# Eun0/XMC-GAN

Measured on AMD Instinct MI355X. Metric: images/sec per G+D step, higher is better.
Workload: dtype bf16; 1 GPU; 256x256 COCO-shaped synthetic batch, 256 images per GPU, one full G+D iteration (D step + G step + Adam x2), df_gan_damsm_nomagp.yml; per_gpu_batch=256, global_batch=256, image_size=256, cfg=df_gan_damsm_nomagp.yml, parallelism=dp1, hipgraph=True, losses_finite=True, workload_name=headline

## Files before the change

include/xmc_gan_hip.h:

```cpp
#ifndef XMC_GAN_HIP_H
#define XMC_GAN_HIP_H

#include <stdint.h>

#ifdef __cplusplus
extern "C" {
#endif

#define XMC_ABI_VERSION 12

enum { XMC_BF16 = 0, XMC_F32 = 1 };
enum { XMC_HALF_IS_BF16 = 0, XMC_HALF_IS_F16 = 1 };
enum { XMC_ACT_NONE = 0, XMC_ACT_LRELU = 1, XMC_ACT_TANH = 2, XMC_ACT_RELU = 3 };
enum { XMC_EINVAL = -1, XMC_EALIGN = -2, XMC_ESHAPE = -3 };

#define XMC_MAX_TAPS 16
#define XMC_MAX_CLASSES 4

typedef struct XmcConvDesc {
    const void* src;
    const void* wpk;
    void* dst;
    const float* bias;
    const void* res;
// ... 12 lines not shown
    int8_t dw[XMC_MAX_CLASSES][XMC_MAX_TAPS];
    int8_t wi[XMC_MAX_CLASSES][XMC_MAX_TAPS];
    int8_t dph[XMC_MAX_CLASSES];
    int8_t dpw[XMC_MAX_CLASSES];
    const void* mask;
    float res_scale;
    int32_t res_mode;
    void* dst2;
    void* dst_pool;
    int32_t round_act;
    int32_t groups;
    int32_t post_act;
    float pool_scale;
    void* sign_bits;
    float* dot;
    const void* mask_bits;
    const void* sc_img;
    const void* sc_frag;
    const float* sc_bias;
    void* splitk_ws;
    int64_t splitk_ws_bytes;
    const void* wpk_lo;
} XmcConvDesc;

int xmc_abi_version(void);
int xmc_half_format(void);
const char* xmc_last_kernel(void);
int xmc_set_fixed_order(int on);
int xmc_set_prezeroed(int on);

int64_t xmc_conv_splitk_ws_bytes(const XmcConvDesc* d);

int xmc_conv_igemm(const XmcConvDesc* d, void* stream);

int xmc_conv_wgrad(const XmcConvDesc* d , float* dwp, void* stream);
#define XMC_BIAS_REPLICAS 16
int xmc_conv_wgrad_bias(const XmcConvDesc* d, float* dwp, float* dbias, void* stream);

int xmc_pack_weight(const float* w, void* wpk, int Co, int Ci, int KH, int KW, int rows_pad, int cols_pad,
                    int transpose , int dtype, const int32_t* row_perm , void* stream);
int xmc_pack_weight_grouped(const float* w, void* wpk, int Co, int Ci, int KH, int KW, int rows_pad, int cols_pad, int transpose,
                            int dtype, const int32_t* row_perm, int groups, void* stream);
int xmc_unpack_wgrad_grouped(const float* dwp, float* gw, int Co, int Ci, int KH, int KW, int rows_pad, int cols_pad,
                             const float* scale_dev, const int32_t* row_perm, int accumulate, int groups, void* stream);
#define XMC_PACK_MULTI_MAX 48
typedef struct XmcPackJob {
    const float* w;
    void* wpk;
    const int32_t* row_perm;
    int32_t Co, Ci, KHW, rows_pad, cols_pad, transpose, dtype, groups, upconv;
    int32_t lo;
} XmcPackJob;
int xmc_pack_weight_multi(const XmcPackJob* jobs , int njobs, void* stream);
int xmc_pack_weight_upconv(const float* w, void* wpk, int Co, int Ci, int rows_pad, int cols_pad, int transpose, int dtype,
                           void* stream);
int xmc_unpack_wgrad(const float* dwp, float* gw, int Co, int Ci, int KH, int KW, int rows_pad, int cols_pad,
                     const float* scale_dev, const int32_t* row_perm, int accumulate, void* stream);
int xmc_unpack_wgrad_bias(const float* dwp, float* gw, int Co, int Ci, int KH, int KW, int rows_pad, int cols_pad,
                          const float* scale_dev, const int32_t* row_perm, int accumulate,
                          const float* gb_replicas, float* gb, int CD, void* stream);
int xmc_unpack_wgrad_bias_dot(const float* dwp, float* gw, int Co, int Ci, int KH, int KW, int rows_pad, int cols_pad,
                              const float* scale_dev, const int32_t* row_perm, int accumulate,
                              const float* gb_replicas, float* gb, int CD, const float* bias_dot, float* dot, void* stream);

int xmc_nchw_to_nhwc8(const float* src , void* dst , int N, int C, int H, int W,
                      int dtype, void* stream);
// ... 223 lines not shown
```

xmc-gan_amd/csrc/common.h:

```cpp
#pragma once
#include <hip/hip_runtime.h>
#include <stdint.h>

#include "xmc_gan_hip.h"

#ifdef XMC_H16_IS_F16
typedef _Float16 xmc_h16;
#define XMC_MFMA_16x16x32 __builtin_amdgcn_mfma_f32_16x16x32_f16
#define XMC_MFMA_32x32x16 __builtin_amdgcn_mfma_f32_32x32x16_f16
#define XMC_HALF_FORMAT 1
#else
typedef __bf16 xmc_h16;
#define XMC_MFMA_16x16x32 __builtin_amdgcn_mfma_f32_16x16x32_bf16
#define XMC_MFMA_32x32x16 __builtin_amdgcn_mfma_f32_32x32x16_bf16
#define XMC_HALF_FORMAT 0
#endif
typedef __attribute__((ext_vector_type(8))) xmc_h16 bf16x8;
typedef __attribute__((ext_vector_type(4))) xmc_h16 bf16x4;
typedef __attribute__((ext_vector_type(4))) float f32x4;
typedef __attribute__((__vector_size__(4 * sizeof(short)))) short xmc_s16x4;
typedef __attribute__((ext_vector_type(4))) uint32_t u32x4;
typedef __attribute__((ext_vector_type(2))) uint32_t u32x2;

#define XMC_LRELU 0.2f
// ... 78 lines not shown

struct XcdWalk { int first, step, end; };
__device__ __forceinline__ XcdWalk xmc_xcd_walk(int ntiles) {
    const int G = (int)gridDim.x, b = (int)blockIdx.x;
#ifdef XMC_XCD_HELPER_OFF
    return XcdWalk{b, G, ntiles};
#endif
    if ((G & 7) != 0 || G < 16) return XcdWalk{b, G, ntiles};
    const int T8 = (ntiles + 7) >> 3, base = (b & 7) * T8;
    return XcdWalk{base + (b >> 3), G >> 3, base + T8 < ntiles ? base + T8 : ntiles};
}
static inline int xmc_ab_grid(int g) {
    static const bool off = xmc_debug_off("no_xcd_map");
    return (off && g >= 16 && (g & 7) == 0) ? g - 1 : g;
}

__device__ __forceinline__ float xmc_xor1(float v) {
    return __builtin_bit_cast(float, __builtin_amdgcn_mov_dpp(__builtin_bit_cast(int, v), 0xB1, 0xF, 0xF, true));
}
__device__ __forceinline__ float xmc_xor2(float v) {
    return __builtin_bit_cast(float, __builtin_amdgcn_mov_dpp(__builtin_bit_cast(int, v), 0x4E, 0xF, 0xF, true));
}
__device__ __forceinline__ float wave_sum(float v) {
#pragma unroll
    for (int o = 32; o > 0; o >>= 1) v += __shfl_xor(v, o, 64);
    return v;
}
__device__ __forceinline__ float wave_max(float v) {
#pragma unroll
    for (int o = 32; o > 0; o >>= 1) v = fmaxf(v, __shfl_xor(v, o, 64));
    return v;
}

template <int ODT>
__device__ __forceinline__ void epilogue_tail(const XmcConvDesc& d, size_t idx8, size_t ridx8, float (&v)[8], float alpha, float* dacc = nullptr) {
    if (d.sign_bits) {
        unsigned b = 0;
#pragma unroll
        for (int k = 0; k < 8; ++k) b |= (v[k] > 0.f ? 1u : 0u) << k;
        reinterpret_cast<unsigned char*>(d.sign_bits)[idx8] = (unsigned char)b;
    }
    if (d.dst2) Vec8<ODT>::store(d.dst2, idx8, v);
    if (ODT == XMC_BF16 && (d.dst2 || d.round_act)) {
#pragma unroll
        for (int k = 0; k < 8; ++k) v[k] = (float)(xmc_h16)v[k];
    }
    float mk[8];
    if (d.mask) {
        Vec8<ODT>::load(d.mask, idx8, mk);
        if (d.dot && dacc) {
#pragma unroll
            for (int k = 0; k < 8; ++k) *dacc += v[k] * mk[k];
        }
    }
    if (d.alpha_dev) {
#pragma unroll
        for (int k = 0; k < 8; ++k) v[k] *= alpha;
    }
    if (d.mask) {
#pragma unroll
        for (int k = 0; k < 8; ++k) v[k] *= lrelu_slope(mk[k]);
    }
    if (d.res) {
        const float rs = d.res_scale == 0.f ? 1.f : d.res_scale;
        float rr[8];
        Vec8<ODT>::load(d.res, ridx8, rr);
#pragma unroll
        for (int k = 0; k < 8; ++k) v[k] += rs * rr[k];
    }
    if (d.post_act == XMC_ACT_LRELU) {
#pragma unroll
        for (int k = 0; k < 8; ++k) v[k] = lrelu_f(v[k]);
    }
    Vec8<ODT>::store(d.dst, idx8, v);
}

constexpr int kEpiBias = 1, kEpiLrelu = 2, kEpiRound = 4, kEpiDst2 = 8, kEpiAlpha = 16, kEpiMask = 32, kEpiRes = 64, kEpiPost = 128, kEpiPool = 256,
              kEpiSign = 512, kEpiDot = 1024, kEpiScImg = 2048;
constexpr int kEpiGSum = kEpiBias | kEpiRound | kEpiAlpha | kEpiRes;
constexpr int kEpiDKeep = kEpiLrelu | kEpiDst2 | kEpiAlpha | kEpiRes | kEpiPool;
constexpr int kEpiDFwd = kEpiLrelu | kEpiRound | kEpiAlpha | kEpiRes | kEpiPool;
constexpr int kEpiDLast = kEpiLrelu | kEpiDst2 | kEpiAlpha | kEpiRes;
constexpr int kEpiDLin = kEpiDst2 | kEpiAlpha | kEpiMask | kEpiRes;
constexpr int kEpiDKeepS = kEpiLrelu | kEpiRound | kEpiSign | kEpiAlpha | kEpiRes | kEpiPool;
constexpr int kEpiDLastS = kEpiLrelu | kEpiRound | kEpiSign | kEpiAlpha | kEpiRes;
constexpr int kEpiDgDot = kEpiMask | kEpiAlpha | kEpiDot;
static inline int xmc_epi_mask(const XmcConvDesc& d) {
    if ((d.act != XMC_ACT_NONE && d.act != XMC_ACT_LRELU) || d.out_dtype != XMC_BF16) return -1;
    return (d.bias ? kEpiBias : 0) | (d.act == XMC_ACT_LRELU ? kEpiLrelu : 0) | ((d.round_act && !d.dst2) ? kEpiRound : 0) | (d.dst2 ? kEpiDst2 : 0) |
           (d.alpha_dev ? kEpiAlpha : 0) | (d.mask ? kEpiMask : 0) | (d.res ? kEpiRes : 0) | (d.post_act == XMC_ACT_LRELU ? kEpiPost : 0) |
           (d.dst_pool ? kEpiPool : 0) | (d.sign_bits ? kEpiSign : 0) | (d.dot ? kEpiDot : 0) | (d.sc_img ? kEpiScImg : 0);
}

__device__ __forceinline__ size_t res_index8(const XmcConvDesc& d, size_t idx8, int n, int y, int x, int a, int b, int ch8) {
    if (d.res_mode == 0) return idx8;
    if (d.res_mode == 1) return ((size_t)(n * d.MH + a) * d.MW + b) * (d.CD >> 3) + ch8;
    return ((size_t)(n * (d.DH >> 1) + (y >> 1)) * (d.DW >> 1) + (x >> 1)) * (d.CD >> 3) + ch8;
}
```

xmc-gan_amd/csrc/conv_igemm.hip:

```cpp
#include "common.h"
#include <stdlib.h>

#ifndef XMC_IGEMM_PIN
#define XMC_IGEMM_PIN 1
#endif

namespace {

template <int DT> struct Mma;
template <> struct Mma<XMC_BF16> {
    __device__ static __forceinline__ f32x4 run(u32x4 a, u32x4 b, f32x4 c) {
        return XMC_MFMA_16x16x32(__builtin_bit_cast(bf16x8, a), __builtin_bit_cast(bf16x8, b), c, 0, 0, 0);
    }
};
template <> struct Mma<XMC_F32> {
    __device__ static __forceinline__ f32x4 run(u32x4 a, u32x4 b, f32x4 c) {
        f32x4 af = __builtin_bit_cast(f32x4, a), bf = __builtin_bit_cast(f32x4, b);
#pragma unroll
        for (int j = 0; j < 4; ++j) c = __builtin_amdgcn_mfma_f32_16x16x4f32(af[j], bf[j], c, 0, 0, 0);
        return c;
    }
};

__device__ __forceinline__ int swz(int row) {
    int q = (row >> 2) & 3;
    return (((q ^ (q >> 1)) & 1) << 1) | (q >> 1);
}

template <int BM, int BN, int KSUB>
struct IgemmLds {
    static constexpr int STAGE_U = 2 * KSUB * (BM + BN) * 4;
    static constexpr int EP_LD = BN + 4;
    static constexpr int EP_ROWS = BN > 128 ? 64 : (BM > 128 ? 128 : BM);
    static constexpr int EP_U = (EP_ROWS * EP_LD * 4 + 15) / 16;
    static constexpr int SMEM_U = STAGE_U > EP_U ? STAGE_U : EP_U;
    static constexpr bool DYNAMIC = SMEM_U * 16 + 4 * XMC_MAX_TAPS > 64 * 1024;
};

template <int ODT>
__device__ __forceinline__ void igemm_epi_item(const XmcConvDesc& d, int cls, int m, int ch, float (&v)[8], float alpha, float* dacc) {
    const int MHW = d.MH * d.MW;
    const int n = m / MHW, rem = m - n * MHW;
    const int a = rem / d.MW, b = rem - a * d.MW;
    const int dph = d.dph[cls], dpw = d.dpw[cls];
    const size_t pix = ((size_t)n * d.DH + a * d.DA + dph) * d.DW + b * d.DA + dpw;
    const size_t idx8 = (pix * d.CD + ch) >> 3;
    if (d.bias) {
#pragma unroll
        for (int k = 0; k < 8; ++k) v[k] += d.bias[ch + k];
    }
    if (d.act == XMC_ACT_LRELU) {
#pragma unroll
        for (int k = 0; k < 8; ++k) v[k] = lrelu_f(v[k]);
    } else if (d.act == XMC_ACT_RELU) {
#pragma unroll
        for (int k = 0; k < 8; ++k) v[k] = fmaxf(v[k], 0.f);
    } else if (d.act == XMC_ACT_TANH) {
#pragma unroll
        for (int k = 0; k < 8; ++k) v[k] = tanhf(v[k]);
    }
    const size_t ridx8 = res_index8(d, idx8, n, a * d.DA + dph, b * d.DA + dpw, a, b, ch >> 3);
    epilogue_tail<ODT>(d, idx8, ridx8, v, alpha, dacc);
}

template <int DT, int BM, int BN, int WM, int WN, int KSUB, bool SK = false>
__global__ __launch_bounds__(64 * WM * WN) void igemm_kernel(const XmcConvDesc d) {
    constexpr int NT = 64 * WM * WN;
    static_assert(WM * WN == 4 || WM * WN == 8, "4 or 8 waves");
    constexpr int RP = NT / 4;
    constexpr int WTM = BM / WM, WTN = BN / WN;
    constexpr int TM = WTM / 16, TN = WTN / 16;
    constexpr int AL = BM * 4 / NT;
    constexpr int BL = (BN * 4 + NT - 1) / NT;
    using Lds = IgemmLds<BM, BN, KSUB>;
    constexpr int EP_LD = Lds::EP_LD, EP_ROWS = Lds::EP_ROWS;
    extern __shared__ u32x4 smem_dyn[];
    __shared__ u32x4 smem_static[Lds::DYNAMIC ? 1 : Lds::SMEM_U];
    u32x4* const smem = Lds::DYNAMIC ? smem_dyn : smem_static;
    __shared__ int s_tap[XMC_MAX_TAPS];

    const int tid = threadIdx.x, lane = tid & 63, wave = tid >> 6;
    const int wm = wave / WN, wn = wave % WN;
    const int cls = blockIdx.z;
    const int MHW = d.MH * d.MW;
    const int M = d.N * MHW;
    int mt, nt;
    {
        const int MT = (M + BM - 1) / BM, NTn = d.CDw / BN;
        const int bid = blockIdx.x, nwg = MT * NTn;
        const int xcd = bid & 7, j = bid >> 3;
        const int q = nwg >> 3, r = nwg & 7;
        const int lin = (xcd < r ? xcd * (q + 1) : r * (q + 1) + (xcd - r) * q) + j;
        mt = lin / NTn; nt = lin - mt * NTn;
    }
    const int m0 = mt * BM, n0 = nt * BN;
    constexpr int ESZ = DT == XMC_BF16 ? 2 : 4;
    const int upt = d.CS * ESZ / 16;
    const int ktot = d.ntaps * upt;
    const int nsub = (ktot + 3) / 4;
// ... 117 lines not shown
    const float alpha = d.alpha_dev ? *d.alpha_dev : 1.f;
    float dacc = 0.f;
    constexpr int CPR = BN / 8;
    for (int half = 0; half < BM / EP_ROWS; ++half) {
        if (half) __syncthreads();
#pragma unroll
        for (int i = 0; i < TM; ++i) {
            const int rbase = wm * WTM + i * 16;
            if (rbase / EP_ROWS == half) {
#pragma unroll
                for (int j = 0; j < TN; ++j)
#pragma unroll
                    for (int r = 0; r < 4; ++r)
                        ep[(rbase - half * EP_ROWS + fc * 4 + r) * EP_LD + wn * WTN + j * 16 + fr] = acc[i][j][r];
            }
        }
        __syncthreads();
        for (int id = tid; id < EP_ROWS * CPR; id += NT) {
            int row = id / CPR, cc = id - row * CPR;
            int m = m0 + half * EP_ROWS + row, ch = n0 + cc * 8;
            if (m >= M) continue;
            const f32x4 e0 = *reinterpret_cast<const f32x4*>(&ep[row * EP_LD + cc * 8]);
            const f32x4 e1 = *reinterpret_cast<const f32x4*>(&ep[row * EP_LD + cc * 8 + 4]);
            if (SK) {
                f32x4* w = reinterpret_cast<f32x4*>(reinterpret_cast<float*>(d.splitk_ws) +
                                                    (((size_t)blockIdx.y * gridDim.z + cls) * M + m) * d.CDw + ch);
                w[0] = e0; w[1] = e1;
                continue;
            }
            if (ch >= d.CD) continue;
            float v[8];
#pragma unroll
            for (int k = 0; k < 4; ++k) { v[k] = e0[k]; v[4 + k] = e1[k]; }
            if (d.out_dtype == XMC_BF16) igemm_epi_item<XMC_BF16>(d, cls, m, ch, v, alpha, &dacc);
            else igemm_epi_item<XMC_F32>(d, cls, m, ch, v, alpha, &dacc);
        }
    }
    if (SK) return;
    if (d.dot) {
        dacc = wave_sum(dacc);
        if (lane == 0) atomicAdd(d.dot, dacc);
    }
}

constexpr int SK_FIN_ITEMS = 4;
__global__ __launch_bounds__(256) void igemm_splitk_finish_kernel(const XmcConvDesc d, int S) {
    const int cls = blockIdx.z;
    const int M = d.N * d.MH * d.MW, C8 = d.CD / 8;
    const float alpha = d.alpha_dev ? *d.alpha_dev : 1.f;
    float dacc = 0.f;
    for (int it = 0; it < SK_FIN_ITEMS; ++it) {
        const int64_t id = ((int64_t)blockIdx.x * SK_FIN_ITEMS + it) * 256 + threadIdx.x;
        if (id >= (int64_t)M * C8) break;
        const int m = (int)(id / C8), ch = (int)(id - (int64_t)m * C8) * 8;
        const float* w = reinterpret_cast<const float*>(d.splitk_ws) + ((size_t)cls * M + m) * d.CDw + ch;
        const size_t stride = (size_t)gridDim.z * M * d.CDw;
        float v[8] = {0, 0, 0, 0, 0, 0, 0, 0};
        for (int s = 0; s < S; ++s) {
            const f32x4 e0 = *reinterpret_cast<const f32x4*>(w + s * stride), e1 = *reinterpret_cast<const f32x4*>(w + s * stride + 4);
#pragma unroll
            for (int k = 0; k < 4; ++k) { v[k] += e0[k]; v[4 + k] += e1[k]; }
        }
        if (d.out_dtype == XMC_BF16) igemm_epi_item<XMC_BF16>(d, cls, m, ch, v, alpha, &dacc);
        else igemm_epi_item<XMC_F32>(d, cls, m, ch, v, alpha, &dacc);
    }
    if (d.dot) {
        __shared__ float sdot[4];
        dacc = wave_sum(dacc);
        if ((threadIdx.x & 63) == 0) sdot[threadIdx.x >> 6] = dacc;
        __syncthreads();
        if (threadIdx.x == 0) atomicAdd(d.dot, sdot[0] + sdot[1] + sdot[2] + sdot[3]);
    }
}

struct SkPlan { int S, big; };
static SkPlan splitk_plan(const XmcConvDesc& d) {
    static const bool off = xmc_debug_off("no_igemm_splitk"), no_big = xmc_debug_off("no_igemm_splitk256");
    SkPlan p = {0, 0};
    if (off || d.dtype != XMC_BF16 || d.CDw % 64 != 0) return p;
    const int64_t M = (int64_t)d.N * d.MH * d.MW, K = (int64_t)d.ntaps * d.CS;
    if (M > 16384 || K < 4096 || d.nclass != 1) return p;
    const int nstep = (int)((K * 2 / 16 + 3) / 4 + 1) / 2;
    p.big = (d.CDw % 256 == 0 && !no_big) ? 1 : (d.CDw % 128 == 0 ? 0 : 2);
    if (p.big == 1) {
        const int64_t t256 = (M + 255) / 256 * (d.CDw / 256);
        if (t256 * (nstep / 4 < 8 ? nstep / 4 : 8) < 192) p.big = 0;
    }
    const int BMp = p.big == 1 ? 256 : 128, BNp = p.big == 1 ? 256 : (p.big == 0 ? 128 : 64);
    const int64_t tiles = (M + BMp - 1) / BMp * (d.CDw / BNp) * d.nclass;
    int S = (int)((p.big == 1 ? 256 : 1024) / tiles);
    if (S > (p.big == 2 ? 16 : 8)) S = p.big == 2 ? 16 : 8;
    if (S > nstep / 4) S = nstep / 4;
    p.S = S >= 2 ? S : 0;
    return p;
}
static int64_t splitk_bytes(const XmcConvDesc& d, int S) { return (int64_t)S * d.nclass * d.N * d.MH * d.MW * d.CDw * 4; }

template <int BM, int BN, int WM, int WN>
int launch_splitk(const XmcConvDesc& d, int S, hipStream_t st) {
    const int64_t M = (int64_t)d.N * d.MH * d.MW;
    dim3 grid((unsigned)(((M + BM - 1) / BM) * (d.CDw / BN)), (unsigned)S, (unsigned)d.nclass);
    using Lds = IgemmLds<BM, BN, 2>;
    size_t dyn = 0;
    if (Lds::DYNAMIC) {
        dyn = (size_t)Lds::SMEM_U * 16;
        XMC_ALLOW_BIG_LDS((igemm_kernel<XMC_BF16, BM, BN, WM, WN, 2, true>));
    }
    hipLaunchKernelGGL((igemm_kernel<XMC_BF16, BM, BN, WM, WN, 2, true>), grid, dim3(64 * WM * WN), dyn, st, d);
    xmc_note_kernel("igemm_kernel<%d, %d, %d, %d, %d, %d, true>", XMC_BF16, BM, BN, WM, WN, 2);
    XMC_LAUNCH_CHECK();
    const int64_t items = M * (d.CD / 8);
    hipLaunchKernelGGL(igemm_splitk_finish_kernel, dim3((unsigned)((items + 256 * SK_FIN_ITEMS - 1) / (256 * SK_FIN_ITEMS)), 1, (unsigned)d.nclass), dim3(256), 0, st, d, S);
    XMC_LAUNCH_CHECK();
    return 0;
}

template <int DT, int BM, int BN, int WM, int WN, int KSUB>
int launch(const XmcConvDesc& d, hipStream_t st) {
    const int64_t M = (int64_t)d.N * d.MH * d.MW;
    dim3 grid((unsigned)(((M + BM - 1) / BM) * (d.CDw / BN)), 1, (unsigned)d.nclass);
    using Lds = IgemmLds<BM, BN, KSUB>;
    size_t dyn = 0;
    if (Lds::DYNAMIC) {
        dyn = (size_t)Lds::SMEM_U * 16;
        XMC_ALLOW_BIG_LDS((igemm_kernel<DT, BM, BN, WM, WN, KSUB>));
    }
    hipLaunchKernelGGL((igemm_kernel<DT, BM, BN, WM, WN, KSUB>), grid, dim3(64 * WM * WN), dyn, st, d);
    xmc_note_kernel("igemm_kernel<%d, %d, %d, %d, %d, %d>", DT, BM, BN, WM, WN, KSUB);
    XMC_LAUNCH_CHECK();
    return 0;
}

template <int DT>
int dispatch(const XmcConvDesc& d, hipStream_t st) {
    static const int variant = xmc_debug_off("igemm128") ? 1 : 0;
    static const bool no_small = xmc_debug_off("no_small_m");
    if (DT == XMC_BF16 && d.splitk_ws) {
        const SkPlan sp = splitk_plan(d);
        if (sp.S && d.splitk_ws_bytes >= splitk_bytes(d, sp.S))
            return sp.big == 1 ? launch_splitk<256, 256, 2, 4>(d, sp.S, st) : sp.big == 0 ? launch_splitk<128, 128, 2, 2>(d, sp.S, st)
                                                                                             : launch_splitk<128, 64, 4, 1>(d, sp.S, st);
    }
    if (!no_small && (int64_t)d.N * d.MH * d.MW <= 1024) return launch<DT, 128, 32, 4, 1, 2>(d, st);
    if (d.CDw % 128 == 0) {
        const int64_t M = (int64_t)d.N * d.MH * d.MW;
        if (variant == 1) return launch<DT, 128, 128, 2, 2, 2>(d, st);
        static const bool no_big = xmc_debug_off("no_igemm256");
        const int64_t tiles256 = (M + 255) / 256 * (d.CDw / 256) * d.nclass;
        if (DT == XMC_BF16 && (M >= 256 * 256 || tiles256 >= 256) && d.CDw % 256 == 0 && !no_big) return launch<DT, 256, 256, 2, 4, 2>(d, st);
        if (DT == XMC_BF16 && M >= 256 * 256) return launch<DT, 256, 128, 2, 2, 1>(d, st);
        static const bool no_m64 = xmc_debug_off("no_igemm_m64");
        static const bool no_k4 = xmc_debug_off("no_igemm_ksub4");
        const bool deepk = DT == XMC_BF16 && !no_k4 && (int64_t)d.ntaps * d.CS >= 2048;
        const int64_t t128 = (M + 127) / 128 * (d.CDw / 128) * d.nclass;
        if (DT == XMC_BF16 && !no_m64 && t128 < 256) {
            if (deepk && (M + 63) / 64 * (d.CDw / 128) * d.nclass <= 256) return launch<DT, 64, 128, 2, 2, 4>(d, st);
            return launch<DT, 64, 128, 2, 2, 2>(d, st);
        }
        if (deepk && t128 <= 256) return launch<DT, 128, 128, 2, 2, 4>(d, st);
        return launch<DT, 128, 128, 2, 2, 2>(d, st);
    }
    if (d.CDw % 64 == 0) {
        static const bool no_k4b = xmc_debug_off("no_igemm_ksub4");
        const int64_t Mb = (int64_t)d.N * d.MH * d.MW;
        if (DT == XMC_BF16 && !no_k4b && (int64_t)d.ntaps * d.CS >= 2048 && (Mb + 127) / 128 * (d.CDw / 64) * d.nclass <= 256)
            return launch<DT, 128, 64, 4, 1, 4>(d, st);
        return launch<DT, 128, 64, 4, 1, 2>(d, st);
    }
    return launch<DT, 128, 32, 4, 1, 2>(d, st);
}

}

int xmc_conv_tile_try(const XmcConvDesc* d, void* stream);
int xmc_conv_thin_try(const XmcConvDesc* d, void* stream);
int xmc_conv_pw1x1_try(const XmcConvDesc* d, void* stream);
int xmc_conv_wtile_try(const XmcConvDesc* d, void* stream);
int xmc_conv_wtile3_try(const XmcConvDesc* d, void* stream);
int xmc_conv_ptile_pool_try(const XmcConvDesc* d, void* stream);
int xmc_conv_ptile_slab128_try(const XmcConvDesc* d, void* stream);
int xmc_conv_group_try(const XmcConvDesc* d, void* stream);
int xmc_conv_thin_out_try(const XmcConvDesc* d, void* stream);

extern "C" int64_t xmc_conv_splitk_ws_bytes(const XmcConvDesc* d) {
    if (!d) return 0;
    const SkPlan sp = splitk_plan(*d);
    return sp.S ? splitk_bytes(*d, sp.S) : 0;
}

extern "C" int xmc_conv_igemm(const XmcConvDesc* d, void* stream) {
    if (!d || !d->src || !d->wpk || !d->dst) return XMC_EINVAL;
    if (d->dtype != XMC_BF16 && d->dtype != XMC_F32) return XMC_EINVAL;
    if (d->out_dtype != XMC_BF16 && d->out_dtype != XMC_F32) return XMC_EINVAL;
    const int esz = xmc_esz(d->dtype);
    if (d->ntaps < 1 || d->ntaps > XMC_MAX_TAPS || d->nclass < 1 || d->nclass > XMC_MAX_CLASSES) return XMC_ESHAPE;
    if ((d->CS * esz) % 16 != 0 || d->CD % 8 != 0 || d->CDw % 32 != 0 || d->CDw < d->CD) return XMC_EALIGN;
    if (d->N < 1 || d->MH < 1 || d->MW < 1 || d->SH < 1 || d->SW < 1 || d->DH < 1 || d->DW < 1) return XMC_ESHAPE;
    if (d->src_shift < 0 || d->src_shift > 1 || d->SA < 1 || d->DA < 1) return XMC_ESHAPE;
    for (int z = 0; z < d->nclass; ++z)
        if ((d->MH - 1) * d->DA + d->dph[z] >= d->DH || (d->MW - 1) * d->DA + d->dpw[z] >= d->DW || d->dph[z] < 0 || d->dpw[z] < 0)
            return XMC_ESHAPE;
    if ((int64_t)d->N * d->MH * d->MW >= (1ll << 31)) return XMC_ESHAPE;
    if (d->dst_pool && (d->DA != 1 || d->nclass != 1 || (d->DH & 1) || (d->DW & 1) || d->out_dtype != d->dtype)) return XMC_ESHAPE;
    if (d->post_act != XMC_ACT_NONE && d->post_act != XMC_ACT_LRELU) return XMC_EINVAL;
    if (d->dot && !d->mask) return XMC_EINVAL;
    if (d->mask_bits) return XMC_EINVAL;
    if (d->sc_img) return XMC_EINVAL;
    if (d->wpk_lo) return XMC_EINVAL;
    if (d->res_mode < 0 || d->res_mode > 2 || (d->res_mode == 2 && (d->DA != 1 || (d->DH & 1) || (d->DW & 1)))) return XMC_ESHAPE;
    static const bool no_tile = xmc_debug_off("no_tile");
    static const bool no_wt2 = xmc_debug_off("no_wtile_v2");
    static const bool no_wt3 = xmc_debug_off("no_wtile3");
    int rc = 1;
    if (!no_tile && d->dst_pool) {
        rc = xmc_conv_thin_try(d, stream);
        if (rc > 0 && !no_wt3) rc = xmc_conv_wtile3_try(d, stream);
        if (rc > 0 && !no_wt2) rc = xmc_conv_wtile_try(d, stream);
        if (rc > 0) rc = xmc_conv_ptile_pool_try(d, stream);
        if (rc <= 0) return rc;
    }
    XmcConvDesc dd = *d;
    dd.dst_pool = nullptr;
    if (!no_tile) {
        rc = xmc_conv_group_try(&dd, stream);
        if (rc > 0) rc = xmc_conv_thin_try(&dd, stream);
        if (rc > 0) rc = xmc_conv_thin_out_try(&dd, stream);
        if (rc > 0) rc = xmc_conv_pw1x1_try(&dd, stream);
        if (rc > 0) rc = xmc_conv_ptile_slab128_try(&dd, stream);
        if (rc > 0 && !no_wt3) rc = xmc_conv_wtile3_try(&dd, stream);
        if (rc > 0 && !no_wt2) rc = xmc_conv_wtile_try(&dd, stream);
        if (rc > 0) rc = xmc_conv_tile_try(&dd, stream);
        if (rc < 0) return rc;
    }
    if (rc > 0) {
        hipStream_t st = reinterpret_cast<hipStream_t>(stream);
        rc = dd.dtype == XMC_BF16 ? dispatch<XMC_BF16>(dd, st) : dispatch<XMC_F32>(dd, st);
        if (rc != 0) return rc;
    }
    if (d->dst_pool) return xmc_sumpool2(d->dst, d->dst_pool, d->N, d->DH, d->DW, d->CD, d->pool_scale == 0.f ? 0.25f : d->pool_scale, d->out_dtype, stream);
    return 0;
}
```

xmc-gan_amd/csrc/conv_tile.hip:

```cpp
#include "common.h"
#include <stdlib.h>
#include <type_traits>

namespace {

struct TileCfg {
    int TH, TW, log2TW;
    int tiles_y, tiles_x;
    int PH[XMC_MAX_CLASSES], PW[XMC_MAX_CLASSES];
    int dh0[XMC_MAX_CLASSES], dw0[XMC_MAX_CLASSES];
    int PHu, PWu, dh0u, dw0u;
    int slab;
    int no_xcd;
};

template <int BN, int WM, int WN>
__global__ __launch_bounds__(256) void tile_kernel(const XmcConvDesc d, const TileCfg t) {
    constexpr int NT = 256, BM = 256;
    static_assert(WM * WN == 4, "4 waves");
    constexpr int WTM = BM / WM, WTN = BN / WN;
    constexpr int TM = WTM / 16, TN = WTN / 16;
    constexpr int EP_ROWS = 128, EP_LD = BN + 4;
    extern __shared__ __attribute__((aligned(16))) unsigned char smem[];

// ... 139 lines not shown
            size_t pix = ((size_t)img * d.DH + (a0 + ty) * d.DA + dph) * d.DW + (b0 + tx) * d.DA + dpw;
            size_t idx8 = (pix * d.CD + ch) >> 3;
            float v[8];
            const f32x4 e0 = *reinterpret_cast<const f32x4*>(&ep[row * EP_LD + cc * 8]);
            const f32x4 e1 = *reinterpret_cast<const f32x4*>(&ep[row * EP_LD + cc * 8 + 4]);
#pragma unroll
            for (int k = 0; k < 4; ++k) { v[k] = e0[k]; v[4 + k] = e1[k]; }
            if (d.bias) {
#pragma unroll
                for (int k = 0; k < 8; ++k) v[k] += d.bias[ch + k];
            }
            if (d.act == XMC_ACT_LRELU) {
#pragma unroll
                for (int k = 0; k < 8; ++k) v[k] = lrelu_f(v[k]);
            } else if (d.act == XMC_ACT_RELU) {
#pragma unroll
                for (int k = 0; k < 8; ++k) v[k] = fmaxf(v[k], 0.f);
            } else if (d.act == XMC_ACT_TANH) {
#pragma unroll
                for (int k = 0; k < 8; ++k) v[k] = tanhf(v[k]);
            }
            const size_t ridx8 = res_index8(d, idx8, img, (a0 + ty) * d.DA + dph, (b0 + tx) * d.DA + dpw, a0 + ty, b0 + tx, (n0 >> 3) + cc);
            if (d.out_dtype == XMC_BF16) epilogue_tail<XMC_BF16>(d, idx8, ridx8, v, alpha, &dacc);
            else epilogue_tail<XMC_F32>(d, idx8, ridx8, v, alpha, &dacc);
        }
    }
    if (d.dot) {
        dacc = wave_sum(dacc);
        if (lane == 0) atomicAdd(d.dot, dacc);
    }
}


template <int BN, int SLAB, int NTAPS, int MC, int SA = 1, bool M32 = false, int EPI = -1>
__global__ __launch_bounds__(512) void ptile3_kernel(const XmcConvDesc d, const TileCfg t, int ntiles) {
    static_assert(!M32 || (SA == 1 && NTAPS > 0), "32x32x16 form: unit stride, unrolled taps");
    constexpr int NS = 256;
    constexpr int TM = SA == 1 ? 4 : 2, TN = BN / 16;
    constexpr int cps = SLAB / 8;
    constexpr int pstride = SLAB * 2 + (M32 ? 16 : 32);
    constexpr int PIT = ((SA == 1 ? 384 : 18 * 34) * cps + NS - 1) / NS;
    constexpr int UPL = BN / 32;
    constexpr int S = SLAB / 32;
    extern __shared__ __attribute__((aligned(16))) unsigned char smem[];

    const int tid = threadIdx.x, lane = tid & 63, wave = tid >> 6;
    const bool stager = wave >= 4;
    const int rt = tid & (NS - 1);
    const int wm = wave & 3;
    const int cls = MC > 1 ? 0 : blockIdx.z;
    const int n0 = blockIdx.y * BN;
    const int tpi = t.tiles_y * t.tiles_x;
    const int PH = MC > 1 ? t.PHu : t.PH[cls], PW = MC > 1 ? t.PWu : t.PW[cls];
    const int dh0 = MC > 1 ? t.dh0u : t.dh0[cls], dw0 = MC > 1 ? t.dw0u : t.dw0[cls];
    __shared__ int s_toff[XMC_MAX_TAPS];
    __shared__ __attribute__((aligned(16))) float s_bias[M32 ? 2 * BN : 4];
    if (M32 && tid >= 64 && tid < 64 + BN) {
        const int ch = n0 + tid - 64;
        s_bias[tid - 64] = (d.bias && ch < d.CD) ? d.bias[ch] : 0.f;
        s_bias[BN + tid - 64] = (d.sc_bias && ch < d.CD) ? d.sc_bias[ch] : 0.f;
    }
    if (tid < XMC_MAX_TAPS) {
        const int sl = tid < MC * d.ntaps ? tid : 0;
        const int c = MC > 1 ? sl / d.ntaps : cls, tt = MC > 1 ? sl % d.ntaps : sl;
        const int th = d.dh[c][tt] - dh0, tw = d.dw[c][tt] - dw0;
        s_toff[tid] = (SA == 1 ? th * PW + tw : (th * 2 + (tw & 1)) * (PW >> 1) + (tw >> 1)) * pstride;
    }
    const int cs_units = d.CS / 8;
    unsigned char* patch = smem;
// ... 317 lines not shown
                            dst8[idx8] = o;
                        }
                    if (MC == 1 && e_pool) {
                        bf16x8* __restrict__ pool8 = reinterpret_cast<bf16x8*>(d.dst_pool);
#pragma unroll
                        for (int v2 = 0; v2 < 2; ++v2) {
                            if (t.log2TW == 5) {
                                bf16x8 o;
#pragma unroll
                                for (int r = 0; r < 8; ++r) {
                                    float sm = fin[0][v2][r] + fin[1][v2][r];
                                    sm += xmc_xor1(sm);
                                    o[r] = (xmc_h16)(pscale * sm);
                                }
                                if ((l32 & 1) == 0)
                                    pool8[((img * (d.DH >> 1) + ((a0 + pty[0]) >> 1)) * (d.DW >> 1) + ((b0 + ptx[0]) >> 1)) * cd8 + (n0 >> 3) + ub + v2] = o;
                            } else {
#pragma unroll
                                for (int pb = 0; pb < 2; ++pb) {
                                    bf16x8 o;
#pragma unroll
                                    for (int r = 0; r < 8; ++r) {
                                        float sm = fin[pb][v2][r];
                                        sm += __shfl_xor(sm, 16, 64);
                                        sm += xmc_xor1(sm);
                                        o[r] = (xmc_h16)(pscale * sm);
                                    }
                                    if ((l32 & 17) == 0)
                                        pool8[((img * (d.DH >> 1) + ((a0 + pty[pb]) >> 1)) * (d.DW >> 1) + ((b0 + ptx[pb]) >> 1)) * cd8 + (n0 >> 3) + ub + v2] = o;
                                }
                            }
                        }
                    }
                }
                if (e_sign && pack_sign) {
#pragma unroll
                    for (int pb = 0; pb < 2; ++pb) {
                        const unsigned keep = hh == 0 ? (sgn[pb] & 0xFFFFu) : (sgn[pb] >> 16);
                        const unsigned send = hh == 0 ? (sgn[pb] >> 16) : (sgn[pb] & 0xFFFFu);
                        const unsigned recv = (unsigned)__shfl_xor((int)send, 32, 64);
                        const unsigned word = hh == 0 ? (keep | (recv << 16)) : (recv | (keep << 16));
                        reinterpret_cast<unsigned*>(d.sign_bits)[(size_t)(eo[pb] >> 2) + hh] = word;
                    }
                }
            }
        }
        if (e_dot) {
            dacc = wave_sum(dacc);
            if (lane == 0) atomicAdd(d.dot, dacc);
        }
    } else {
        const int fr = lane & 15, fc = lane >> 4;
        const int cd8 = d.CD / 8;
        int abyte[TM], eoff[TM], roff[TM];
#pragma unroll
        for (int i = 0; i < TM; ++i) {
            const int ml = wm * (16 * TM) + i * 16 + fr;
            const int ty = ml >> t.log2TW, tx = ml & (t.TW - 1);
            abyte[i] = ((SA == 1 ? ty * PW : 2 * ty * PW) + tx) * pstride + fc * 16;
            eoff[i] = ((ty * d.DA) * d.DW + tx * d.DA) * cd8 + fc;
            roff[i] = (ty * d.MW + tx) * cd8 + fc;
        }
        const int bbyte = fr * pstride + fc * 16;
        const int ch0 = n0 + fc * 8;
        const float alpha = d.alpha_dev ? *d.alpha_dev : 1.f;
        const float pscale = d.pool_scale == 0.f ? 0.25f : d.pool_scale;
        float bias8[UPL][8];
#pragma unroll
        for (int u = 0; u < UPL; ++u)
#pragma unroll
            for (int c = 0; c < 8; ++c) bias8[u][c] = (d.bias && ch0 + u * 32 < d.CD) ? d.bias[ch0 + u * 32 + c] : 0.f;
        constexpr bool RT = EPI < 0;
        constexpr int EB = RT ? 0 : (EPI & ~kEpiBias);
        const bool fast = RT ? (d.out_dtype == XMC_BF16 && d.res == nullptr && d.mask == nullptr && d.alpha_dev == nullptr && d.dst2 == nullptr &&
                                d.dst_pool == nullptr && d.post_act == XMC_ACT_NONE && d.sign_bits == nullptr && d.dot == nullptr &&
                                (d.act == XMC_ACT_NONE || d.act == XMC_ACT_LRELU || d.act == XMC_ACT_TANH))
                             : (EB == 0 || EB == kEpiLrelu);
        const bool do_tanh = RT ? d.act == XMC_ACT_TANH : false;
        const float slope = RT ? (d.act == XMC_ACT_LRELU ? XMC_LRELU : 1.f) : ((EPI & kEpiLrelu) ? XMC_LRELU : 1.f);
        const bool e_lrelu = RT ? d.act == XMC_ACT_LRELU : (EPI & kEpiLrelu) != 0;
        const bool e_relu = RT ? d.act == XMC_ACT_RELU : false;
        const bool e_round = RT ? (d.dst2 != nullptr || d.round_act != 0) : (EPI & (kEpiRound | kEpiDst2)) != 0;
        const bool e_dst2 = RT ? d.dst2 != nullptr : (EPI & kEpiDst2) != 0;
        const bool e_alpha = RT ? d.alpha_dev != nullptr : (EPI & kEpiAlpha) != 0;
        const bool e_mask = RT ? d.mask != nullptr : (EPI & kEpiMask) != 0;
        const bool e_res = RT ? d.res != nullptr : (EPI & kEpiRes) != 0;
        const bool e_post = RT ? d.post_act == XMC_ACT_LRELU : (EPI & kEpiPost) != 0;
        const bool e_pool = RT ? d.dst_pool != nullptr : (EPI & kEpiPool) != 0;
        constexpr bool e_sign = !RT && (EPI & kEpiSign) != 0;
        constexpr bool e_dot = !RT && (EPI & kEpiDot) != 0;
        float dacc = 0.f;
        __syncthreads();
        int toffr[NTAPS > 0 ? MC * NTAPS : 1];
        if constexpr (NTAPS > 0) {
#pragma unroll
            for (int k = 0; k < MC * NTAPS; ++k) toffr[k] = __builtin_amdgcn_readfirstlane(s_toff[k]);
        }
        for (int tile = tile0; tile < xlim; tile += tstep) {
            const int img = tile / tpi, trem = tile - img * tpi;
            const int a0 = (trem / t.tiles_x) * t.TH, b0 = (trem % t.tiles_x) * t.TW;
            __syncthreads();
            constexpr bool HOIST = UPL == 1;
            bf16x8 mkv[HOIST ? TM : 1], rrv[HOIST ? TM : 1];
#pragma unroll
          for (int mc = 0; mc < MC; ++mc) {
            const int ccls = MC > 1 ? mc : cls;
// ... 54 lines not shown
                for (int g = 0; g < G; ++g) fr_[0][gslot(g)] = rd(0, gslot(g));
#pragma unroll
                for (int st = 0; st < NST; ++st) {
                    const int cur = st & 1, nxt = cur ^ 1;
#pragma unroll
                    for (int g = 0; g < G; ++g) {
                        if (st + 1 < NST) fr_[nxt][gslot(g)] = rd(st + 1, gslot(g));
#pragma unroll
                        for (int m = g * M / G; m < (g + 1) * M / G; ++m) {
                            const int mi = m % TM, mj = m / TM;
                            acc[mi][mj] = XMC_MFMA_16x16x32(__builtin_bit_cast(bf16x8, fr_[cur][TM + mj]),
                                                                                   __builtin_bit_cast(bf16x8, fr_[cur][mi]), acc[mi][mj], 0, 0, 0);
                        }
                        __builtin_amdgcn_sched_barrier(0);
                    }
                }
            } else {
                u32x4 pf[2][TM], wf[2][TN];
                const int nsteps = d.ntaps * S;
                ldfrag(s_toff[0], 0, 0, pf[0], wf[0]);
                for (int step = 0; step < nsteps; step += 2) {
                    if (step + 1 < nsteps) ldfrag(s_toff[(step + 1) / S], (step + 1) / S, (step + 1) % S, pf[1], wf[1]);
                    mma(pf[0], wf[0]);
                    if (step + 2 < nsteps) ldfrag(s_toff[(step + 2) / S], (step + 2) / S, (step + 2) % S, pf[0], wf[0]);
                    if (step + 1 < nsteps) mma(pf[1], wf[1]);
                }
            }
            if (mc == MC - 1) __syncthreads();
            if (fast) {
                bf16x8* __restrict__ dst8 = reinterpret_cast<bf16x8*>(d.dst) + dbase;
#pragma unroll
                for (int u = 0; u < UPL; ++u) {
                    if (ch0 + u * 32 >= d.CD) continue;
#pragma unroll
                    for (int i = 0; i < TM; ++i) {
                        bf16x8 o;
                        if (slope != 1.f) {
#pragma unroll
                            for (int q = 0; q < 4; ++q) {
                                const float x0 = acc[i][2 * u][q] + bias8[u][q], x1 = acc[i][2 * u + 1][q] + bias8[u][4 + q];
                                o[q] = (xmc_h16)fmaxf(x0, x0 * slope);
                                o[4 + q] = (xmc_h16)fmaxf(x1, x1 * slope);
                            }
                        } else if (do_tanh) {
#pragma unroll
                            for (int q = 0; q < 4; ++q) {
                                o[q] = (xmc_h16)tanh_fast(acc[i][2 * u][q] + bias8[u][q]);
                                o[4 + q] = (xmc_h16)tanh_fast(acc[i][2 * u + 1][q] + bias8[u][4 + q]);
                            }
                        } else {
#pragma unroll
                            for (int q = 0; q < 4; ++q) {
                                o[q] = (xmc_h16)(acc[i][2 * u][q] + bias8[u][q]);
                                o[4 + q] = (xmc_h16)(acc[i][2 * u + 1][q] + bias8[u][4 + q]);
                            }
                        }
                        dst8[eoff[i] + u * 4] = o;
                    }
                }
            } else {
#pragma unroll
                for (int u = 0; u < UPL; ++u) {
                    if (ch0 + u * 32 >= d.CD) continue;
                    float fin[TM][8];
                    size_t rix[TM];
                    bf16x8 mkl[HOIST ? 1 : TM], rrl[HOIST ? 1 : TM];
                    if (!pre || !HOIST) {
#pragma unroll
                        for (int i = 0; i < TM; ++i) {
                            const size_t idx8 = (size_t)(dbase + eoff[i] + u * 4);
                            rix[i] = d.res_mode == 1 ? (size_t)(rbase + roff[i] + u * 4) : idx8;
                            if (d.res_mode == 2) {
                                const int ml_ = wm * (16 * TM) + i * 16 + fr;
                                const int y_ = (a0 + (ml_ >> t.log2TW)) * d.DA + dph, x_ = (b0 + (ml_ & (t.TW - 1))) * d.DA + dpw;
                                rix[i] = res_index8(d, idx8, img, y_, x_, 0, 0, (n0 >> 3) + fc + u * 4);
                            }
                            if (pre && e_mask) mkl[HOIST ? 0 : i] = reinterpret_cast<const bf16x8*>(d.mask)[idx8];
                            if (pre && e_res) rrl[HOIST ? 0 : i] = reinterpret_cast<const bf16x8*>(d.res)[rix[i]];
                        }
                    }
#pragma unroll
                    for (int i = 0; i < TM; ++i) {
                        const size_t idx8 = (size_t)(dbase + eoff[i] + u * 4);
                        float v[8];
#pragma unroll
                        for (int q = 0; q < 4; ++q) { v[q] = acc[i][2 * u][q] + bias8[u][q]; v[4 + q] = acc[i][2 * u + 1][q] + bias8[u][4 + q]; }
                        if (e_lrelu) {
#pragma unroll
                            for (int q = 0; q < 8; ++q) v[q] = lrelu_f(v[q]);
                        } else if (e_relu) {
// ... 48 lines not shown
                            for (int q = 0; q < 8; ++q) fin[i][q] = v[q];
                        }
                    }
                    if (SA == 1 && MC == 1 && TM == 4 && e_pool) {
                        bf16x8* __restrict__ pool8 = reinterpret_cast<bf16x8*>(d.dst_pool);
#pragma unroll
                        for (int pr = 0; pr < 2; ++pr) {
                            const int i0 = t.log2TW == 5 ? pr : 2 * pr;
                            const int ml_ = wm * 64 + i0 * 16 + fr;
                            const int ty_ = ml_ >> t.log2TW, tx_ = ml_ & (t.TW - 1);
                            bf16x8 o;
#pragma unroll
                            for (int q = 0; q < 8; ++q) {
                                float sm = t.log2TW == 5 ? fin[pr][q] + fin[(pr + 2) % TM][q] : fin[(2 * pr) % TM][q] + fin[(2 * pr + 1) % TM][q];
                                sm += xmc_xor1(sm);
                                o[q] = (xmc_h16)(pscale * sm);
                            }
                            if ((fr & 1) == 0)
                                pool8[((img * (d.DH >> 1) + ((a0 + ty_) >> 1)) * (d.DW >> 1) + ((b0 + tx_) >> 1)) * cd8 + (n0 >> 3) + fc + u * 4] = o;
                        }
                    }
                }
            }
          }
        }
        if (e_dot) {
            dacc = wave_sum(dacc);
            if (lane == 0) atomicAdd(d.dot, dacc);
        }
    }
}

template <int BN>
int launch_ptile(const XmcConvDesc& d, const TileCfg& t, hipStream_t st) {
    if (d.sc_img && !(d.SA == 1 && d.ntaps == 9 && d.nclass == 1 && t.slab == 64 && d.out_dtype == XMC_BF16 && (d.dst_pool || d.sign_bits))) return XMC_ESHAPE;
    int maxpatch = 0;
    for (int z = 0; z < d.nclass; ++z) maxpatch = t.PH[z] * t.PW[z] > maxpatch ? t.PH[z] * t.PW[z] : maxpatch;
    if (d.SA == 2) {
        const size_t lds2 = (size_t)((maxpatch * 96 + 15) & ~15) + (size_t)16 * BN * 96;
        if (lds2 > XMC_MAX_DYN_LDS || t.slab != 32) return XMC_ESHAPE;
        const int nt2 = d.N * t.tiles_y * t.tiles_x;
        int g2 = 256 / (int)(d.CDw / BN);
        if (g2 > nt2) g2 = nt2;
        static const bool no_epi2 = xmc_debug_off("no_ptile_epi");
        const int epi2 = no_epi2 ? -1 : (xmc_epi_mask(d) & ~kEpiBias);
#define XMC_PT3S2(E)                                                                                                        \
        if (epi2 == (E)) {                                                                                                  \
            XMC_ALLOW_BIG_LDS((ptile3_kernel<BN, 32, 16, 1, 2, false, (E)>));                                               \
            hipLaunchKernelGGL((ptile3_kernel<BN, 32, 16, 1, 2, false, (E)>), dim3(g2, d.CDw / BN, 1), dim3(512), lds2, st, d, t, nt2); \
            xmc_note_kernel("ptile3_kernel<%d, 32, 16, 1, 2>", BN);                                                         \
            XMC_LAUNCH_CHECK();                                                                                             \
            return 0;                                                                                                       \
        }
        XMC_PT3S2(kEpiLrelu) XMC_PT3S2(0) XMC_PT3S2(kEpiMask)
#undef XMC_PT3S2
        if (d.sign_bits || d.dot) return XMC_ESHAPE;
        xmc_note_generic_epi("ptile3<s2>", epi2);
        XMC_ALLOW_BIG_LDS((ptile3_kernel<BN, 32, 16, 1, 2>));
        hipLaunchKernelGGL((ptile3_kernel<BN, 32, 16, 1, 2>), dim3(g2, d.CDw / BN, 1), dim3(512), lds2, st, d, t, nt2);
        xmc_note_kernel("ptile3_kernel<%d, 32, 16, 1, 2>", BN);
        XMC_LAUNCH_CHECK();
        return 0;
    }
    if (maxpatch > 384) return XMC_ESHAPE;
    const int pstride = t.slab * 2 + 32;
    const size_t pb = (size_t)((maxpatch * pstride + 15) & ~15);
    const size_t lds = pb + (size_t)d.ntaps * BN * pstride;
    if (lds > XMC_MAX_DYN_LDS) return XMC_ESHAPE;
    const int ntiles = d.N * t.tiles_y * t.tiles_x;
    const int per_cu = (lds <= 80 * 1024 && BN == 32 && t.slab == 32) ? 2 : 1;
    int gx = 256 * per_cu / (int)((d.CDw / BN) * d.nclass);
    if (gx < 1) gx = 1;
    if (gx > ntiles) gx = ntiles;
    dim3 grid((unsigned)gx, (unsigned)(d.CDw / BN), (unsigned)d.nclass);
    if (t.slab == 128) {
        if (BN != 64 || d.ntaps != 4 || d.sign_bits || d.dot) return XMC_ESHAPE;
        const int epis = xmc_debug_off("no_ptile_epi") ? -1 : (xmc_epi_mask(d) & ~kEpiBias);
#define XMC_PT3W(E)                                                                                                         \
        if (epis == (E)) {                                                                                                  \
            XMC_ALLOW_BIG_LDS((ptile3_kernel<64, 128, 4, 1, 1, false, (E)>));                                               \
            hipLaunchKernelGGL((ptile3_kernel<64, 128, 4, 1, 1, false, (E)>), grid, dim3(512), lds, st, d, t, ntiles);      \
        } else
        XMC_PT3W(kEpiRes) XMC_PT3W(0)
#undef XMC_PT3W
        {
            xmc_note_generic_epi("ptile3<128>", epis);
            XMC_ALLOW_BIG_LDS((ptile3_kernel<64, 128, 4, 1>));
            hipLaunchKernelGGL((ptile3_kernel<64, 128, 4, 1>), grid, dim3(512), lds, st, d, t, ntiles);
        }
        xmc_note_kernel("ptile3_kernel<64, 128, 4, 1>");
        XMC_LAUNCH_CHECK();
        return 0;
    }
    if (d.nclass == 4 && d.ntaps == 4 && t.PHu * t.PWu <= 384) {
        const size_t ldsm = (size_t)((t.PHu * t.PWu * pstride + 15) & ~15) + (size_t)16 * BN * pstride;
        static const bool no_merge = xmc_debug_off("no_class_merge");
        if (ldsm <= XMC_MAX_DYN_LDS && !no_merge) {
            int gm = 256 / (int)(d.CDw / BN);
            if (gm > ntiles) gm = ntiles;
            dim3 gridm((unsigned)gm, (unsigned)(d.CDw / BN), 1);
            if (d.sign_bits || d.dot) return XMC_ESHAPE;
            static const bool no_epim = xmc_debug_off("no_ptile_epi");
            const int epim = no_epim ? -1 : (xmc_epi_mask(d) & ~kEpiBias);
#define XMC_PT3M(SL, E)                                                                                                     \
            if (t.slab == (SL) && epim == (E)) {                                                                            \
                XMC_ALLOW_BIG_LDS((ptile3_kernel<BN, SL, 4, 4, 1, false, (E)>));                                            \
                hipLaunchKernelGGL((ptile3_kernel<BN, SL, 4, 4, 1, false, (E)>), gridm, dim3(512), ldsm, st, d, t, ntiles); \
            } else
            XMC_PT3M(64, kEpiRes) XMC_PT3M(64, 0) XMC_PT3M(32, kEpiRes) XMC_PT3M(32, 0)
#undef XMC_PT3M
            if (t.slab == 64) {
                xmc_note_generic_epi("ptile3<4,4>", epim);
                XMC_ALLOW_BIG_LDS((ptile3_kernel<BN, 64, 4, 4>));
                hipLaunchKernelGGL((ptile3_kernel<BN, 64, 4, 4>), gridm, dim3(512), ldsm, st, d, t, ntiles);
            } else {
                XMC_ALLOW_BIG_LDS((ptile3_kernel<BN, 32, 4, 4>));
                hipLaunchKernelGGL((ptile3_kernel<BN, 32, 4, 4>), gridm, dim3(512), ldsm, st, d, t, ntiles);
            }
            xmc_note_kernel("ptile3_kernel<%d, %d, 4, 4>", BN, t.slab);
            XMC_LAUNCH_CHECK();
            return 0;
        }
    }
    static const bool no_m32 = xmc_debug_off("no_ptile_m32");
    static const bool m32_all = xmc_debug_off("ptile_m32_all");
    if (!no_m32 && d.ntaps == 9 && d.out_dtype == XMC_BF16 && t.slab == 64 &&
        (m32_all || d.res || d.dst2 || d.dst_pool || d.mask || d.sign_bits)) {
        int epi = xmc_epi_mask(d);
        static const bool no_epi = xmc_debug_off("no_ptile_epi");
        if (no_epi) epi = -1;
        if (d.sc_img) {
            if (BN != 64 || d.res || t.TW != 32 || d.CD != 64 || lds + 18 * 66 * 8 > XMC_MAX_DYN_LDS) return XMC_ESHAPE;
#define XMC_PT3_SCI(E)                                                                                                   \
            if (epi == (E)) {                                                                                            \
                XMC_ALLOW_BIG_LDS((ptile3_kernel<64, 64, 9, 1, 1, true, (E)>));                                          \
                hipLaunchKernelGGL((ptile3_kernel<64, 64, 9, 1, 1, true, (E)>), grid, dim3(512), lds + 18 * 66 * 8, st, d, t, ntiles); \
                xmc_note_kernel("ptile3_kernel<64, 64, 9, 1, 1, true, sc>");                                             \
                XMC_LAUNCH_CHECK();                                                                                      \
                return 0;                                                                                                \
            }
            XMC_PT3_SCI((kEpiDKeepS & ~kEpiRes) | kEpiScImg) XMC_PT3_SCI((kEpiDFwd & ~kEpiRes) | kEpiScImg)
#undef XMC_PT3_SCI
            return XMC_ESHAPE;
        }
#define XMC_PT3_EPI(E)                                                                                                   \
        if (epi == (E)) {                                                                                                \
            XMC_ALLOW_BIG_LDS((ptile3_kernel<BN, 64, 9, 1, 1, true, (E)>));                                              \
            hipLaunchKernelGGL((ptile3_kernel<BN, 64, 9, 1, 1, true, (E)>), grid, dim3(512), lds, st, d, t, ntiles);     \
            xmc_note_kernel("ptile3_kernel<%d, 64, 9, 1, 1, true>", BN);                                                 \
            XMC_LAUNCH_CHECK();                                                                                          \
            return 0;                                                                                                    \
        }
        XMC_PT3_EPI(kEpiGSum) XMC_PT3_EPI(kEpiDKeep) XMC_PT3_EPI(kEpiDFwd) XMC_PT3_EPI(kEpiDLast) XMC_PT3_EPI(kEpiDLin)
        XMC_PT3_EPI(kEpiDKeepS) XMC_PT3_EPI(kEpiDLastS) XMC_PT3_EPI(kEpiDgDot)
        XMC_PT3_EPI(kEpiMask)
#undef XMC_PT3_EPI
        if (d.sign_bits || d.dot) return XMC_ESHAPE;
        xmc_note_generic_epi("ptile3<M32>", epi);
// ... 100 lines not shown
    if (!(d->CS <= 64 && t.slab == d->CS && d->CDw <= 64) || xmc_debug_off("no_ptile")) return 1;
    const int rc = d->CDw == 64 ? launch_ptile<64>(*d, t, reinterpret_cast<hipStream_t>(stream))
                                : launch_ptile<32>(*d, t, reinterpret_cast<hipStream_t>(stream));
    return rc == XMC_ESHAPE ? 1 : rc;
}

extern "C" int xmc_conv_ptile_scimg(const XmcConvDesc* d, void* stream) {
    if (!d || !d->src || !d->wpk || !d->dst || !d->sc_img || !d->sc_frag || !d->sc_bias) return XMC_EINVAL;
    static const bool off = xmc_debug_off("no_scimg");
    if (off || d->res || d->dtype != XMC_BF16 || d->out_dtype != XMC_BF16 || d->SA != 1 || d->DA != 1 || d->nclass != 1 || d->ntaps != 9 ||
        d->src_shift != 0 || d->CS != 64 || d->CDw != 64 || d->CD != 64 || d->MW % 32 != 0 || d->MH % 8 != 0 || d->SH != d->MH || d->SW != d->MW ||
        d->DH != d->MH || d->DW != d->MW || xmc_debug_off("no_ptile") || xmc_debug_off("no_ptile_m32") || xmc_debug_off("no_ptile_epi"))
        return 1;
    for (int k = 0; k < 9; ++k)
        if (d->dh[0][k] < -1 || d->dh[0][k] > 1 || d->dw[0][k] < -1 || d->dw[0][k] > 1) return 1;
    TileCfg t;
    if (!tile_plan(d, &t) || t.slab != 64) return 1;
    const int rc = launch_ptile<64>(*d, t, reinterpret_cast<hipStream_t>(stream));
    return rc == XMC_ESHAPE ? 1 : rc;
}

extern "C" int xmc_conv_ptile_bits(const XmcConvDesc* d, void* stream) {
    if (!d || !d->src || !d->wpk || !d->dst || !d->mask_bits) return XMC_EINVAL;
    static const bool off = xmc_debug_off("no_stage_bits");
    if (off || d->dtype != XMC_BF16 || d->SA != 1 || d->DA != 1 || d->nclass != 1 || d->src_shift != 0 || d->dst_pool) return 1;
    TileCfg t;
    if (!tile_plan(d, &t)) return 1;
    if (!(d->CS <= 64 && t.slab == d->CS && d->CDw <= 64) || xmc_debug_off("no_ptile")) return 1;
    const int rc = d->CDw == 64 ? launch_ptile<64>(*d, t, reinterpret_cast<hipStream_t>(stream))
                                : launch_ptile<32>(*d, t, reinterpret_cast<hipStream_t>(stream));
    return rc == XMC_ESHAPE ? 1 : rc;
}

int xmc_conv_ptile_slab128_try(const XmcConvDesc* d, void* stream) {
    if (d->CS != 128 || d->CDw != 64 || d->ntaps != 4 || d->nclass != 4 || d->dst_pool || xmc_debug_off("no_ptile")) return 1;
    TileCfg t;
    if (!tile_plan(d, &t) || t.slab != 128) return 1;
    const int rc = launch_ptile<64>(*d, t, reinterpret_cast<hipStream_t>(stream));
    return rc == XMC_ESHAPE ? 1 : rc;
}

int xmc_conv_tile_try(const XmcConvDesc* d, void* stream) {
    TileCfg t;
    if (!tile_plan(d, &t)) return 1;
    if (t.slab == 128) return 1;
    hipStream_t st = reinterpret_cast<hipStream_t>(stream);
    int rc;
    static const bool no_pt = xmc_debug_off("no_ptile");
    if (!no_pt && d->CS <= 64 && t.slab == d->CS && d->CDw <= 64) {
        rc = d->CDw == 64 ? launch_ptile<64>(*d, t, st) : launch_ptile<32>(*d, t, st);
        if (rc != XMC_ESHAPE) return rc;
    }
    static const bool no_pt128 = xmc_debug_off("no_ptile_cd128");
    if (!no_pt && !no_pt128 && d->CS == 32 && t.slab == 32 && d->CDw == 128 && d->SA == 1 && d->nclass == 1 && d->ntaps == 9) {
        rc = launch_ptile<64>(*d, t, st);
        if (rc != XMC_ESHAPE) return rc;
    }
    if (d->SA != 1) return 1;
    if (d->CDw % 128 == 0) rc = launch_tile<128, 2, 2>(*d, t, st);
    else if (d->CDw % 64 == 0) rc = launch_tile<64, 4, 1>(*d, t, st);
    else rc = launch_tile<32, 4, 1>(*d, t, st);
    return rc == XMC_ESHAPE ? 1 : rc;
}
```

xmc-gan_amd/csrc/conv_wtile.hip:

```cpp
#include "common.h"
#include <stdlib.h>
#include <type_traits>

#ifndef WT_ABL
#define WT_ABL 0
#endif

namespace {

struct WtCfg {
    int TH, TW, log2TW;
    int tiles_y, tiles_x;
    int PH[XMC_MAX_CLASSES], PW[XMC_MAX_CLASSES];
    int dh0[XMC_MAX_CLASSES], dw0[XMC_MAX_CLASSES];
    int nslab;
    int patch_bytes;
    int8_t tsel[4][4];
};

constexpr int kPStride = 160;
constexpr int kPIT = 12;

template <int NTAPS, int MODE, int TN, int CW, int EPI = -1>
__global__ __launch_bounds__(64 * CW + 256) void wtile2_kernel(const XmcConvDesc d, const WtCfg t, int ntiles) {
    constexpr int BN = 16 * TN, TM = 4, NS = 64 * CW;
    constexpr int TNW = TN * 4 / CW;
    static_assert(CW == 4 || CW == 8, "4 or 8 compute waves");
    static_assert(TNW % 2 == 0, "a lane's 8-channel unit needs a pair of blocks");
    constexpr int WL = BN / 32;
    constexpr int WSTG = BN * 128;
    extern __shared__ __attribute__((aligned(16))) unsigned char smem[];
    __shared__ int s_toff[XMC_MAX_TAPS];
    __shared__ int s_wbase[XMC_MAX_TAPS];
    __shared__ int s_slab[64];

    const int tid = threadIdx.x, lane = tid & 63, wave = tid >> 6;
    const int n0 = blockIdx.y * BN;
    const int cls = blockIdx.z;
    const int tpi = t.tiles_y * t.tiles_x;
    const int PW = t.PW[cls];
    const int dh0 = MODE == 0 ? t.dh0[cls] : 0, dw0 = MODE == 0 ? t.dw0[cls] : 0;
    const int cs_units = d.CS / 8;
    const int nslab = t.nslab;
    const int cb = d.CS / 64;
    if (tid < XMC_MAX_TAPS) {
        if (MODE == 0) {
            const int tt = tid < NTAPS ? tid : 0;
            s_toff[tid] = ((d.dh[cls][tt] - dh0) * PW + (d.dw[cls][tt] - dw0)) * kPStride;
            s_wbase[tid] = d.wi[cls][tt] * d.CDw * cs_units;
        } else {
            const int g4 = tid >> 2, tp = tid & 3;
            s_toff[tid] = ((tp >> 1) * PW + (tp & 1)) * kPStride;
            s_wbase[tid] = d.wi[0][t.tsel[g4][tp]] * d.CDw * cs_units;
        }
    }
    if (tid >= 64 && tid < 128) {
        const int sl = tid - 64;
// ... 167 lines not shown
        auto rdw = [&](const unsigned char* wb, int sub, int mj) -> u32x4 {
            return *reinterpret_cast<const u32x4*>(wb + (sub ? bb1 : bb0) + mj * 2048);
        };
        const int ch0 = n0 + wn * (BN / 2) * (CW / 4 - 1) + fc * 8;
        const int nw8 = (n0 + wn * (BN / 2) * (CW / 4 - 1)) >> 3;
        auto epilogue = [&](int tile) {
            int lane_op = fr;
            asm volatile("" : "+v"(lane_op) :: "memory");
            const int img = tile / tpi, trem = tile - img * tpi;
            const int a0 = (trem / t.tiles_x) * t.TH, b0 = (trem % t.tiles_x) * t.TW;
            const int dbase = (((img * d.DH + a0 * d.DA + d.dph[cls]) * d.DW) + b0 * d.DA + d.dpw[cls]) * cd8 + nw8;
            const int rbase = d.res_mode ? ((img * d.MH + a0) * d.MW + b0) * cd8 + nw8 : dbase;
            const int rsy = d.res_mode ? d.MW : d.DA * d.DW, rsx = d.res_mode ? 1 : d.DA;
            constexpr bool RT = EPI < 0;
            const bool e_bias = RT ? d.bias != nullptr : (EPI & kEpiBias) != 0;
            const bool e_tanh = RT ? d.act == XMC_ACT_TANH : false;
            const bool e_round = RT ? (d.dst2 != nullptr || d.round_act != 0) : (EPI & (kEpiRound | kEpiDst2)) != 0;
            const bool e_dst2 = RT ? d.dst2 != nullptr : (EPI & kEpiDst2) != 0;
            const bool e_alpha = RT ? d.alpha_dev != nullptr : (EPI & kEpiAlpha) != 0;
            const bool e_mask = RT ? d.mask != nullptr : (EPI & kEpiMask) != 0;
            const bool e_res = RT ? d.res != nullptr : (EPI & kEpiRes) != 0;
            const bool e_post = RT ? d.post_act == XMC_ACT_LRELU : (EPI & kEpiPost) != 0;
            const bool e_pool = RT ? d.dst_pool != nullptr : (EPI & kEpiPool) != 0;
            constexpr bool e_sign = !RT && (EPI & kEpiSign) != 0;
            constexpr bool e_dot = !RT && (EPI & kEpiDot) != 0;
            const float slope = RT ? (d.act == XMC_ACT_LRELU ? XMC_LRELU : (d.act == XMC_ACT_RELU ? 0.f : 1.f)) : ((EPI & kEpiLrelu) ? XMC_LRELU : 1.f);
            const float alpha = d.alpha_dev ? *d.alpha_dev : 1.f;
            const float rs = d.res_scale == 0.f ? 1.f : d.res_scale;
            bf16x8* __restrict__ dst8 = reinterpret_cast<bf16x8*>(d.dst);
            const bf16x8* __restrict__ mask8 = reinterpret_cast<const bf16x8*>(d.mask);
            const bf16x8* __restrict__ res8 = reinterpret_cast<const bf16x8*>(d.res);
            bf16x8* __restrict__ dst2_8 = reinterpret_cast<bf16x8*>(d.dst2);
            bf16x8* __restrict__ pool8 = reinterpret_cast<bf16x8*>(d.dst_pool);
            int eo[TM], ro[TM];
#pragma unroll
            for (int i = 0; i < TM; ++i) {
                const int ml = wm * 64 + i * 16 + lane_op;
                const int ty = ml >> t.log2TW, tx = ml & (t.TW - 1);
                eo[i] = dbase + ((ty * d.DA) * d.DW + tx * d.DA) * cd8 + fc;
                if (d.res_mode == 2)
                    ro[i] = ((img * (d.DH >> 1) + ((a0 + ty) >> 1)) * (d.DW >> 1) + ((b0 + tx) >> 1)) * cd8 + nw8 + fc;
                else
                    ro[i] = rbase + (ty * rsy + tx * rsx) * cd8 + fc;
            }
#pragma unroll
            for (int u = 0; u < TNW / 2; ++u) {
                if (ch0 + u * 32 >= d.CD) continue;
                float fin[TM][8];
                bf16x8 mkv[TM], rrv[TM];
                if (e_mask) {
#pragma unroll
                    for (int i = 0; i < TM; ++i) mkv[i] = mask8[eo[i] + u * 4];
                }
                if (e_res) {
#pragma unroll
                    for (int i = 0; i < TM; ++i) rrv[i] = res8[ro[i] + u * 4];
                }
#pragma unroll
                for (int i = 0; i < TM; ++i) {
                    float v[8];
#pragma unroll
                    for (int r = 0; r < 4; ++r) { v[r] = acc[i][2 * u][r]; v[4 + r] = acc[i][2 * u + 1][r]; }
                    if (e_bias && !(WT_ABL & 32)) {
                        const f32x4 b0v = *reinterpret_cast<const f32x4*>(d.bias + ch0 + u * 32), b1v = *reinterpret_cast<const f32x4*>(d.bias + ch0 + u * 32 + 4);
#pragma unroll
                        for (int r = 0; r < 4; ++r) { v[r] += b0v[r]; v[4 + r] += b1v[r]; }
                    }
                    if (e_tanh) {
#pragma unroll
                        for (int r = 0; r < 8; ++r) v[r] = tanhf(v[r]);
                    } else if (slope != 1.f) {
#pragma unroll
                        for (int r = 0; r < 8; ++r) v[r] = fmaxf(v[r], v[r] * slope);
                    }
                    if (e_sign) {
                        unsigned sb = 0;
#pragma unroll
                        for (int r = 0; r < 8; ++r) sb |= (v[r] > 0.f ? 1u : 0u) << r;
                        reinterpret_cast<unsigned char*>(d.sign_bits)[eo[i] + u * 4] = (unsigned char)sb;
                    }
                    if (e_round) {
                        bf16x8 o2;
#pragma unroll
                        for (int r = 0; r < 8; ++r) { o2[r] = (xmc_h16)v[r]; v[r] = (float)o2[r]; }
                        if (e_dst2) dst2_8[eo[i] + u * 4] = o2;
                    }
                    if (e_dot && e_mask) {
#pragma unroll
                        for (int r = 0; r < 8; ++r) dacc += v[r] * (float)mkv[i][r];
                    }
                    if (e_alpha) {
#pragma unroll
                        for (int r = 0; r < 8; ++r) v[r] *= alpha;
                    }
                    if (e_mask) {
#pragma unroll
                        for (int r = 0; r < 8; ++r) v[r] *= lrelu_slope((float)mkv[i][r]);
                    }
                    if (e_res) {
#pragma unroll
                        for (int r = 0; r < 8; ++r) v[r] += rs * (float)rrv[i][r];
                    }
                    if (e_post) {
#pragma unroll
                        for (int r = 0; r < 8; ++r) v[r] = fmaxf(v[r], v[r] * XMC_LRELU);
                    }
                    bf16x8 o;
#pragma unroll
                    for (int r = 0; r < 8; ++r) { o[r] = (xmc_h16)v[r]; fin[i][r] = (float)o[r]; }
                    if (!(WT_ABL & 16)) dst8[eo[i] + u * 4] = o;
                    else asm volatile("" :: "v"(o));
                }
                if (e_pool) {
#pragma unroll
                    for (int pr = 0; pr < 2; ++pr) {
                        const int i0 = t.log2TW == 5 ? pr : 2 * pr, i1 = t.log2TW == 5 ? pr + 2 : 2 * pr + 1;
                        const int ml = wm * 64 + i0 * 16 + lane_op;
                        const int ty = ml >> t.log2TW, tx = ml & (t.TW - 1);
                        bf16x8 o;
#pragma unroll
                        for (int r = 0; r < 8; ++r) {
                            float sm = (t.log2TW == 5 ? fin[pr][r] + fin[pr + 2][r] : fin[2 * pr][r] + fin[2 * pr + 1][r]);
                            sm += xmc_xor1(sm);
                            o[r] = (xmc_h16)((d.pool_scale == 0.f ? 0.25f : d.pool_scale) * sm);
                        }
                        (void)i1;
                        if ((lane_op & 1) == 0)
                            pool8[((img * (d.DH >> 1) + ((a0 + ty) >> 1)) * (d.DW >> 1) + ((b0 + tx) >> 1)) * cd8 + nw8 + fc + u * 4] = o;
                    }
                }
            }
#pragma unroll
            for (int i = 0; i < TM; ++i)
#pragma unroll
                for (int j = 0; j < TNW; ++j) acc[i][j] = f32x4{0.f, 0.f, 0.f, 0.f};
        };
        int toffr[NTAPS];
#pragma unroll
        for (int k = 0; k < NTAPS; ++k) toffr[k] = __builtin_amdgcn_readfirstlane(s_toff[k]);
        __syncthreads();
        {
            const unsigned char* pa = patch0 + toffr[0];
#pragma unroll
            for (int k = 0; k < TM; ++k) P[0][k] = rdp(pa, 0, k);
// ... 72 lines not shown
            t->PH[z] = TH + (hmax - hmin); t->PW[z] = TW + (wmax - wmin);
            if (t->PH[z] * t->PW[z] > 32 * kPIT) return 0;
            if (d->SH != d->MH || d->SW != d->MW) return 0;
            maxpix = t->PH[z] * t->PW[z] > maxpix ? t->PH[z] * t->PW[z] : maxpix;
        }
    } else if (d->SA == 2) {
        if (d->ntaps != 16 || d->nclass != 1 || d->DA != 1 || d->SH != 2 * d->MH || d->SW != 2 * d->MW) return 0;
        *mode = 1;
        t->nslab = 4 * (d->CS / 64);
        if (t->nslab > 64) return 0;
        for (int g = 0; g < 4; ++g)
            for (int tp = 0; tp < 4; ++tp) {
                const int wh = 2 * (tp >> 1) + (g >> 1) - 1, ww = 2 * (tp & 1) + (g & 1) - 1;
                int found = -1;
                for (int k = 0; k < 16; ++k)
                    if (d->dh[0][k] == wh && d->dw[0][k] == ww) found = found < 0 ? k : 99;
                if (found < 0 || found > 15) return 0;
                t->tsel[g][tp] = (int8_t)found;
            }
        t->PH[0] = TH + 1; t->PW[0] = TW + 1; t->dh0[0] = t->dw0[0] = 0;
        maxpix = t->PH[0] * t->PW[0];
        if (maxpix > 32 * kPIT) return 0;
    } else {
        return 0;
    }
    if (d->dst_pool && (d->DA != 1 || d->nclass != 1 || (d->DH & 1) || (d->DW & 1))) return 0;
    if (d->res_mode == 2 && d->DA != 1) return 0;
    t->patch_bytes = (maxpix * kPStride + 15) & ~15;
    if ((int64_t)d->N * d->SH * d->SW * (d->CS / 8) >= (1ll << 31) || (int64_t)d->N * d->DH * d->DW * (d->CD / 8) >= (1ll << 31)) return 0;
    return 1;
}

template <int NTAPS, int MODE, int TN, int CW>
int launch(const XmcConvDesc& d, const WtCfg& t, hipStream_t st) {
    constexpr int BN = 16 * TN;
    const size_t lds = (size_t)3 * BN * 128 + 2 * (size_t)t.patch_bytes;
    if (lds > XMC_MAX_DYN_LDS) return XMC_ESHAPE;
    const int ntiles = d.N * t.tiles_y * t.tiles_x, ny = d.CDw / BN;
    int gx = 256 / (ny * d.nclass);
    if (gx < 1) gx = 1;
    if (gx > ntiles) gx = ntiles;
    gx = xmc_ab_grid(gx);
    static const bool no_epi = xmc_debug_off("no_wtile_epi");
    const int epi = (no_epi || CW != 8) ? -1 : xmc_epi_mask(d);
#define XMC_W2_EPI(E)                                                                                                                          \
    if (epi == (E)) {                                                                                                                          \
        XMC_ALLOW_BIG_LDS((wtile2_kernel<NTAPS, MODE, TN, CW, (E)>));                                                                          \
        hipLaunchKernelGGL((wtile2_kernel<NTAPS, MODE, TN, CW, (E)>), dim3((unsigned)gx, (unsigned)ny, (unsigned)d.nclass), dim3(64 * CW + 256), lds, st, \
                           d, t, ntiles);                                                                                                      \
        xmc_note_kernel("wtile2_kernel<%d, %d, %d, %d>", NTAPS, MODE, TN, CW);                                                                 \
        XMC_LAUNCH_CHECK();                                                                                                                    \
        return 0;                                                                                                                              \
    }
    if constexpr (CW == 8 && NTAPS == 9 && TN == 8) {
        XMC_W2_EPI(kEpiGSum) XMC_W2_EPI(kEpiDKeep) XMC_W2_EPI(kEpiDFwd) XMC_W2_EPI(kEpiDLast) XMC_W2_EPI(kEpiMask) XMC_W2_EPI(0) XMC_W2_EPI(kEpiDLin)
        XMC_W2_EPI(kEpiDKeepS) XMC_W2_EPI(kEpiDLastS) XMC_W2_EPI(kEpiDgDot)
        XMC_W2_EPI(kEpiBias) XMC_W2_EPI(kEpiBias | kEpiLrelu)
    } else if constexpr (CW == 8 && NTAPS == 9) {
        XMC_W2_EPI(kEpiBias) XMC_W2_EPI(kEpiBias | kEpiLrelu) XMC_W2_EPI(0)
    } else if constexpr (CW == 8 && MODE == 1 && TN == 8) {
        XMC_W2_EPI(kEpiLrelu) XMC_W2_EPI(0) XMC_W2_EPI(kEpiMask)
    } else if constexpr (CW == 8 && NTAPS == 4 && MODE == 0) {
        XMC_W2_EPI(kEpiRes) XMC_W2_EPI(kEpiBias) XMC_W2_EPI(0)
    }
#undef XMC_W2_EPI
    if (d.sign_bits || d.dot) return 1;
    xmc_note_generic_epi(NTAPS == 9 ? (TN == 8 ? "wtile2<9,0,8>" : "wtile2<9,0,4>") : MODE == 1 ? (TN == 8 ? "wtile2<4,1,8>" : "wtile2<4,1,4>") : "wtile2<4,0>", CW == 8 ? xmc_epi_mask(d) : -1);
    XMC_ALLOW_BIG_LDS((wtile2_kernel<NTAPS, MODE, TN, CW>));
    hipLaunchKernelGGL((wtile2_kernel<NTAPS, MODE, TN, CW>), dim3((unsigned)gx, (unsigned)ny, (unsigned)d.nclass), dim3(64 * CW + 256), lds, st, d, t,
                       ntiles);
    xmc_note_kernel("wtile2_kernel<%d, %d, %d, %d>", NTAPS, MODE, TN, CW);
    XMC_LAUNCH_CHECK();
    return 0;
}

}

int xmc_conv_wtile_try(const XmcConvDesc* d, void* stream) {
    WtCfg t;
    int mode = 0, tn = 8;
    if (!plan(d, &t, &mode, &tn)) return 1;
    hipStream_t st = reinterpret_cast<hipStream_t>(stream);
    int rc;
    static const bool cw4 = xmc_debug_off("wtile_cw4");
#define WT_GO(NT_, MD_, TN_) (cw4 ? launch<NT_, MD_, TN_, 4>(*d, t, st) : launch<NT_, MD_, TN_, 8>(*d, t, st))
    if (mode == 1) rc = tn == 8 ? WT_GO(4, 1, 8) : WT_GO(4, 1, 4);
    else if (d->ntaps == 9) rc = tn == 8 ? WT_GO(9, 0, 8) : WT_GO(9, 0, 4);
    else rc = tn == 8 ? WT_GO(4, 0, 8) : WT_GO(4, 0, 4);
#undef WT_GO
    return rc == XMC_ESHAPE ? 1 : rc;
}
```

xmc-gan_amd/csrc/conv_wtile3.hip:

```cpp
#include "common.h"
#include <stdlib.h>
#include <type_traits>

namespace {

struct W3Cfg {
    int TH, TW, log2TW;
    int tiles_y, tiles_x;
    int PH[XMC_MAX_CLASSES], PW[XMC_MAX_CLASSES];
    int dh0[XMC_MAX_CLASSES], dw0[XMC_MAX_CLASSES];
    int nslab;
    int patch_bytes;
    int8_t tsel[4][4];
    int ipt;
};

constexpr int kPI = 6;
constexpr int kPieces = 47;
constexpr int kPatchSlots = kPieces * 8;

__device__ __attribute__((aligned(16))) unsigned char g_zero16[16];

typedef __attribute__((address_space(3))) unsigned char lds_u8;
typedef const __attribute__((address_space(1))) void* gptr_t;

__device__ __forceinline__ void glds16(const void* src, lds_u8* dst) {
    __builtin_amdgcn_global_load_lds((gptr_t)src, (__attribute__((address_space(3))) void*)dst, 16, 0, 0);
}

template <int NTAPS, int MODE, int WM, int EPI = -1>
__global__ __launch_bounds__(512) void wtile3_kernel(const XmcConvDesc d, const W3Cfg t, int ntiles) {
    constexpr int WN = 8 / WM, BN = 64 * WN;
    constexpr int TMW = 16 / WM;
    constexpr int TNW = 4;
    constexpr int NPH = TMW / 2;
    constexpr int RING = WM == 2 ? 2 : 4;
    constexpr int WSTG = BN * 128;
    constexpr int NI = BN / 64;
    constexpr int PPS = (kPI + NTAPS - 1) / NTAPS;
    extern __shared__ __attribute__((aligned(16))) unsigned char smem[];
    unsigned char* const wring = smem;
    unsigned char* const patch0 = smem + RING * WSTG;
    const int pbytes = t.patch_bytes;
    int* const s_toff = reinterpret_cast<int*>(smem + RING * WSTG + 2 * pbytes);
    int* const s_wbase = s_toff + XMC_MAX_TAPS;
    int* const s_slab = s_wbase + XMC_MAX_TAPS;

    const int tid = threadIdx.x, lane = tid & 63;
    const int wave = __builtin_amdgcn_readfirstlane(tid >> 6);
    const int half = wave >> 2;
    const int wr = WM == 2 ? (wave >> 2) : (wave & 3);
    const int wc = WM == 2 ? (wave & 3) : (wave >> 2);
    const int n0 = blockIdx.y * BN;
    const int cls = blockIdx.z;
    const int tpi = t.tiles_y * t.tiles_x;
    const int PW = t.PW[cls], PH = t.PH[cls];
    const int dh0 = MODE == 0 ? t.dh0[cls] : 0, dw0 = MODE == 0 ? t.dw0[cls] : 0;
    const int cs_units = d.CS / 8;
    const int nslab = t.nslab;
    const int cb = d.CS / 64;
    const bool mi = t.ipt > 1;
    if (tid < XMC_MAX_TAPS) {
        if (MODE == 0) {
            const int tt = tid < NTAPS ? tid : 0;
// ... 118 lines not shown

    const int cd8 = d.CD / 8;
    const int ch0 = n0 + wc * 64 + fc * 8;
    const int nw8 = (n0 + wc * 64) >> 3;
    auto epilogue = [&](int tile) {
        int lane_op = fr;
        asm volatile("" : "+v"(lane_op) :: "memory");
        const int timg = tile / tpi, trem = tile - timg * tpi, img = timg * t.ipt;
        const int a0 = (trem / t.tiles_x) * t.TH, b0 = (trem % t.tiles_x) * t.TW;
        const int dbase = (((img * d.DH + a0 * d.DA + d.dph[cls]) * d.DW) + b0 * d.DA + d.dpw[cls]) * cd8 + nw8;
        const int dimg = d.DH * d.DW * cd8, rimg = d.res_mode ? d.MH * d.MW * cd8 : dimg;
        const int rbase = d.res_mode ? ((img * d.MH + a0) * d.MW + b0) * cd8 + nw8 : dbase;
        const int rsy = d.res_mode ? d.MW : d.DA * d.DW, rsx = d.res_mode ? 1 : d.DA;
        constexpr bool RT = EPI < 0;
        const bool e_bias = RT ? d.bias != nullptr : (EPI & kEpiBias) != 0;
        const bool e_tanh = RT ? d.act == XMC_ACT_TANH : false;
        const bool e_round = RT ? (d.dst2 != nullptr || d.round_act != 0) : (EPI & (kEpiRound | kEpiDst2)) != 0;
        const bool e_dst2 = RT ? d.dst2 != nullptr : (EPI & kEpiDst2) != 0;
        const bool e_alpha = RT ? d.alpha_dev != nullptr : (EPI & kEpiAlpha) != 0;
        const bool e_mask = RT ? d.mask != nullptr : (EPI & kEpiMask) != 0;
        const bool e_res = RT ? d.res != nullptr : (EPI & kEpiRes) != 0;
        const bool e_post = RT ? d.post_act == XMC_ACT_LRELU : (EPI & kEpiPost) != 0;
        const bool e_pool = RT ? d.dst_pool != nullptr : (EPI & kEpiPool) != 0;
        constexpr bool e_sign = !RT && (EPI & kEpiSign) != 0;
        constexpr bool e_dot = !RT && (EPI & kEpiDot) != 0;
        const float slope = RT ? (d.act == XMC_ACT_LRELU ? XMC_LRELU : (d.act == XMC_ACT_RELU ? 0.f : 1.f)) : ((EPI & kEpiLrelu) ? XMC_LRELU : 1.f);
        const float alpha = d.alpha_dev ? *d.alpha_dev : 1.f;
        const float rs = d.res_scale == 0.f ? 1.f : d.res_scale;
        bf16x8* __restrict__ dst8 = reinterpret_cast<bf16x8*>(d.dst);
        const bf16x8* __restrict__ mask8 = reinterpret_cast<const bf16x8*>(d.mask);
        const bf16x8* __restrict__ res8 = reinterpret_cast<const bf16x8*>(d.res);
        bf16x8* __restrict__ dst2_8 = reinterpret_cast<bf16x8*>(d.dst2);
        bf16x8* __restrict__ pool8 = reinterpret_cast<bf16x8*>(d.dst_pool);
#pragma unroll
        for (int g = 0; g < TMW / 4; ++g) {
            int eo[4], ro[4];
#pragma unroll
            for (int i = 0; i < 4; ++i) {
                const int ml = wr * (256 / WM) + (g * 4 + i) * 16 + lane_op;
                const int ty = ml >> t.log2TW, txt = ml & (t.TW - 1);
                const int tx = mi ? (txt & 7) : txt, ki = mi ? (txt >> 3) : 0;
                eo[i] = dbase + ((ty * d.DA) * d.DW + tx * d.DA) * cd8 + ki * dimg + fc;
                if (d.res_mode == 2)
                    ro[i] = (((img + ki) * (d.DH >> 1) + ((a0 + ty) >> 1)) * (d.DW >> 1) + ((b0 + tx) >> 1)) * cd8 + nw8 + fc;
                else
                    ro[i] = rbase + (ty * rsy + tx * rsx) * cd8 + ki * rimg + fc;
            }
#pragma unroll
            for (int u = 0; u < TNW / 2; ++u) {
                if (ch0 + u * 32 >= d.CD) continue;
                float fin[4][8];
                bf16x8 mkv[4], rrv[4];
                if (e_mask) {
#pragma unroll
                    for (int i = 0; i < 4; ++i) mkv[i] = mask8[eo[i] + u * 4];
                }
                if (e_res) {
#pragma unroll
                    for (int i = 0; i < 4; ++i) rrv[i] = res8[ro[i] + u * 4];
                }
#pragma unroll
                for (int i = 0; i < 4; ++i) {
                    float v[8];
#pragma unroll
                    for (int r = 0; r < 4; ++r) { v[r] = acc[g * 4 + i][2 * u][r]; v[4 + r] = acc[g * 4 + i][2 * u + 1][r]; }
                    if (e_bias) {
                        const f32x4 b0v = *reinterpret_cast<const f32x4*>(d.bias + ch0 + u * 32), b1v = *reinterpret_cast<const f32x4*>(d.bias + ch0 + u * 32 + 4);
#pragma unroll
                        for (int r = 0; r < 4; ++r) { v[r] += b0v[r]; v[4 + r] += b1v[r]; }
                    }
                    if (e_tanh) {
#pragma unroll
                        for (int r = 0; r < 8; ++r) v[r] = tanhf(v[r]);
                    } else if (slope != 1.f) {
#pragma unroll
                        for (int r = 0; r < 8; ++r) v[r] = fmaxf(v[r], v[r] * slope);
                    }
                    if (e_sign) {
                        unsigned sb = 0;
#pragma unroll
                        for (int r = 0; r < 8; ++r) sb |= (v[r] > 0.f ? 1u : 0u) << r;
                        reinterpret_cast<unsigned char*>(d.sign_bits)[eo[i] + u * 4] = (unsigned char)sb;
                    }
                    if (e_round) {
                        bf16x8 o2;
#pragma unroll
                        for (int r = 0; r < 8; ++r) { o2[r] = (xmc_h16)v[r]; v[r] = (float)o2[r]; }
                        if (e_dst2) dst2_8[eo[i] + u * 4] = o2;
                    }
                    if (e_dot && e_mask) {
#pragma unroll
                        for (int r = 0; r < 8; ++r) dacc += v[r] * (float)mkv[i][r];
                    }
                    if (e_alpha) {
#pragma unroll
                        for (int r = 0; r < 8; ++r) v[r] *= alpha;
                    }
                    if (e_mask) {
#pragma unroll
                        for (int r = 0; r < 8; ++r) v[r] *= lrelu_slope((float)mkv[i][r]);
                    }
                    if (e_res) {
#pragma unroll
                        for (int r = 0; r < 8; ++r) v[r] += rs * (float)rrv[i][r];
                    }
                    if (e_post) {
#pragma unroll
                        for (int r = 0; r < 8; ++r) v[r] = fmaxf(v[r], v[r] * XMC_LRELU);
                    }
                    bf16x8 o;
#pragma unroll
                    for (int r = 0; r < 8; ++r) { o[r] = (xmc_h16)v[r]; fin[i][r] = (float)o[r]; }
                    dst8[eo[i] + u * 4] = o;
                }
                if (e_pool) {
#pragma unroll
                    for (int pr = 0; pr < 2; ++pr) {
                        const int i0 = t.log2TW == 5 ? pr : 2 * pr;
                        const int ml = wr * (256 / WM) + (g * 4 + i0) * 16 + lane_op;
                        const int ty = ml >> t.log2TW, txt = ml & (t.TW - 1);
                        const int tx = mi ? (txt & 7) : txt, ki = mi ? (txt >> 3) : 0;
                        bf16x8 o;
#pragma unroll
                        for (int r = 0; r < 8; ++r) {
                            float sm = (t.log2TW == 5 ? fin[pr][r] + fin[pr + 2][r] : fin[2 * pr][r] + fin[2 * pr + 1][r]);
                            sm += xmc_xor1(sm);
                            o[r] = (xmc_h16)((d.pool_scale == 0.f ? 0.25f : d.pool_scale) * sm);
                        }
                        if ((lane_op & 1) == 0)
                            pool8[(((img + ki) * (d.DH >> 1) + ((a0 + ty) >> 1)) * (d.DW >> 1) + ((b0 + tx) >> 1)) * cd8 + nw8 + fc + u * 4] = o;
                    }
                }
            }
        }
#pragma unroll
        for (int i = 0; i < TMW; ++i)
#pragma unroll
            for (int j = 0; j < TNW; ++j) acc[i][j] = f32x4{0.f, 0.f, 0.f, 0.f};
    };

    int toffr[NTAPS];
#pragma unroll
    for (int k = 0; k < NTAPS; ++k) toffr[k] = __builtin_amdgcn_readfirstlane(s_toff[k]);

    patch_setup(0);
    if (MODE == 1) wbm_setup(0, 0);
// ... 138 lines not shown
                if (t->PH[z] * t->PW[z] > kPieces * 8 || (hmax > 0 ? (t->PH[z] - 1) * t->PW[z] : t->PH[z] * t->PW[z]) > (kPieces - 1) * 8) return 0;
            }
            if (d->SH != d->MH || d->SW != d->MW) return 0;
            if (!mi) maxpix = t->PH[z] * t->PW[z] > maxpix ? t->PH[z] * t->PW[z] : maxpix;
        }
    } else if (d->SA == 2) {
        if (d->ntaps != 16 || d->nclass != 1 || d->DA != 1 || d->SH != 2 * d->MH || d->SW != 2 * d->MW) return 0;
        *mode = 1;
        t->nslab = 4 * (d->CS / 64);
        if (t->nslab > 64) return 0;
        for (int g = 0; g < 4; ++g)
            for (int tp = 0; tp < 4; ++tp) {
                const int wh = 2 * (tp >> 1) + (g >> 1) - 1, ww = 2 * (tp & 1) + (g & 1) - 1;
                int found = -1;
                for (int k = 0; k < 16; ++k)
                    if (d->dh[0][k] == wh && d->dw[0][k] == ww) found = found < 0 ? k : 99;
                if (found < 0 || found > 15) return 0;
                t->tsel[g][tp] = (int8_t)found;
            }
        t->PH[0] = TH + 1; t->PW[0] = mi ? 36 : TW + 1; t->dh0[0] = t->dw0[0] = 0;
        maxpix = t->PH[0] * t->PW[0];
    } else {
        return 0;
    }
    if (maxpix > (kPieces - 1) * 8) return 0;
    if (d->dst_pool && (d->DA != 1 || d->nclass != 1 || (d->DH & 1) || (d->DW & 1))) return 0;
    if (d->res_mode == 2 && d->DA != 1) return 0;
    t->patch_bytes = kPatchSlots * 128;
    if ((int64_t)d->N * d->SH * d->SW * (d->CS / 8) >= (1ll << 31) || (int64_t)d->N * d->DH * d->DW * (d->CD / 8) >= (1ll << 31)) return 0;
    return 1;
}

template <int NTAPS, int MODE, int WM>
int launch3(const XmcConvDesc& d, const W3Cfg& t, hipStream_t st) {
    constexpr int BN = 64 * (8 / WM), RING = WM == 2 ? 2 : 4;
    const size_t lds = (size_t)RING * BN * 128 + 2 * (size_t)t.patch_bytes + (size_t)(2 * XMC_MAX_TAPS + 64) * sizeof(int);
    if (lds > XMC_MAX_DYN_LDS) return XMC_ESHAPE;
    const int ntiles = d.N / t.ipt * t.tiles_y * t.tiles_x, ny = d.CDw / BN;
    int gx = 256 / (ny * d.nclass);
    if (gx < 1) gx = 1;
    if (gx > ntiles) gx = ntiles;
    gx = xmc_ab_grid(gx);
    static const bool no_epi = xmc_debug_off("no_wtile_epi");
    const int epi = no_epi ? -1 : xmc_epi_mask(d);
#define XMC_W3_EPI(E)                                                                                                                        \
    if (epi == (E)) {                                                                                                                        \
        XMC_ALLOW_BIG_LDS((wtile3_kernel<NTAPS, MODE, WM, (E)>));                                                                            \
        hipLaunchKernelGGL((wtile3_kernel<NTAPS, MODE, WM, (E)>), dim3((unsigned)gx, (unsigned)ny, (unsigned)d.nclass), dim3(512), lds, st, d, t, ntiles); \
        xmc_note_kernel("wtile3_kernel<%d, %d, %d>", NTAPS, MODE, WM);                                                                       \
        XMC_LAUNCH_CHECK();                                                                                                                  \
        return 0;                                                                                                                            \
    }
    if constexpr (NTAPS == 9) {
        XMC_W3_EPI(kEpiGSum) XMC_W3_EPI(kEpiDKeep) XMC_W3_EPI(kEpiDFwd) XMC_W3_EPI(kEpiDLast) XMC_W3_EPI(kEpiMask) XMC_W3_EPI(0) XMC_W3_EPI(kEpiDLin)
        XMC_W3_EPI(kEpiDKeepS) XMC_W3_EPI(kEpiDLastS) XMC_W3_EPI(kEpiDgDot)
    } else if constexpr (MODE == 1) {
        XMC_W3_EPI(kEpiLrelu) XMC_W3_EPI(0) XMC_W3_EPI(kEpiMask)
    } else {
        XMC_W3_EPI(kEpiRes) XMC_W3_EPI(kEpiBias) XMC_W3_EPI(0)
    }
#undef XMC_W3_EPI
    if (d.sign_bits || d.dot) return 1;
    xmc_note_generic_epi(NTAPS == 9 ? "wtile3<9,0>" : MODE == 1 ? "wtile3<4,1>" : "wtile3<4,0>", epi);
    XMC_ALLOW_BIG_LDS((wtile3_kernel<NTAPS, MODE, WM>));
    hipLaunchKernelGGL((wtile3_kernel<NTAPS, MODE, WM>), dim3((unsigned)gx, (unsigned)ny, (unsigned)d.nclass), dim3(512), lds, st, d, t, ntiles);
    xmc_note_kernel("wtile3_kernel<%d, %d, %d>", NTAPS, MODE, WM);
    XMC_LAUNCH_CHECK();
    return 0;
}

}

int xmc_conv_wtile3_try(const XmcConvDesc* d, void* stream) {
    W3Cfg t;
    int mode = 0, wm = 2;
    if (!plan3(d, &t, &mode, &wm)) return 1;
    static const bool bn128 = xmc_debug_off("wtile3_bn128"), bn128_epi = xmc_debug_off("wtile3_bn128_epi"), bn128_plain = xmc_debug_off("wtile3_bn128_plain");
    const bool heavy = d->res || d->dst2 || d->dst_pool || d->mask || d->sign_bits;
    static const bool any_count = xmc_debug_off("wtile3_any_tile_count");
    const long long tiles = (long long)d->N / t.ipt * t.tiles_y * t.tiles_x * d->nclass;
    if (t.ipt > 1) {
        if (wm == 2 && tiles * (d->CDw / 256) < 256 && !any_count) wm = 4;
        if (wm == 4 && tiles * (d->CDw / 128) < 256 && !any_count) return 1;
    } else {
        if (wm == 4 && !(bn128 || (bn128_epi && heavy) || (bn128_plain && !heavy))) return 1;
        if (wm == 2 && tiles * (d->CDw / 256) < 256 && !any_count) return 1;
    }
    hipStream_t st = reinterpret_cast<hipStream_t>(stream);
    int rc;
#define W3_GO(NT_, MD_) (wm == 2 ? launch3<NT_, MD_, 2>(*d, t, st) : launch3<NT_, MD_, 4>(*d, t, st))
    if (mode == 1) rc = W3_GO(4, 1);
    else if (d->ntaps == 9) rc = W3_GO(9, 0);
    else rc = W3_GO(4, 0);
#undef W3_GO
    return rc == XMC_ESHAPE ? 1 : rc;
}
```

xmc-gan_amd/csrc/pointwise.hip:

```cpp
#include "common.h"
#include <stdlib.h>
#include <string.h>
#include <cstdarg>
#include <cstdio>

namespace {

constexpr int NT = 256;
inline int nblocks(int64_t items, int per_block = NT, int cap = 256 * 16) {
    int64_t b = (items + per_block - 1) / per_block;
    if (b < 1) b = 1;
    return (int)(b > cap ? cap : b);
}

constexpr int UN = 4;
constexpr int STREAM_BLOCKS = 1024;
inline int sblocks(int64_t n8) { return nblocks((n8 + UN - 1) / UN, NT, STREAM_BLOCKS); }

template <int DT, class F>
__global__ void map1_kernel(const void* x, void* y, int64_t n8, F f) {
    for (int64_t base = (int64_t)blockIdx.x * (NT * UN); base < n8; base += (int64_t)gridDim.x * (NT * UN)) {
        float v[UN][8];
#pragma unroll
        for (int j = 0; j < UN; ++j) {
// ... 296 lines not shown
        for (int c = 0; c < C; ++c) v[c] = src[(n * C + c) * HW + p];
        Vec8<DT>::store(dst, i, v);
    }
}
template <int DT>
__global__ void nhwc8_to_nchw_kernel(const void* src, float* dst, int N, int C, int HW) {
    const int64_t total = (int64_t)N * HW;
    for (int64_t i = blockIdx.x * (int64_t)blockDim.x + threadIdx.x; i < total; i += (int64_t)gridDim.x * blockDim.x) {
        int64_t n = i / HW, p = i - n * HW;
        float v[8];
        Vec8<DT>::load(src, i, v);
        for (int c = 0; c < C; ++c) dst[(n * C + c) * HW + p] = v[c];
    }
}

template <int DT>
__global__ void affine2_fwd_kernel(const void* x, const float* g0, const float* b0, const float* g1, const float* b1,
                                   void* y, int HW, int C8, int pix_per_block, float slope) {
    const int n = blockIdx.y, groups = NT / C8;
    const int cc = threadIdx.x % C8, g = threadIdx.x / C8;
    if (g >= groups) return;
    float G0[8], B0[8], G1[8], B1[8];
    const size_t pb = ((size_t)n * C8 + cc) * 8;
    const bool two = g1 != nullptr;
#pragma unroll
    for (int k = 0; k < 8; ++k) { G0[k] = g0[pb + k]; B0[k] = b0[pb + k]; G1[k] = two ? g1[pb + k] : 1.f; B1[k] = two ? b1[pb + k] : 0.f; }
    const int p_end = min(HW, (int)(blockIdx.x + 1) * pix_per_block);
    for (int p = blockIdx.x * pix_per_block + g; p < p_end; p += groups) {
        float v[8];
        const size_t idx = ((size_t)n * HW + p) * C8 + cc;
        Vec8<DT>::load(x, idx, v);
#pragma unroll
        for (int k = 0; k < 8; ++k) {
            float u = v[k] * G0[k] + B0[k];
            u = u > 0.f ? u : slope * u;
            const float t = u * G1[k] + B1[k];
            v[k] = two ? (t > 0.f ? t : slope * t) : u;
        }
        Vec8<DT>::store(y, idx, v);
    }
}
template <int DT, bool POOL>
__global__ __launch_bounds__(NT, 2) void affine2_bwd_kernel(
                                   const void* x, const void* dy, const float* g0, const float* b0, const float* g1,
                                   const float* b1, void* dx, float* dg0, float* db0, float* dg1, float* db1,
                                   int HW, int C8, int pix_per_block, float slope, const void* dx_in,
                                   const float* alpha_dev, float* dot, void* dx_pool, int Wq) {
    const float al = alpha_dev ? *alpha_dev : 1.f;
    float dacc = 0.f;
    const int n = blockIdx.y, groups = NT / C8;
    const int cc = threadIdx.x % C8, g = threadIdx.x / C8;
    float G0[8], B0[8], G1[8], B1[8];
    float sg0[8], sb0[8], sg1[8], sb1[8];
    const size_t pb = ((size_t)n * C8 + cc) * 8;
    const bool two = g1 != nullptr;
#pragma unroll
    for (int k = 0; k < 8; ++k) {
        G0[k] = g0[pb + k]; B0[k] = b0[pb + k]; G1[k] = two ? g1[pb + k] : 1.f; B1[k] = two ? b1[pb + k] : 0.f;
        sg0[k] = sb0[k] = sg1[k] = sb1[k] = 0.f;
    }
    auto pixel = [&](size_t idx, float (&xv)[8], const float (&dv)[8], const float (&o)[8], float* acc8) {
#pragma unroll
        for (int k = 0; k < 8; ++k) {
            float u = xv[k] * G0[k] + B0[k];
            float a1 = u > 0.f ? u : slope * u;
            float v = a1 * G1[k] + B1[k];
            if (dot) {
                const float y2 = two ? (v > 0.f ? v : slope * v) : a1;
                dacc += dv[k] * (DT == XMC_BF16 ? (float)(xmc_h16)y2 : y2);
            }
// ... 786 lines not shown
```

xmc-gan_amd/lib.py:

```python
import ctypes as C
import os

HERE = os.path.dirname(os.path.abspath(__file__))
LIB_PATH = os.environ.get("XMC_LIB_PATH", os.path.join(HERE, "libxmc_gan_hip.so"))
LIB_PATH_F16 = os.environ.get("XMC_LIB_PATH_F16", os.path.join(HERE, "libxmc_gan_hip_f16.so"))
ABI_VERSION = 12

BF16, F32 = 0, 1
H16 = BF16
ACT_NONE, ACT_LRELU, ACT_TANH, ACT_RELU = 0, 1, 2, 3
MAX_TAPS, MAX_CLASSES = 16, 4
POOL_MAX, POOL_AVG_VALID = 0, 1
DIFFAUG_PARTS = 64

vp, i32, i64, f32 = C.c_void_p, C.c_int32, C.c_int64, C.c_float


class ConvDesc(C.Structure):
    _fields_ = [("src", vp), ("wpk", vp), ("dst", vp), ("bias", vp), ("res", vp), ("alpha_dev", vp),
                ("N", i32), ("SH", i32), ("SW", i32), ("CS", i32),
                ("DH", i32), ("DW", i32), ("CD", i32),
                ("MH", i32), ("MW", i32), ("SA", i32), ("DA", i32), ("src_shift", i32),
                ("ntaps", i32), ("nclass", i32), ("CDw", i32), ("act", i32), ("dtype", i32), ("out_dtype", i32),
                ("dh", (C.c_int8 * MAX_TAPS) * MAX_CLASSES), ("dw", (C.c_int8 * MAX_TAPS) * MAX_CLASSES),
                ("wi", (C.c_int8 * MAX_TAPS) * MAX_CLASSES),
                ("dph", C.c_int8 * MAX_CLASSES), ("dpw", C.c_int8 * MAX_CLASSES),
                ("mask", vp), ("res_scale", f32), ("res_mode", i32), ("dst2", vp), ("dst_pool", vp), ("round_act", i32), ("groups", i32),
                ("post_act", i32), ("pool_scale", f32), ("sign_bits", vp), ("dot", vp), ("mask_bits", vp), ("sc_img", vp), ("sc_frag", vp), ("sc_bias", vp),
                ("splitk_ws", vp), ("splitk_ws_bytes", C.c_int64), ("wpk_lo", vp)]


GEMM_PROBLEM = [("A", "u8"), ("B", "u8"), ("bias", "u8"), ("mask", "u8"), ("C", "u8"), ("rowsum", "u8"),
                ("M", "i4"), ("N", "i4"), ("K", "i4"), ("sa_i", "i4"), ("sa_r", "i4"), ("sb_j", "i4"), ("sb_r", "i4"),
                ("flags", "i4"), ("tile0", "i4"), ("reserved", "i4")]
GP_BIAS, GP_RELU, GP_MASK, GP_ATOMIC = 1, 2, 4, 8


class PackJob(C.Structure):
    _fields_ = [("w", vp), ("wpk", vp), ("row_perm", vp), ("Co", i32), ("Ci", i32), ("KHW", i32), ("rows_pad", i32),
                ("cols_pad", i32), ("transpose", i32), ("dtype", i32), ("groups", i32), ("upconv", i32), ("lo", i32)]


class AdamEntry(C.Structure):
    _fields_ = [("param", vp), ("grad", vp), ("m", vp), ("v", vp), ("step", vp), ("n", i64)]


class EmaEntry(C.Structure):
    _fields_ = [("shadow", vp), ("param", vp), ("n", i64)]


_SIGS = {
    "xmc_abi_version": [],
    "xmc_half_format": [],
    "xmc_last_kernel": [],
    "xmc_set_fixed_order": [i32],
    "xmc_set_prezeroed": [i32],
    "xmc_conv_splitk_ws_bytes": [vp],
    "xmc_conv_igemm": [C.POINTER(ConvDesc), vp],
    "xmc_conv_wgrad": [C.POINTER(ConvDesc), vp, vp],
    "xmc_conv_wgrad_bias": [C.POINTER(ConvDesc), vp, vp, vp],
    "xmc_pack_weight": [vp, vp, i32, i32, i32, i32, i32, i32, i32, i32, vp, vp],
    "xmc_pack_weight_grouped": [vp, vp, i32, i32, i32, i32, i32, i32, i32, i32, vp, i32, vp],
    "xmc_pack_weight_upconv": [vp, vp, i32, i32, i32, i32, i32, i32, vp],
    "xmc_pack_weight_multi": [C.POINTER(PackJob), i32, vp],
    "xmc_axpby_up": [vp, vp, vp, vp, i32, i32, i32, i32, i32, vp],
    "xmc_unpack_wgrad": [vp, vp, i32, i32, i32, i32, i32, i32, vp, vp, i32, vp],
    "xmc_unpack_wgrad_grouped": [vp, vp, i32, i32, i32, i32, i32, i32, vp, vp, i32, i32, vp],
    "xmc_unpack_wgrad_bias": [vp, vp, i32, i32, i32, i32, i32, i32, vp, vp, i32, vp, vp, i32, vp],
    "xmc_unpack_wgrad_bias_dot": [vp, vp, i32, i32, i32, i32, i32, i32, vp, vp, i32, vp, vp, i32, vp, vp, vp],
    "xmc_nchw_to_nhwc8": [vp, vp, i32, i32, i32, i32, i32, vp],
    "xmc_nhwc8_to_nchw": [vp, vp, i32, i32, i32, i32, i32, vp],
    "xmc_lrelu": [vp, vp, i64, f32, i32, vp],
    "xmc_lrelu_mask": [vp, vp, vp, i64, f32, i32, vp],
    "xmc_tanh": [vp, vp, i64, i32, vp],
    "xmc_signmask_apply": [vp, vp, vp, i64, f32, i32, vp],
    "xmc_conv_pw1x1_masked_src": [C.POINTER(ConvDesc), vp, vp, f32, vp],
    "xmc_conv_pw1x1_split": [C.POINTER(ConvDesc), vp],
    "xmc_conv_ptile_bits": [C.POINTER(ConvDesc), vp],
    "xmc_conv_ptile_scimg": [C.POINTER(ConvDesc), vp],
    "xmc_conv_wgrad_bits": [C.POINTER(ConvDesc), vp, vp],
    "xmc_tanh_bwd": [vp, vp, vp, i64, i32, vp],
    "xmc_axpby": [vp, vp, vp, vp, i64, i32, vp],
    "xmc_scale_mask_dot": [vp, vp, vp, vp, vp, i64, i32, vp],
    "xmc_axpby_bwd": [vp, vp, vp, vp, vp, vp, i32, i32, i32, i32, i32, vp, i32, vp],
    "xmc_axpby_up_lrelu": [vp, vp, vp, vp, i32, i32, i32, i32, i32, vp],
    "xmc_scale": [vp, vp, vp, i64, i32, vp],
    "xmc_dot": [vp, vp, vp, i64, i32, vp],
    "xmc_gemm_group": [vp, i32, vp],
    "xmc_embedding_gather": [vp, vp, vp, i64, i32, i64, vp],
    "xmc_lstm_bidir": [vp, vp, vp, vp, vp, i32, i32, i32, vp],
    "xmc_gru_bidir": [vp, vp, vp, vp, vp, vp, i32, i32, i32, vp],
# ... 139 lines not shown
```

xmc-gan_amd/ops/_engine.py:

```python
import ctypes as C
import weakref
import torch
from .. import lib as L
from .. import prof
from ._config import (
    _DEBUG_DISPATCH, _code, _nbytes, _need_cuda, _p, _st, _weights_epoch, bump_weights_epoch, chan_pad, pad_to)


class ConvGeom:

    __slots__ = ("cin", "cout", "k", "s", "p", "row_perm", "_perm_dev", "groups", "kh", "kw", "ph", "pw")

    def __init__(self, cin, cout, k=1, s=1, p=0, row_perm=None, groups=1):
        self.kh, self.kw = k if isinstance(k, (tuple, list)) else (k, k)
        self.ph, self.pw = p if isinstance(p, (tuple, list)) else (p, p)
        assert self.kh >= 1 and self.kw >= 1 and self.kh * self.kw <= 127 and s >= 1
        assert cin % groups == 0 and cout % groups == 0
        self.cin, self.cout, self.s = cin, cout, s
        self.k = self.kh if self.kh == self.kw else None
        self.p = self.ph if self.ph == self.pw else None
        self.groups = groups
        self.row_perm = row_perm
        self._perm_dev = None

    @property
    def ntaps(self):
        return self.kh * self.kw

    def out_hw(self, h, w):
        return (h + 2 * self.ph - self.kh) // self.s + 1, (w + 2 * self.pw - self.kw) // self.s + 1

    def taps(self):
        return [(i - self.ph, j - self.pw, i * self.kw + j) for i in range(self.kh) for j in range(self.kw)]

    def perm_dev(self, device):
        if self.row_perm is None:
            return None
        if self._perm_dev is None or self._perm_dev.device != device:
            self._perm_dev = torch.as_tensor(self.row_perm, dtype=torch.int32, device=device).contiguous()
        return self._perm_dev


def _igemm(d, what):
    lib = L.load()
    nb = lib.xmc_conv_splitk_ws_bytes(C.byref(d))
    if nb > 0:
        ws = torch.empty(nb, dtype=torch.uint8, device=torch.cuda.current_device())
        d.splitk_ws, d.splitk_ws_bytes = ws.data_ptr(), nb
    L.check(lib.xmc_conv_igemm(C.byref(d), _st()), what)


def _fill_taps(d, cls, taps):
    for t, (dh, dw, wi) in enumerate(taps):
        d.dh[cls][t] = dh
        d.dw[cls][t] = dw
        d.wi[cls][t] = wi


_pack_cache = {}


class _PackEntry:
    __slots__ = ("ref", "version", "pepoch", "gepoch", "geom", "out", "up", "transpose", "wf", "private", "born", "lo")

    def valid(self, w, geom):
        return (self.ref() is w and self.version == w._version and self.pepoch == getattr(w, "_xmc_epoch", 0) and
                self.gepoch == _weights_epoch[0] and self.geom is geom)


def _pack_shape(geom, transpose, dtype, up):
    cs_p = chan_pad(geom.cin, dtype)
    cd_p = pad_to(geom.cout, 8)
    rows, cols = (pad_to(cs_p, 32), cd_p) if transpose else (pad_to(cd_p, 32), cs_p)
    return (16 if up else geom.ntaps), rows, cols


def _pack_job(wf, out, geom, transpose, up, lo=False):
    j = L.PackJob()
    j.lo = int(bool(lo))
    j.w, j.wpk = wf.data_ptr(), out.data_ptr()
    perm = None if up else geom.perm_dev(wf.device)
    j.row_perm = perm.data_ptr() if perm is not None else None
# ... 77 lines not shown
def repack_params(params):
    ids = {id(p): p for p in params}
    jobs, ents = [], []
    for k in [k for k, e in _pack_cache.items() if e.ref() is None]:
        if _graphs_alive[0]:
            _retired_packs.append(_pack_cache[k].out)
        del _pack_cache[k]
    for (pid, _up, _tr, _dt), e in _pack_cache.items():
        w = ids.get(pid)
        if w is None or e.ref() is not w or e.wf is None or e.gepoch != _weights_epoch[0] or e.version != w._version:
            continue
        if e.wf.data_ptr() != w.data_ptr():
            continue
        jobs.append(_pack_job(e.wf, e.out, e.geom, e.transpose, e.up, e.lo))
        ents.append((e, w))
    if not jobs:
        return 0
    arr = (L.PackJob * len(jobs))(*jobs)
    L.check(L.load().xmc_pack_weight_multi(arr, len(jobs), _st()), "xmc_pack_weight_multi")
    for e, w in ents:
        e.pepoch = getattr(w, "_xmc_epoch", 0)
    return len(jobs)


def _cast_raw(x, dtype):
    if x.dtype == dtype:
        return x
    x = x.contiguous()
    y = torch.empty_like(x, dtype=dtype)
    L.call("xmc_cast", _p(x), _p(y), x.numel(), _code(x.dtype), _code(dtype), _st())
    return y


def _upconv_fwd_raw(x, w, bias, geom, act, out_dtype):
    _need_cuda(x, w)
    assert geom.k == 3 and geom.s == 1 and geom.p == 1
    N, H, W, CS = x.shape
    cd_p = pad_to(geom.cout, 8)
    wpk = _packed_upconv_cached(w, geom, 0, x.dtype)
    y = torch.empty((N, 2 * H, 2 * W, cd_p), dtype=out_dtype, device=x.device)
    d = L.ConvDesc()
    d.src, d.wpk, d.dst = x.data_ptr(), wpk.data_ptr(), y.data_ptr()
    d.bias = bias.data_ptr() if bias is not None else None
    d.N, d.SH, d.SW, d.CS = N, H, W, CS
    d.DH, d.DW, d.CD = 2 * H, 2 * W, cd_p
    d.MH, d.MW, d.SA, d.DA, d.src_shift = H, W, 1, 2, 0
    d.ntaps, d.nclass, d.CDw = 4, 4, wpk.shape[1]
    d.act, d.dtype, d.out_dtype = act, _code(x.dtype), _code(out_dtype)
    for i in range(2):
        for j in range(2):
            cls = i * 2 + j
            _fill_taps(d, cls, [(i - 1 + th, j - 1 + tw, cls * 4 + th * 2 + tw) for th in range(2) for tw in range(2)])
            d.dph[cls], d.dpw[cls] = i, j
    with prof.launch("igemm_kernel (conv fwd+dgrad, MFMA implicit GEMM)", 2.0 * N * 4 * H * W * geom.cout * geom.cin * 9,
                     f"upconv-fwd {x.dtype} N{N} {2 * H}x{2 * W} {geom.cin}->{geom.cout} k3s1", _nbytes(x, wpk, y)):
        _igemm(d, "xmc_conv_igemm(upconv fwd)")
    return y


def _upconv_dgrad_raw(dy, w, geom, in_dtype):
    _need_cuda(dy, w)
    N, OH, OW, CDy = dy.shape
    H, W = OH // 2, OW // 2
    cs_p = chan_pad(geom.cin, in_dtype)
    wpk = _packed_upconv_cached(w, geom, 1, dy.dtype)
    dx = torch.empty((N, H, W, cs_p), dtype=in_dtype, device=dy.device)
    d = L.ConvDesc()
    d.src, d.wpk, d.dst = dy.data_ptr(), wpk.data_ptr(), dx.data_ptr()
    d.N, d.SH, d.SW, d.CS = N, OH, OW, CDy
    d.DH, d.DW, d.CD = H, W, cs_p
    d.MH, d.MW, d.SA, d.DA, d.src_shift = H, W, 2, 1, 0
    d.ntaps, d.nclass, d.CDw = 16, 1, wpk.shape[1]
    d.act, d.dtype, d.out_dtype = L.ACT_NONE, _code(dy.dtype), _code(in_dtype)
    taps = []
    for i in range(2):
        for th in range(2):
            ro = i - 2 * (i - 1 + th)
            for j in range(2):
                for tw in range(2):
                    co = j - 2 * (j - 1 + tw)
                    taps.append((ro, co, (i * 2 + j) * 4 + th * 2 + tw))
    _fill_taps(d, 0, taps)
    with prof.launch("igemm_kernel (conv fwd+dgrad, MFMA implicit GEMM)", 2.0 * N * OH * OW * geom.cout * geom.cin * 9,
                     f"upconv-dgrad {dy.dtype} N{N} {OH}x{OW} {geom.cin}->{geom.cout} k3s1", _nbytes(dy, wpk, dx)):
        _igemm(d, "xmc_conv_igemm(upconv dgrad)")
    return dx


def _conv_fwd_raw(x, w, bias, geom, act, out_dtype, res=None, alpha=None, up=False, res_mode=0, want2=False, want_pool=False,
                  round_act=False, mask=None, out=None, post_act=L.ACT_NONE, want_sign=False, sc_img=None, w_lo=False, taps=None):
    _need_cuda(x, w)
    table = geom.taps() if taps is None else geom.taps()[taps[0]:taps[1]]
    assert 1 <= len(table) <= L.MAX_TAPS, (geom.kh, geom.kw, taps)
    N, H, W, CS = x.shape
    sh = 1 if up else 0
    Hv, Wv = H << sh, W << sh
    OH, OW = geom.out_hw(Hv, Wv)
    cd_p = pad_to(geom.cout, 8)
    assert CS == chan_pad(geom.cin, x.dtype), (CS, geom.cin)
    wpk = _packed_cached(w, geom, 0, x.dtype, lo=w_lo)
    if out is None:
        y = torch.empty((N, OH, OW, cd_p), dtype=out_dtype, device=x.device)
    else:
        assert tuple(out.shape) == (N, OH, OW, cd_p) and out.dtype == out_dtype and out.is_contiguous() and out.device == x.device
        y = out
    d = L.ConvDesc()
    d.src, d.wpk, d.dst = x.data_ptr(), wpk.data_ptr(), y.data_ptr()
    d.bias = bias.data_ptr() if bias is not None else None
    d.res = res.data_ptr() if res is not None else None
    d.alpha_dev = alpha.data_ptr() if alpha is not None else None
    d.N, d.SH, d.SW, d.CS = N, H, W, CS
    d.DH, d.DW, d.CD = OH, OW, cd_p
    d.MH, d.MW, d.SA, d.DA, d.src_shift = OH, OW, geom.s, 1, sh
    d.ntaps, d.nclass, d.CDw = len(table), 1, wpk.shape[1]
    d.act, d.dtype, d.out_dtype = act, _code(x.dtype), _code(out_dtype)
    d.res_mode, d.round_act = res_mode, int(bool(round_act))
    d.groups = geom.groups
    d.post_act = post_act
    _fill_taps(d, 0, table)
    if bias is not None:
        assert bias.dtype == torch.float32 and bias.numel() >= cd_p, "bias must be f32 and padded to the stored channels"
    if res is not None:
        want = (N, OH // 2, OW // 2, cd_p) if res_mode == 2 else tuple(y.shape)
        assert tuple(res.shape) == want and res.dtype == out_dtype and res.is_contiguous(), (res.shape, want)
    if mask is not None:
        assert mask.shape == y.shape and mask.dtype == out_dtype and mask.is_contiguous()
        d.mask = mask.data_ptr()
    outs = [y]
    if want2:
        y2 = torch.empty_like(y)
        d.dst2 = y2.data_ptr()
        outs.append(y2)
    if want_sign:
        assert not want2
        bits = torch.empty((N, OH, OW, cd_p // 8), dtype=torch.uint8, device=x.device)
        d.sign_bits = bits.data_ptr()
        outs.append(bits)
    if want_pool:
        assert OH % 2 == 0 and OW % 2 == 0 and out_dtype == x.dtype
        yp = torch.empty((N, OH // 2, OW // 2, cd_p), dtype=out_dtype, device=x.device)
        d.dst_pool = yp.data_ptr()
        outs.append(yp)
    if sc_img is not None:
        img, frag, sbias = sc_img
        assert res is None and tuple(img.shape) == (N, 2 * OH, 2 * OW, 8) and img.dtype == x.dtype and img.is_contiguous()
        d.sc_img, d.sc_frag, d.sc_bias = img.data_ptr(), frag.data_ptr(), sbias.data_ptr()
        with prof.launch("igemm_kernel (conv fwd+dgrad, MFMA implicit GEMM)", 2.0 * N * OH * OW * geom.cout * (geom.cin * geom.k * geom.k + 48),
                         f"fwd+sc {x.dtype} N{N} {H}x{W} {geom.cin}->{geom.cout} k{geom.k}s{geom.s}", _nbytes(x, wpk, img, *outs)):
            rc = L.load().xmc_conv_ptile_scimg(C.byref(d), _st())
        if rc == 1:
            return None
        L.check(rc, "xmc_conv_ptile_scimg")
        return y if len(outs) == 1 else tuple(outs)
    with prof.launch("igemm_kernel (conv fwd+dgrad, MFMA implicit GEMM)", 2.0 * N * OH * OW * geom.cout * geom.cin * len(table),
                     f"fwd {x.dtype} N{N} {H}x{W} {geom.cin}->{geom.cout} k{geom.k or f'{geom.kh}x{geom.kw}'}s{geom.s}", _nbytes(x, wpk, res, mask, *outs)):
        _igemm(d, "xmc_conv_igemm(fwd)")
    return y if len(outs) == 1 else tuple(outs)


def _conv1x1_pair_raw(x, w, bias, geom, out_dtype):
    _need_cuda(x, w)
    assert geom.k == 1 and geom.s == 1 and geom.p == 0 and geom.groups == 1
    N, H, W, CS = x.shape
    cd_p = pad_to(geom.cout, 8)
    if "no_pw1x1_split" not in _DEBUG_DISPATCH:
        wpk, wlo = _packed_cached(w, geom, 0, x.dtype), _packed_cached(w, geom, 0, x.dtype, lo=True)
        y = torch.empty((N, H, W, cd_p), dtype=out_dtype, device=x.device)
        d = L.ConvDesc()
        d.src, d.wpk, d.wpk_lo, d.dst = x.data_ptr(), wpk.data_ptr(), wlo.data_ptr(), y.data_ptr()
        d.bias = bias.data_ptr() if bias is not None else None
        d.N, d.SH, d.SW, d.CS = N, H, W, CS
        d.DH, d.DW, d.CD = H, W, cd_p
        d.MH, d.MW, d.SA, d.DA, d.src_shift = H, W, 1, 1, 0
        d.ntaps, d.nclass, d.CDw = 1, 1, wpk.shape[1]
        d.act, d.dtype, d.out_dtype = L.ACT_NONE, _code(x.dtype), _code(out_dtype)
        _fill_taps(d, 0, [(0, 0, 0)])
        with prof.launch("igemm_kernel (conv fwd+dgrad, MFMA implicit GEMM)", 2.0 * N * H * W * geom.cout * geom.cin,
                         f"fwd-pair {x.dtype} N{N} {H}x{W} {geom.cin}->{geom.cout} k1s1", _nbytes(x, wpk, wlo, y)):
            rc = L.load().xmc_conv_pw1x1_split(C.byref(d), _st())
        if rc == 0:
            return y
        if rc != 1:
            L.check(rc, "xmc_conv_pw1x1_split")
    y32 = _conv_fwd_raw(_cast_raw(x, torch.float32), w, bias, geom, L.ACT_NONE, torch.float32)
    return _cast_raw(y32, out_dtype)


class _StagedMask:

# ... 399 lines not shown
```

xmc-gan_amd/ops/_functional.py:

```python
import torch
from ._config import act_dtype
from ._nodes_leaf import AxpbyFn, AxpbyUpFn, CastFn, DiffAugFn, GapFn, LreluFn, NchwToNhwc8Fn, Nhwc8ToNchwFn, SumPool2Fn, Up2Fn
from ._nodes_conv import UpConvFn
from ._nodes_block import Affine2LreluFn, AttnPoolFn, GroupNormFn
from ._nodes_loss import ContrastiveFn, HingeFn


def lrelu(x, slope=0.2):
    return LreluFn.apply(x, slope)


def avgpool2(x):
    return SumPool2Fn.apply(x, 0.25)


def upsample2(x):
    return Up2Fn.apply(x, 1.0)


def axpby(a, b, alpha):
    return AxpbyFn.apply(a, b, alpha)


def global_avgpool(x, out_dtype=torch.float32):
    return GapFn.apply(x, out_dtype)


def to_nhwc8(x_nchw, out=None):
    return NchwToNhwc8Fn.apply(x_nchw, act_dtype(), out)


def to_nchw(x_nhwc8, c):
    return Nhwc8ToNchwFn.apply(x_nhwc8, c)


def affine2_lrelu(x, g0, b0, g1, b1):
    return Affine2LreluFn.apply(x, g0, b0, g1, b1)


def upconv3x3(x_lo, w, b, geom):
    return UpConvFn.apply(x_lo, w, b, geom)


def axpby_up(a_lo, b_hi, alpha, lrelu=False):
    return AxpbyUpFn.apply(a_lo, b_hi, alpha, lrelu)


def affine_lrelu(x, g, b):
    return Affine2LreluFn.apply(x, g, b, None, None)


def affine_act(x, g, b, slope):
    return Affine2LreluFn.apply(x, g, b, None, None, slope)


def groupnorm(x, w, b, groups, slope=-1.0, eps=1e-5):
    return GroupNormFn.apply(x, w, b, groups, slope, eps)


def attn_pool(key, q, x, ncon, scale=1.0):
    return AttnPoolFn.apply(key, q, x, ncon, scale)


def hinge(logits_padded, sign):
    return HingeFn.apply(logits_padded, sign)


def contrastive(a, b, labels=None, inv_num_pos=None):
    return ContrastiveFn.apply(a, b, labels, inv_num_pos)


def cast(x, dtype):
    return CastFn.apply(x, dtype)

# ... 4 lines not shown
```

xmc-gan_amd/ops/_nodes_block.py:

```python
import torch
from .. import lib as L
from ._config import _DEBUG_DISPATCH, _code, _need_cuda, _p, _second_order, _skip_wgrad, _st, precise_trunk
from ._engine import (
    _StagedMask, _affine_bwd_raw, _affine_fwd_raw, _conv1x1_pair_raw, _conv_dgrad_raw, _conv_fwd_raw, _conv_wgrad_raw,
    _dstem_border_fwd_raw, _dstem_compose_bwd_raw, _dstem_compose_raw, _dstem_dgrad_raw, _dstem_fwd_raw, _dstem_sc_operands,
    _dstem_wgrad_raw, _pooled_put, _zeros_f32, _zeros_f32_out)
from ._nodes_leaf import CastFn
from ._nodes_conv import _bias_padded


class ResDFn(torch.autograd.Function):

    @staticmethod
    def forward(ctx, x, w0, w2, ws, bs, gamma, g0, g2, gs, xp_hint=None, want_pool=False):
        x = x.contiguous()
        dt = x.dtype
        N, H, W, _ = x.shape
        xp32 = None
        if xp_hint is not None and xp_hint.dtype == torch.float32 and dt != torch.float32:
            xp32 = xp_hint
            xp = None
        elif xp_hint is not None:
            xp = xp_hint
        else:
# ... 354 lines not shown
    @staticmethod
    @torch.autograd.function.once_differentiable
    def backward(ctx, dy):
        x, *ps = ctx.saved_tensors
        dx, red = _affine_bwd_raw(x, dy.contiguous(), ps, ctx.slope)
        if ctx.two:
            return dx, red[0], red[1], red[2], red[3], None
        return dx, red[0], red[1], None, None, None


def _gn_fwd_raw(x, wf, bf, groups, slope, eps):
    N, H, W, Cc = x.shape
    y = torch.empty_like(x)
    stats = torch.empty((N, groups, 2), dtype=torch.float32, device=x.device)
    ws = _zeros_f32((N, Cc, 2), x.device)
    L.call("xmc_groupnorm_fwd", _p(x), _p(wf), _p(bf), _p(y), _p(stats), _p(ws), N, H * W, Cc, groups, float(eps),
           float(slope), _code(x.dtype), _st())
    return y, stats


def _gn_bwd_raw(x, dy, wf, bf, stats, groups, slope):
    N, H, W, Cc = x.shape
    dx = torch.empty_like(x)
    dw, db = torch.empty_like(wf), torch.empty_like(bf)
    ws = _zeros_f32(N * Cc * 2 + N * groups * 2, x.device)
    L.call("xmc_groupnorm_bwd", _p(x), _p(dy), _p(wf), _p(bf), _p(stats), _p(dx), _p(dw), _p(db), _p(ws), N, H * W, Cc,
           groups, float(slope), _code(x.dtype), _st())
    return dx, dw, db


class Affine2LreluSkipFn(torch.autograd.Function):

    @staticmethod
    def forward(ctx, x, g0, b0, g1, b1, pool_grad=False):
        x = x.contiguous()
        ps = [t.contiguous().float() for t in (g0, b0, g1, b1)]
        y = _affine_fwd_raw(x, ps, 0.2)
        ctx.set_materialize_grads(False)
        ctx.pool = bool(pool_grad)
        ctx.save_for_backward(x, *ps)
        return y, x.view_as(x)

    @staticmethod
    @torch.autograd.function.once_differentiable
    def backward(ctx, dy, dskip):
        x, *ps = ctx.saved_tensors
        if dy is None:
            return dskip, None, None, None, None, None
        if ctx.pool and x.shape[1] % 2 == 0 and x.shape[2] % 2 == 0 and x.shape[3] // 8 in (1, 2, 4, 8, 16, 32):
            dx, red, dxp = _affine_bwd_raw(x, dy.contiguous(), ps, 0.2, dx_acc=dskip, want_sumpool=True)
            _pooled_put(dx, dxp)
        else:
            dx, red = _affine_bwd_raw(x, dy.contiguous(), ps, 0.2, dx_acc=dskip)
        return dx, red[0], red[1], red[2], red[3], None


def affine2_lrelu_skip(x, g0, b0, g1, b1, pool_grad=False):
    return Affine2LreluSkipFn.apply(x, g0, b0, g1, b1, pool_grad)


class GroupNormFn(torch.autograd.Function):

    @staticmethod
    def forward(ctx, x, w, b, groups, slope, eps):
        x = x.contiguous()
        wf, bf = w.detach().float().contiguous(), b.detach().float().contiguous()
        y, stats = _gn_fwd_raw(x, wf, bf, groups, slope, eps)
        ctx.groups, ctx.slope = groups, slope
        ctx.save_for_backward(x, wf, bf, stats)
        return y

    @staticmethod
    @torch.autograd.function.once_differentiable
    def backward(ctx, dy):
        x, wf, bf, stats = ctx.saved_tensors
        dx, dw, db = _gn_bwd_raw(x, dy.contiguous(), wf, bf, stats, ctx.groups, ctx.slope)
        return dx, dw, db, None, None, None


class BatchNormTrainFn(torch.autograd.Function):

    @staticmethod
    def forward(ctx, x, w, b, eps):
        x = x.contiguous()
        N, H, W, Cc = x.shape
        wf, bf = w.detach().float().contiguous(), b.detach().float().contiguous()
        y = torch.empty_like(x)
        stats = torch.empty((1, Cc, 2), dtype=torch.float32, device=x.device)
        ws = _zeros_f32((1, Cc, 2), x.device)
        L.call("xmc_groupnorm_fwd", _p(x), _p(wf), _p(bf), _p(y), _p(stats), _p(ws), 1, N * H * W, Cc, Cc, float(eps), -1.0,
               _code(x.dtype), _st())
# ... 96 lines not shown
```

xmc-gan_amd/ops/_nodes_conv.py:

```python
import ctypes as C
import numpy as np
import torch
from .. import lib as L
from ._config import _code, _p, _skip_wgrad, _st, act_dtype, pad_to
from ._engine import (
    _affine_bwd_raw, _affine_fwd_raw, _axpby_bwd_fused, _conv1x1_pair_raw, _conv_dgrad_raw, _conv_fwd_raw, _conv_wgrad_raw,
    _pooled_take, _upconv_dgrad_raw, _upconv_fwd_raw, _zeros_f32, _zeros_f32_out)
from ._nodes_leaf import CastFn, ColSumFn, MaskFn, TanhBwdFn


def _bias_padded(b, geom, permute=False):
    if b is None:
        return None
    bp = b.detach().float()
    if permute and geom.row_perm is not None:
        bp = bp.index_select(0, geom.perm_dev(b.device).long())
    cd_p = pad_to(geom.cout, 8)
    if bp.numel() < cd_p:
        bp = torch.nn.functional.pad(bp, (0, cd_p - bp.numel()))
    return bp.contiguous()


def _act_bwd(dy, y, act, dtype):
    dy = dy.contiguous()
# ... 123 lines not shown
        if ctx.needs_input_grad[1] and not _skip_wgrad():
            dw = ConvWgradFn.apply(g, dy, geom).view(w.shape)
        return ddy, dw, None, None, None


class ConvWgradFn(torch.autograd.Function):

    @staticmethod
    def forward(ctx, x, dy, geom, want_bias=False):
        x, dy = x.contiguous(), dy.contiguous()
        r = _conv_wgrad_raw(x, dy, geom, want_bias=want_bias)
        ctx.geom = geom
        ctx.save_for_backward(x, dy)
        if want_bias:
            ctx.mark_non_differentiable(r[1])
        return r

    @staticmethod
    def backward(ctx, ggw, _ggb=None):
        x, dy = ctx.saved_tensors
        geom = ctx.geom
        ggw = ggw.contiguous().view(geom.cout, geom.cin // geom.groups, geom.k, geom.k)
        dx = ddy = None
        if ctx.needs_input_grad[0]:
            dx = ConvDgradFn.apply(dy, ggw, geom, (x.shape[1], x.shape[2]), x.dtype)
        if ctx.needs_input_grad[1]:
            ddy = ConvFn.apply(x, ggw, None, geom, L.ACT_NONE, dy.dtype)
        return dx, ddy, None, None


class UpConvFn(torch.autograd.Function):

    @staticmethod
    def forward(ctx, x, w, b, geom):
        x = x.contiguous()
        y = _upconv_fwd_raw(x, w, _bias_padded(b, geom), geom, L.ACT_NONE, x.dtype)
        ctx.geom, ctx.has_b = geom, b is not None
        ctx.save_for_backward(x, w)
        return y

    @staticmethod
    @torch.autograd.function.once_differentiable
    def backward(ctx, dy):
        x, w = ctx.saved_tensors
        geom = ctx.geom
        dy = dy.contiguous()
        dx = _upconv_dgrad_raw(dy, w, geom, x.dtype) if ctx.needs_input_grad[0] else None
        dw, db = _wgrad_bias_raw(ctx, x, dy, w, geom, up=True)
        return dx, dw, db, None


class ConvAxpbyUpFn(torch.autograd.Function):

    @staticmethod
    def forward(ctx, h, w, b, geom, sc_lo, gamma):
        h, sc_lo = h.contiguous(), sc_lo.contiguous()
        bp = _bias_padded(b, geom)
        al = gamma.detach().reshape(-1).float()
        y, res = _conv_fwd_raw(h, w, bp, geom, L.ACT_NONE, h.dtype, res=sc_lo, alpha=al, res_mode=2, want2=True)
        ctx.geom, ctx.has_b = geom, b is not None
        ctx.save_for_backward(h, w, res, gamma)
        return y

    @staticmethod
    @torch.autograd.function.once_differentiable
    def backward(ctx, dy):
        h, w, res, gamma = ctx.saved_tensors
        geom = ctx.geom
        dy = dy.contiguous()
        al = gamma.detach().reshape(-1).float()
        dsc, _, dgamma = _axpby_bwd_fused(dy, res, gamma, up=True, want_db=False)
        dh = _conv_dgrad_raw(dy, w, geom, (h.shape[1], h.shape[2]), h.dtype, alpha=al) if ctx.needs_input_grad[0] else None
        dw, db = _wgrad_bias_raw(ctx, h, dy, w, geom, scale=al)
        return dh, dw, db, None, (dsc if ctx.needs_input_grad[4] else None), (dgamma if ctx.needs_input_grad[5] else None)


def conv_axpby_up(h, w, b, geom, sc_lo, gamma):
    return ConvAxpbyUpFn.apply(h, w, b, geom, sc_lo, gamma)


class GBlockEndFn(torch.autograd.Function):

    @staticmethod
    def forward(ctx, h1, g0, b0, g1, b1, w2, b2, geom2, sc_lo, gamma, w_out=None, b_out=None, geom_out=None, nhwc_dst=None):
        h1, sc_lo = h1.contiguous(), sc_lo.contiguous()
        ps = [t.contiguous().float() for t in (g0, b0, g1, b1)]
        h2 = _affine_fwd_raw(h1, ps, 0.2)
        al = gamma.detach().reshape(-1).float()
        tail = w_out is not None
        y = _conv_fwd_raw(h2, w2, _bias_padded(b2, geom2), geom2, L.ACT_NONE, h2.dtype, res=sc_lo, alpha=al, res_mode=2,
                          round_act=True, post_act=L.ACT_LRELU if tail else L.ACT_NONE)
        img = None
        if tail:
            assert nhwc_dst is None or nhwc_dst._version == 0, "GBlockEndFn(nhwc_dst=): the destination must be a fresh tensor"
            img = _conv_fwd_raw(y, w_out, _bias_padded(b_out, geom_out), geom_out, L.ACT_TANH, y.dtype, out=nhwc_dst)
        ctx.geom2, ctx.geom_out, ctx.tail = geom2, geom_out, tail
        ctx.has_b2, ctx.has_bo = b2 is not None, b_out is not None
        ctx.save_for_backward(h1, *ps, h2, w2, b2, gamma, y if tail else None, w_out, img)
        return img if tail else y

    @staticmethod
    @torch.autograd.function.once_differentiable
    def backward(ctx, dy):
        h1, g0, b0, g1, b1, h2, w2, b2, gamma, y, w_out, img = ctx.saved_tensors
        geom2, geom_out = ctx.geom2, ctx.geom_out
        dt = h1.dtype
        N, H, W, _ = h2.shape
        dy = dy.contiguous()
        if dy.dtype != dt:
            dy = dy.to(dt)
        skip_w = _skip_wgrad()
        dw_out = db_out = None
        if ctx.tail:
            dpre = torch.empty_like(dy)
            L.call("xmc_tanh_bwd", _p(dy), _p(img), _p(dpre), dy.numel(), _code(dt), _st())
            if not skip_w:
                r = _conv_wgrad_raw(y, dpre, geom_out, want_bias=ctx.has_bo)
                dw_out, db_out = r if ctx.has_bo else (r, None)
                dw_out = dw_out.view(w_out.shape)
                if db_out is not None:
                    db_out = db_out[: geom_out.cout]
            dz, dsc = _conv_dgrad_raw(dpre, w_out, geom_out, (H, W), dt, mask=y, want_sumpool=True)
        else:
            dz = dy
            dsc = _pooled_take(dz)
            if dsc is None:
                dsc = torch.empty((N, H // 2, W // 2, dz.shape[3]), dtype=dt, device=dz.device)
                L.call("xmc_sumpool2", _p(dz), _p(dsc), N, H, W, dz.shape[3], 1.0, _code(dt), _st())
        al = gamma.detach().reshape(-1).float()
        dot = _zeros_f32_out(1, dz.device)
        dw2 = db2 = None
        if ctx.has_b2:
            bdot = _bias_padded(b2, geom2)
            dw2, db2 = _conv_wgrad_raw(h2, dz, geom2, scale=al, want_bias=True, bias_dot=bdot, dot=dot)
            dw2, db2 = dw2.view(w2.shape), db2[: geom2.cout]
        elif not skip_w:
            dw2 = _conv_wgrad_raw(h2, dz, geom2, scale=al).view(w2.shape)
        dh2u = _conv_dgrad_raw(dz, w2, geom2, (H, W), dt)
        dh1, red = _affine_bwd_raw(h1, dh2u, (g0, b0, g1, b1), 0.2, alpha=al, dot=dot)
        dgamma = dot.reshape(gamma.shape).to(gamma.dtype)
        if skip_w:
            dw2 = db2 = None
        return (dh1, red[0], red[1], red[2], red[3], dw2, db2, None, dsc, dgamma, dw_out, db_out, None, None)


def g_block_end(h1, mod4, c2w, c2b, geom2, sc_lo, gamma, tail=None, nhwc_dst=None):
    if tail is None:
        return GBlockEndFn.apply(h1, *mod4, c2w, c2b, geom2, sc_lo, gamma)
    return GBlockEndFn.apply(h1, *mod4, c2w, c2b, geom2, sc_lo, gamma, tail[0], tail[1], tail[2], nhwc_dst)


def conv2d(x, w, b, geom, act=L.ACT_NONE, out_dtype=None, want_pool=False, out=None, pair=False):
    return ConvFn.apply(x, w, b, geom, act, out_dtype or x.dtype, want_pool, out, pair)


def linear(x, w, b, geom, act=L.ACT_NONE, out_dtype=None):
    y = ConvFn.apply(x.contiguous().view(x.shape[0], 1, 1, x.shape[1]), w, b, geom, act, out_dtype or x.dtype)
    return y.view(x.shape[0], -1)


def _gemm_group(tab):
    L.call("xmc_gemm_group", C.c_void_p(tab.ctypes.data), len(tab), _st())


def _offsets(sizes):
    off = np.zeros(len(sizes) + 1, dtype=np.int64)
    np.cumsum(sizes, out=off[1:])
    return off


class CondMLPBankFn(torch.autograd.Function):

    @staticmethod
    def forward(ctx, c, *params):
        assert len(params) % 4 == 0 and c.dtype == torch.float32 and c.is_cuda
        c = c.contiguous()
        G = len(params) // 4
        w1, b1, w2, b2 = params[0::4], params[1::4], params[2::4], params[3::4]
        B, K = c.shape
        Hd = w1[0].shape[0]
        for g in range(G):
            assert w1[g].shape == (Hd, K) and w2[g].shape[1] == Hd and w1[g].is_contiguous() and w2[g].is_contiguous()
# ... 239 lines not shown
```

xmc_gan/model/df_gan.py:

```python
from collections import OrderedDict

import torch
import torch.nn as nn

from xmc_gan_amd import ops
from xmc_gan_amd.lib import ACT_LRELU, ACT_NONE, ACT_RELU, ACT_TANH

from .modules import HipConv2d, HipLinear, as_nchw_view, as_nhwc, conv2d_nxn, linear


def gen_arch(img_size, nch):
    assert img_size in [64, 128, 256]
    depth = {64: 5, 128: 6, 256: 7}[img_size]
    mult = [8] * (depth - 2) + [4, 2, 1]
    return {
        'in_channels': [m * nch for m in mult[:-1]],
        'out_channels': [m * nch for m in mult[1:]],
        'upsample': [True] * (depth - 1) + [False],
        'resolution': [8 << i for i in range(depth - 1)] + [img_size],
        'depth': depth,
    }


def disc_arch(img_size, nch):
# ... 28 lines not shown
        self.proj_sent = HipLinear(cfg.TEXT.EMBEDDING_DIM, cfg.TRAIN.NEF) \
            if (cfg.TEXT.EMBEDDING_DIM != cfg.TRAIN.NEF) else nn.Identity()
        self.upblocks = nn.ModuleList(
            [G_Block(in_dim=arch['in_channels'][i], out_dim=arch['out_channels'][i],
                     cond_dim=cfg.TRAIN.NEF, upsample=arch['upsample'][i]) for i in range(arch['depth'])])
        self.conv_out = nn.Sequential(
            nn.LeakyReLU(0.2, inplace=True),
            HipConv2d(arch['out_channels'][-1], 3, 3, 1, 1),
            nn.Tanh(),
        )

    def stem(self, noise):
        out = self.proj_noise(noise.float(), out_dtype=ops.act_dtype())
        return out.view(noise.size(0), 4, 4, 8 * self.ngf)

    nhwc_dst_ok = True

    def tail(self, out, lrelu_done=False, return_nhwc=False, nhwc_dst=None):
        if not lrelu_done:
            out = ops.lrelu(out)
        out = self.conv_out[1](out, act=ACT_TANH, out=nhwc_dst)
        img = ops.to_nchw(out, 3)
        return (img, out) if return_nhwc else img

    def forward(self, noise, sent_embs, return_nhwc=False, nhwc_dst=None, **kwargs):
        out = self.stem(noise)
        sent_embs = self.proj_sent(sent_embs.float())
        nblk = len(self.upblocks)
        flat = ops.cond_mlp_bank(sent_embs, [m for g in self.upblocks for m in g.modulation_mlps()])
        mods = [flat[8 * i:8 * i + 8] for i in range(nblk)]
        pending_up = False
        lrelu_done = False
        from_end = False
        for bi, (gblock, m) in enumerate(zip(self.upblocks, mods)):
            last = bi == nblk - 1 and not gblock.upsample
            fuse = gblock.fuses_end(out, pending_up)
            if last and fuse:
                co = self.conv_out[1]
                out8 = gblock.forward_fused(out, m, pending_up, out_lrelu=True, tail=(co.weight, co.bias, co.geom), nhwc_dst=nhwc_dst,
                                            x_from_end=from_end)
                img = ops.to_nchw(out8, 3)
                return (img, out8) if return_nhwc else img
            out = gblock.forward_fused(out, m, pending_up, out_lrelu=last, x_from_end=from_end)
            from_end = fuse and not last
            lrelu_done = last
            pending_up = gblock.upsample
        if pending_up:
            out = ops.upsample2(out)
        return self.tail(out, lrelu_done, return_nhwc, nhwc_dst)


class NetD(nn.Module):
    def __init__(self, cfg, **kwargs):
        super(NetD, self).__init__()
        ndf = cfg.TRAIN.NCH
        spec_norm = cfg.DISC.SPEC_NORM
        arch = disc_arch(img_size=cfg.IMG.SIZE, nch=ndf)
        self.conv_img = conv2d_nxn(in_dim=arch['in_channels'][0], out_dim=arch['out_channels'][0], kernel_size=3,
                                   stride=1, padding=1, spec_norm=spec_norm)
        self.downblocks = nn.ModuleList(
            [resD(in_dim=arch['in_channels'][i], out_dim=arch['out_channels'][i],
                  downsample=arch['downsample'][i], spec_norm=spec_norm) for i in range(1, arch['depth'])])
        self.COND_DNET = D_GET_LOGITS(cfg, ndf=ndf, spec_norm=spec_norm)

    def forward(self, x, nhwc8=None, **kwargs):
        pooled = None
        xin = ops.to_nhwc8(x) if nhwc8 is None else nhwc8
        src = x if nhwc8 is None else nhwc8
        leaf_in = torch.is_tensor(src) and src.requires_grad and src.is_leaf
        with ops.second_order(leaf_in or ops.second_order_active()):
            nblk = len(self.downblocks)
            b0 = self.downblocks[0]
            first = 0
            sink, cut = self.cut_sink, self.cut_block()
            if (ops.fused_blocks() and not self.conv_img.spec_norm and b0.downsample
                    and not (ops.second_order_active() and ops.debug_switch("no_dstem2"))
# ... 87 lines not shown
        super(G_Block, self).__init__()
        self.learnable_sc = (in_dim != out_dim)
        self.upsample = upsample
        self.c1 = HipConv2d(in_dim, out_dim, 3, 1, 1)
        self.c2 = HipConv2d(out_dim, out_dim, 3, 1, 1)
        self.affine0 = affine(num_features=in_dim, cond_dim=cond_dim)
        self.affine1 = affine(num_features=in_dim, cond_dim=cond_dim)
        self.affine2 = affine(num_features=out_dim, cond_dim=cond_dim)
        self.affine3 = affine(num_features=out_dim, cond_dim=cond_dim)
        self.gamma = nn.Parameter(torch.zeros(1))
        if self.learnable_sc:
            self.c_sc = HipConv2d(in_dim, out_dim, 1, stride=1, padding=0)

    def modulation_mlps(self):
        out = []
        for a in (self.affine0, self.affine1, self.affine2, self.affine3):
            for m in (a.fc_gamma, a.fc_beta):
                out.append((m.linear1.weight, m.linear1.bias, m.linear2.weight, m.linear2.bias))
        return out

    def modulation(self, c):
        return (*self.affine0.scale_shift(c), *self.affine1.scale_shift(c),
                *self.affine2.scale_shift(c), *self.affine3.scale_shift(c))

    def forward(self, x, c, mod=None):
        out = ops.axpby(self.shortcut(x), self.residual(x, c, mod), self.gamma)
        if self.upsample:
            out = ops.upsample2(out)
        return out

    def fuses_end(self, x, x_pending_up):
        return bool(x_pending_up) and ops.fused_blocks() and x.is_cuda

    def forward_fused(self, x, mod, x_pending_up, out_lrelu=False, tail=None, nhwc_dst=None, x_from_end=False):
        if not x_pending_up:
            out = ops.axpby(self.shortcut(x), self.residual(x, None, mod), self.gamma)
            return ops.lrelu(out) if out_lrelu else out
        h, xs = ops.affine2_lrelu_skip(x, *mod[0:4], pool_grad=x_from_end) if x.is_cuda else (ops.affine2_lrelu(x, *mod[0:4]), x)
        h = ops.upconv3x3(h, self.c1.weight, self.c1.bias, self.c1.geom)
        if self.fuses_end(x, x_pending_up) and (tail is not None or not out_lrelu):
            return ops.g_block_end(h, mod[4:8], self.c2.weight, self.c2.bias, self.c2.geom, self.shortcut(xs), self.gamma,
                                   tail=tail, nhwc_dst=nhwc_dst)
        assert tail is None
        h = ops.affine2_lrelu(h, *mod[4:8])
        if not out_lrelu and ops.fused_blocks() and h.shape[1] % 2 == 0:
            return ops.conv_axpby_up(h, self.c2.weight, self.c2.bias, self.c2.geom, self.shortcut(xs), self.gamma)
        return ops.axpby_up(self.shortcut(xs), self.c2(h), self.gamma, lrelu=out_lrelu)

    def shortcut(self, x):
        return self.c_sc(x, pair=ops.precise_trunk()) if self.learnable_sc else x

    def residual(self, x, c, mod=None):
        m = self.modulation(c) if mod is None else mod
        h = ops.affine2_lrelu(x, *m[0:4])
        h = self.c1(h)
        h = ops.affine2_lrelu(h, *m[4:8])
        return self.c2(h)


class _CondMLP(nn.Module):

    def __init__(self, cond_dim, num_features):
        super().__init__()
        self.linear1 = HipLinear(cond_dim, 256)
        self.relu1 = nn.ReLU(inplace=True)
        self.linear2 = HipLinear(256, num_features)

    def forward(self, y):
        return self.linear2(self.linear1(y, act=ACT_RELU))


class affine(nn.Module):
    def __init__(self, num_features, cond_dim):
        super(affine, self).__init__()
        self.fc_gamma = _CondMLP(cond_dim, num_features)
        self.fc_beta = _CondMLP(cond_dim, num_features)
# ... 54 lines not shown
```

Measured before the change: 5949 images/s.

## Fuse affine2+LeakyReLU into conv epilogues for generator blocks

Adds a second output to the implicit-GEMM and tile conv kernels that applies the double affine modulation plus LeakyReLU in the epilogue and writes the activated tensor alongside the raw conv output. The generator uses it for the upconv's following affine and for the next block's first affine, which skips separate elementwise passes over large activations. The cost is an extra bf16 store and parameter loads per epilogue item, plus more register pressure in those kernels. Large non-resident sites fall back to the unfused path by heuristic.

```diff
diff --git a/include/xmc_gan_hip.h b/include/xmc_gan_hip.h
--- a/include/xmc_gan_hip.h
+++ b/include/xmc_gan_hip.h
@@ -68,6 +68,16 @@
 int64_t xmc_conv_splitk_ws_bytes(const XmcConvDesc* d);
 
 int xmc_conv_igemm(const XmcConvDesc* d, void* stream);
+
+typedef struct XmcAffOut {
+    void* dst;
+    const float* g0;
+    const float* b0;
+    const float* g1;
+    const float* b1;
+    float slope;
+} XmcAffOut;
+int xmc_conv_igemm_aff(const XmcConvDesc* d, const XmcAffOut* a, void* stream);
 
 int xmc_conv_wgrad(const XmcConvDesc* d , float* dwp, void* stream);
 #define XMC_BIAS_REPLICAS 16
diff --git a/xmc-gan_amd/csrc/common.h b/xmc-gan_amd/csrc/common.h
--- a/xmc-gan_amd/csrc/common.h
+++ b/xmc-gan_amd/csrc/common.h
@@ -134,8 +134,33 @@
     return v;
 }
 
+__device__ __forceinline__ float xmc_affine_act(float x, float g, float b, float slope) {
+    const float u = __builtin_fmaf(x, g, b);
+    return u > 0.f ? u : slope * u;
+}
+__device__ __forceinline__ float xmc_affine2_act(float x, float g0, float b0, float g1, float b1, float slope) {
+    return xmc_affine_act(xmc_affine_act(x, g0, b0, slope), g1, b1, slope);
+}
+struct XmcAffRegs { f32x4 g0[2], b0[2], g1[2], b1[2]; };
+__device__ __forceinline__ void xmc_aff_load(const XmcAffOut& a, int off, XmcAffRegs& p) {
+#pragma unroll
+    for (int h = 0; h < 2; ++h) {
+        p.g0[h] = *reinterpret_cast<const f32x4*>(a.g0 + off + 4 * h); p.b0[h] = *reinterpret_cast<const f32x4*>(a.b0 + off + 4 * h);
+        p.g1[h] = *reinterpret_cast<const f32x4*>(a.g1 + off + 4 * h); p.b1[h] = *reinterpret_cast<const f32x4*>(a.b1 + off + 4 * h);
+    }
+}
+__device__ __forceinline__ bf16x8 xmc_aff_unit(const bf16x8 r, const XmcAffRegs& p, float slope) {
+    bf16x8 o;
+#pragma unroll
+    for (int k = 0; k < 8; ++k) o[k] = (xmc_h16)xmc_affine2_act((float)r[k], p.g0[k >> 2][k & 3], p.b0[k >> 2][k & 3], p.g1[k >> 2][k & 3], p.b1[k >> 2][k & 3], slope);
+    return o;
+}
+__device__ __forceinline__ const XmcAffOut* xmc_aff_arg() { return nullptr; }
+__device__ __forceinline__ const XmcAffOut* xmc_aff_arg(const XmcAffOut& a) { return &a; }
+
 template <int ODT>
-__device__ __forceinline__ void epilogue_tail(const XmcConvDesc& d, size_t idx8, size_t ridx8, float (&v)[8], float alpha, float* dacc = nullptr) {
+__device__ __forceinline__ void epilogue_tail(const XmcConvDesc& d, size_t idx8, size_t ridx8, float (&v)[8], float alpha, float* dacc = nullptr,
+                                              const XmcAffOut* aff = nullptr, int aff_off = 0) {
     if (d.sign_bits) {
         unsigned b = 0;
 #pragma unroll
@@ -175,10 +200,19 @@
         for (int k = 0; k < 8; ++k) v[k] = lrelu_f(v[k]);
     }
     Vec8<ODT>::store(d.dst, idx8, v);
+    if (ODT == XMC_BF16 && aff) {
+        bf16x8 r;
+#pragma unroll
+        for (int k = 0; k < 8; ++k) r[k] = (xmc_h16)v[k];
+        XmcAffRegs p;
+        xmc_aff_load(*aff, aff_off, p);
+        reinterpret_cast<bf16x8*>(aff->dst)[idx8] = xmc_aff_unit(r, p, aff->slope);
+    }
 }
 
 constexpr int kEpiBias = 1, kEpiLrelu = 2, kEpiRound = 4, kEpiDst2 = 8, kEpiAlpha = 16, kEpiMask = 32, kEpiRes = 64, kEpiPost = 128, kEpiPool = 256,
-              kEpiSign = 512, kEpiDot = 1024, kEpiScImg = 2048;
+              kEpiSign = 512, kEpiDot = 1024, kEpiScImg = 2048,
+              kEpiAff = 4096;
 constexpr int kEpiGSum = kEpiBias | kEpiRound | kEpiAlpha | kEpiRes;
 constexpr int kEpiDKeep = kEpiLrelu | kEpiDst2 | kEpiAlpha | kEpiRes | kEpiPool;
 constexpr int kEpiDFwd = kEpiLrelu | kEpiRound | kEpiAlpha | kEpiRes | kEpiPool;
diff --git a/xmc-gan_amd/csrc/conv_igemm.hip b/xmc-gan_amd/csrc/conv_igemm.hip
--- a/xmc-gan_amd/csrc/conv_igemm.hip
+++ b/xmc-gan_amd/csrc/conv_igemm.hip
@@ -38,7 +38,8 @@
 };
 
 template <int ODT>
-__device__ __forceinline__ void igemm_epi_item(const XmcConvDesc& d, int cls, int m, int ch, float (&v)[8], float alpha, float* dacc) {
+__device__ __forceinline__ void igemm_epi_item(const XmcConvDesc& d, int cls, int m, int ch, float (&v)[8], float alpha, float* dacc,
+                                               const XmcAffOut* aff = nullptr) {
     const int MHW = d.MH * d.MW;
     const int n = m / MHW, rem = m - n * MHW;
     const int a = rem / d.MW, b = rem - a * d.MW;
@@ -60,11 +61,12 @@
         for (int k = 0; k < 8; ++k) v[k] = tanhf(v[k]);
     }
     const size_t ridx8 = res_index8(d, idx8, n, a * d.DA + dph, b * d.DA + dpw, a, b, ch >> 3);
-    epilogue_tail<ODT>(d, idx8, ridx8, v, alpha, dacc);
-}
-
-template <int DT, int BM, int BN, int WM, int WN, int KSUB, bool SK = false>
-__global__ __launch_bounds__(64 * WM * WN) void igemm_kernel(const XmcConvDesc d) {
+    epilogue_tail<ODT>(d, idx8, ridx8, v, alpha, dacc, aff, n * d.CD + ch);
+}
+
+template <int DT, int BM, int BN, int WM, int WN, int KSUB, bool SK = false, class... AFF>
+__global__ __launch_bounds__(64 * WM * WN) void igemm_kernel(const XmcConvDesc d, const AFF... aff) {
+    static_assert(sizeof...(AFF) == 0 || (DT == XMC_BF16 && !SK), "affine output: 16-bit launches, not the partial sums of a split one");
     constexpr int NT = 64 * WM * WN;
     static_assert(WM * WN == 4 || WM * WN == 8, "4 or 8 waves");
     constexpr int RP = NT / 4;
@@ -248,7 +250,7 @@
             float v[8];
 #pragma unroll
             for (int k = 0; k < 4; ++k) { v[k] = e0[k]; v[4 + k] = e1[k]; }
-            if (d.out_dtype == XMC_BF16) igemm_epi_item<XMC_BF16>(d, cls, m, ch, v, alpha, &dacc);
+            if (d.out_dtype == XMC_BF16) igemm_epi_item<XMC_BF16>(d, cls, m, ch, v, alpha, &dacc, xmc_aff_arg(aff...));
             else igemm_epi_item<XMC_F32>(d, cls, m, ch, v, alpha, &dacc);
         }
     }
@@ -260,7 +262,8 @@
 }
 
 constexpr int SK_FIN_ITEMS = 4;
-__global__ __launch_bounds__(256) void igemm_splitk_finish_kernel(const XmcConvDesc d, int S) {
+template <class... AFF>
+__global__ __launch_bounds__(256) void igemm_splitk_finish_kernel(const XmcConvDesc d, int S, const AFF... aff) {
     const int cls = blockIdx.z;
     const int M = d.N * d.MH * d.MW, C8 = d.CD / 8;
     const float alpha = d.alpha_dev ? *d.alpha_dev : 1.f;
@@ -277,7 +280,7 @@
 #pragma unroll
             for (int k = 0; k < 4; ++k) { v[k] += e0[k]; v[4 + k] += e1[k]; }
         }
-        if (d.out_dtype == XMC_BF16) igemm_epi_item<XMC_BF16>(d, cls, m, ch, v, alpha, &dacc);
+        if (d.out_dtype == XMC_BF16) igemm_epi_item<XMC_BF16>(d, cls, m, ch, v, alpha, &dacc, xmc_aff_arg(aff...));
         else igemm_epi_item<XMC_F32>(d, cls, m, ch, v, alpha, &dacc);
     }
     if (d.dot) {
@@ -313,7 +316,7 @@
 static int64_t splitk_bytes(const XmcConvDesc& d, int S) { return (int64_t)S * d.nclass * d.N * d.MH * d.MW * d.CDw * 4; }
 
 template <int BM, int BN, int WM, int WN>
-int launch_splitk(const XmcConvDesc& d, int S, hipStream_t st) {
+int launch_splitk(const XmcConvDesc& d, int S, hipStream_t st, const XmcAffOut* aff) {
     const int64_t M = (int64_t)d.N * d.MH * d.MW;
     dim3 grid((unsigned)(((M + BM - 1) / BM) * (d.CDw / BN)), (unsigned)S, (unsigned)d.nclass);
     using Lds = IgemmLds<BM, BN, 2>;
@@ -326,17 +329,32 @@
     xmc_note_kernel("igemm_kernel<%d, %d, %d, %d, %d, %d, true>", XMC_BF16, BM, BN, WM, WN, 2);
     XMC_LAUNCH_CHECK();
     const int64_t items = M * (d.CD / 8);
-    hipLaunchKernelGGL(igemm_splitk_finish_kernel, dim3((unsigned)((items + 256 * SK_FIN_ITEMS - 1) / (256 * SK_FIN_ITEMS)), 1, (unsigned)d.nclass), dim3(256), 0, st, d, S);
+    const dim3 fgrid((unsigned)((items + 256 * SK_FIN_ITEMS - 1) / (256 * SK_FIN_ITEMS)), 1, (unsigned)d.nclass);
+    if (aff) hipLaunchKernelGGL(igemm_splitk_finish_kernel<XmcAffOut>, fgrid, dim3(256), 0, st, d, S, *aff);
+    else hipLaunchKernelGGL(igemm_splitk_finish_kernel<>, fgrid, dim3(256), 0, st, d, S);
     XMC_LAUNCH_CHECK();
     return 0;
 }
 
 template <int DT, int BM, int BN, int WM, int WN, int KSUB>
-int launch(const XmcConvDesc& d, hipStream_t st) {
+int launch(const XmcConvDesc& d, hipStream_t st, const XmcAffOut* aff) {
     const int64_t M = (int64_t)d.N * d.MH * d.MW;
     dim3 grid((unsigned)(((M + BM - 1) / BM) * (d.CDw / BN)), 1, (unsigned)d.nclass);
     using Lds = IgemmLds<BM, BN, KSUB>;
     size_t dyn = 0;
+    if constexpr (DT == XMC_BF16) {
+        if (aff) {
+            if (Lds::DYNAMIC) {
+                dyn = (size_t)Lds::SMEM_U * 16;
+                XMC_ALLOW_BIG_LDS((igemm_kernel<DT, BM, BN, WM, WN, KSUB, false, XmcAffOut>));
+            }
+            hipLaunchKernelGGL((igemm_kernel<DT, BM, BN, WM, WN, KSUB, false, XmcAffOut>), grid, dim3(64 * WM * WN), dyn, st, d, *aff);
+            xmc_note_kernel("igemm_kernel<%d, %d, %d, %d, %d, %d, aff>", DT, BM, BN, WM, WN, KSUB);
+            XMC_LAUNCH_CHECK();
+            return 0;
+        }
+    }
+    if (aff) return XMC_EINVAL;
     if (Lds::DYNAMIC) {
         dyn = (size_t)Lds::SMEM_U * 16;
         XMC_ALLOW_BIG_LDS((igemm_kernel<DT, BM, BN, WM, WN, KSUB>));
@@ -348,53 +366,53 @@
 }
 
 template <int DT>
-int dispatch(const XmcConvDesc& d, hipStream_t st) {
+int dispatch(const XmcConvDesc& d, hipStream_t st, const XmcAffOut* aff = nullptr) {
     static const int variant = xmc_debug_off("igemm128") ? 1 : 0;
     static const bool no_small = xmc_debug_off("no_small_m");
     if (DT == XMC_BF16 && d.splitk_ws) {
         const SkPlan sp = splitk_plan(d);
         if (sp.S && d.splitk_ws_bytes >= splitk_bytes(d, sp.S))
-            return sp.big == 1 ? launch_splitk<256, 256, 2, 4>(d, sp.S, st) : sp.big == 0 ? launch_splitk<128, 128, 2, 2>(d, sp.S, st)
-                                                                                             : launch_splitk<128, 64, 4, 1>(d, sp.S, st);
-    }
-    if (!no_small && (int64_t)d.N * d.MH * d.MW <= 1024) return launch<DT, 128, 32, 4, 1, 2>(d, st);
+            return sp.big == 1 ? launch_splitk<256, 256, 2, 4>(d, sp.S, st, aff) : sp.big == 0 ? launch_splitk<128, 128, 2, 2>(d, sp.S, st, aff)
+                                                                                             : launch_splitk<128, 64, 4, 1>(d, sp.S, st, aff);
+    }
+    if (!no_small && (int64_t)d.N * d.MH * d.MW <= 1024) return launch<DT, 128, 32, 4, 1, 2>(d, st, aff);
     if (d.CDw % 128 == 0) {
         const int64_t M = (int64_t)d.N * d.MH * d.MW;
-        if (variant == 1) return launch<DT, 128, 128, 2, 2, 2>(d, st);
+        if (variant == 1) return launch<DT, 128, 128, 2, 2, 2>(d, st, aff);
         static const bool no_big = xmc_debug_off("no_igemm256");
         const int64_t tiles256 = (M + 255) / 256 * (d.CDw / 256) * d.nclass;
-        if (DT == XMC_BF16 && (M >= 256 * 256 || tiles256 >= 256) && d.CDw % 256 == 0 && !no_big) return launch<DT, 256, 256, 2, 4, 2>(d, st);
-        if (DT == XMC_BF16 && M >= 256 * 256) return launch<DT, 256, 128, 2, 2, 1>(d, st);
+        if (DT == XMC_BF16 && (M >= 256 * 256 || tiles256 >= 256) && d.CDw % 256 == 0 && !no_big) return launch<DT, 256, 256, 2, 4, 2>(d, st, aff);
+        if (DT == XMC_BF16 && M >= 256 * 256) return launch<DT, 256, 128, 2, 2, 1>(d, st, aff);
         static const bool no_m64 = xmc_debug_off("no_igemm_m64");
         static const bool no_k4 = xmc_debug_off("no_igemm_ksub4");
         const bool deepk = DT == XMC_BF16 && !no_k4 && (int64_t)d.ntaps * d.CS >= 2048;
         const int64_t t128 = (M + 127) / 128 * (d.CDw / 128) * d.nclass;
         if (DT == XMC_BF16 && !no_m64 && t128 < 256) {
-            if (deepk && (M + 63) / 64 * (d.CDw / 128) * d.nclass <= 256) return launch<DT, 64, 128, 2, 2, 4>(d, st);
-            return launch<DT, 64, 128, 2, 2, 2>(d, st);
-        }
-        if (deepk && t128 <= 256) return launch<DT, 128, 128, 2, 2, 4>(d, st);
-        return launch<DT, 128, 128, 2, 2, 2>(d, st);
+            if (deepk && (M + 63) / 64 * (d.CDw / 128) * d.nclass <= 256) return launch<DT, 64, 128, 2, 2, 4>(d, st, aff);
+            return launch<DT, 64, 128, 2, 2, 2>(d, st, aff);
+        }
+        if (deepk && t128 <= 256) return launch<DT, 128, 128, 2, 2, 4>(d, st, aff);
+        return launch<DT, 128, 128, 2, 2, 2>(d, st, aff);
     }
     if (d.CDw % 64 == 0) {
         static const bool no_k4b = xmc_debug_off("no_igemm_ksub4");
         const int64_t Mb = (int64_t)d.N * d.MH * d.MW;
         if (DT == XMC_BF16 && !no_k4b && (int64_t)d.ntaps * d.CS >= 2048 && (Mb + 127) / 128 * (d.CDw / 64) * d.nclass <= 256)
-            return launch<DT, 128, 64, 4, 1, 4>(d, st);
-        return launch<DT, 128, 64, 4, 1, 2>(d, st);
-    }
-    return launch<DT, 128, 32, 4, 1, 2>(d, st);
-}
-
-}
-
-int xmc_conv_tile_try(const XmcConvDesc* d, void* stream);
+            return launch<DT, 128, 64, 4, 1, 4>(d, st, aff);
+        return launch<DT, 128, 64, 4, 1, 2>(d, st, aff);
+    }
+    return launch<DT, 128, 32, 4, 1, 2>(d, st, aff);
+}
+
+}
+
+int xmc_conv_tile_try(const XmcConvDesc* d, void* stream, const XmcAffOut* aff = nullptr);
 int xmc_conv_thin_try(const XmcConvDesc* d, void* stream);
 int xmc_conv_pw1x1_try(const XmcConvDesc* d, void* stream);
-int xmc_conv_wtile_try(const XmcConvDesc* d, void* stream);
-int xmc_conv_wtile3_try(const XmcConvDesc* d, void* stream);
+int xmc_conv_wtile_try(const XmcConvDesc* d, void* stream, const XmcAffOut* aff = nullptr);
+int xmc_conv_wtile3_try(const XmcConvDesc* d, void* stream, const XmcAffOut* aff = nullptr);
 int xmc_conv_ptile_pool_try(const XmcConvDesc* d, void* stream);
-int xmc_conv_ptile_slab128_try(const XmcConvDesc* d, void* stream);
+int xmc_conv_ptile_slab128_try(const XmcConvDesc* d, void* stream, const XmcAffOut* aff = nullptr);
 int xmc_conv_group_try(const XmcConvDesc* d, void* stream);
 int xmc_conv_thin_out_try(const XmcConvDesc* d, void* stream);
 
@@ -404,7 +422,7 @@
     return sp.S ? splitk_bytes(*d, sp.S) : 0;
 }
 
-extern "C" int xmc_conv_igemm(const XmcConvDesc* d, void* stream) {
+static int igemm_validate(const XmcConvDesc* d) {
     if (!d || !d->src || !d->wpk || !d->dst) return XMC_EINVAL;
     if (d->dtype != XMC_BF16 && d->dtype != XMC_F32) return XMC_EINVAL;
     if (d->out_dtype != XMC_BF16 && d->out_dtype != XMC_F32) return XMC_EINVAL;
@@ -424,6 +442,11 @@
     if (d->sc_img) return XMC_EINVAL;
     if (d->wpk_lo) return XMC_EINVAL;
     if (d->res_mode < 0 || d->res_mode > 2 || (d->res_mode == 2 && (d->DA != 1 || (d->DH & 1) || (d->DW & 1)))) return XMC_ESHAPE;
+    return 0;
+}
+
+extern "C" int xmc_conv_igemm(const XmcConvDesc* d, void* stream) {
+    if (const int bad = igemm_validate(d)) return bad;
     static const bool no_tile = xmc_debug_off("no_tile");
     static const bool no_wt2 = xmc_debug_off("no_wtile_v2");
     static const bool no_wt3 = xmc_debug_off("no_wtile3");
@@ -456,3 +479,34 @@
     if (d->dst_pool) return xmc_sumpool2(d->dst, d->dst_pool, d->N, d->DH, d->DW, d->CD, d->pool_scale == 0.f ? 0.25f : d->pool_scale, d->out_dtype, stream);
     return 0;
 }
+
+extern "C" int xmc_affine2_act_fwd(const void* x, const float* g0, const float* b0, const float* g1, const float* b1,
+                                   void* y, int N, int HW, int C, float slope, int dtype, void* s);
+
+static bool aff_site_unfused(const XmcConvDesc& d) {
+    const bool up_resident = d.ntaps == 4 && d.nclass == 4 && d.DA == 2 && d.CDw <= 64 && d.CS <= 128;
+    return !up_resident && (int64_t)d.N * d.MH * d.MW > 8192;
+}
+
+extern "C" int xmc_conv_igemm_aff(const XmcConvDesc* d, const XmcAffOut* a, void* stream) {
+    if (!a || !a->dst || !a->g0 || !a->b0 || !a->g1 || !a->b1) return XMC_EINVAL;
+    if (const int bad = igemm_validate(d)) return bad;
+    if (d->out_dtype != XMC_BF16 || d->dtype != XMC_BF16) return XMC_EINVAL;
+    if (d->post_act != XMC_ACT_NONE || d->dst_pool || d->sign_bits || d->dot || d->mask_bits || d->sc_img || d->wpk_lo) return XMC_EINVAL;
+    static const bool off = xmc_debug_off("no_aff_epi"), all = xmc_debug_off("aff_epi_all");
+    static const bool no_tile = xmc_debug_off("no_tile"), no_wt2 = xmc_debug_off("no_wtile_v2"), no_wt3 = xmc_debug_off("no_wtile3");
+    int rc = (off || (!all && aff_site_unfused(*d))) ? 2 : 1;
+    if (rc == 1 && !no_tile) {
+        rc = xmc_conv_ptile_slab128_try(d, stream, a);
+        if (rc == 1 && !no_wt3) rc = xmc_conv_wtile3_try(d, stream, a);
+        if (rc == 1 && !no_wt2) rc = xmc_conv_wtile_try(d, stream, a);
+        if (rc == 1) rc = xmc_conv_tile_try(d, stream, a);
+        if (rc <= 0) return rc;
+    }
+    if (rc == 2) {
+        rc = xmc_conv_igemm(d, stream);
+        if (rc != 0) return rc;
+        return xmc_affine2_act_fwd(d->dst, a->g0, a->b0, a->g1, a->b1, a->dst, d->N, d->DH * d->DW, d->CD, a->slope, XMC_BF16, stream);
+    }
+    return dispatch<XMC_BF16>(*d, reinterpret_cast<hipStream_t>(stream), a);
+}
diff --git a/xmc-gan_amd/csrc/conv_tile.hip b/xmc-gan_amd/csrc/conv_tile.hip
--- a/xmc-gan_amd/csrc/conv_tile.hip
+++ b/xmc-gan_amd/csrc/conv_tile.hip
@@ -195,9 +195,13 @@
 }
 
 
-template <int BN, int SLAB, int NTAPS, int MC, int SA = 1, bool M32 = false, int EPI = -1>
-__global__ __launch_bounds__(512) void ptile3_kernel(const XmcConvDesc d, const TileCfg t, int ntiles) {
+template <int BN, int SLAB, int NTAPS, int MC, int SA = 1, bool M32 = false, int EPI = -1, class... AFF>
+__global__ __launch_bounds__(512) void ptile3_kernel(const XmcConvDesc d, const TileCfg t, int ntiles, const AFF... aff) {
     static_assert(!M32 || (SA == 1 && NTAPS > 0), "32x32x16 form: unit stride, unrolled taps");
+    constexpr bool e_aff = sizeof...(AFF) > 0;
+    static_assert(e_aff == (EPI >= 0 && (EPI & kEpiAff) != 0), "the affine output travels with kEpiAff, and only with it");
+    static_assert(!e_aff || M32 || (EPI & ~(kEpiBias | kEpiAff)) == 0, "16x16x32 role: the affine output is written by the bias-only epilogue");
+    const XmcAffOut* const ao = xmc_aff_arg(aff...);
     constexpr int NS = 256;
     constexpr int TM = SA == 1 ? 4 : 2, TN = BN / 16;
     constexpr int cps = SLAB / 8;
@@ -581,6 +585,21 @@
                             }
                         }
                     }
+                    if (e_aff) {
+#pragma unroll
+                        for (int v2 = 0; v2 < 2; ++v2) {
+                            if (n0 + (ub + v2) * 8 >= d.CD) continue;
+                            XmcAffRegs ap;
+                            xmc_aff_load(*ao, img * d.CD + n0 + (ub + v2) * 8, ap);
+#pragma unroll
+                            for (int pb = 0; pb < 2; ++pb) {
+                                bf16x8 o;
+#pragma unroll
+                                for (int r = 0; r < 8; ++r) o[r] = (xmc_h16)fin[pb][v2][r];
+                                reinterpret_cast<bf16x8*>(ao->dst)[(size_t)(eo[pb] + ub + v2)] = xmc_aff_unit(o, ap, ao->slope);
+                            }
+                        }
+                    }
                 }
                 if (e_sign && pack_sign) {
 #pragma unroll
@@ -620,7 +639,7 @@
 #pragma unroll
             for (int c = 0; c < 8; ++c) bias8[u][c] = (d.bias && ch0 + u * 32 < d.CD) ? d.bias[ch0 + u * 32 + c] : 0.f;
         constexpr bool RT = EPI < 0;
-        constexpr int EB = RT ? 0 : (EPI & ~kEpiBias);
+        constexpr int EB = RT ? 0 : (EPI & ~(kEpiBias | kEpiAff));
         const bool fast = RT ? (d.out_dtype == XMC_BF16 && d.res == nullptr && d.mask == nullptr && d.alpha_dev == nullptr && d.dst2 == nullptr &&
                                 d.dst_pool == nullptr && d.post_act == XMC_ACT_NONE && d.sign_bits == nullptr && d.dot == nullptr &&
                                 (d.act == XMC_ACT_NONE || d.act == XMC_ACT_LRELU || d.act == XMC_ACT_TANH))
@@ -741,6 +760,8 @@
 #pragma unroll
                 for (int u = 0; u < UPL; ++u) {
                     if (ch0 + u * 32 >= d.CD) continue;
+                    XmcAffRegs ap;
+                    if (e_aff) xmc_aff_load(*ao, img * d.CD + ch0 + u * 32, ap);
 #pragma unroll
                     for (int i = 0; i < TM; ++i) {
                         bf16x8 o;
@@ -765,6 +786,7 @@
                             }
                         }
                         dst8[eoff[i] + u * 4] = o;
+                        if (e_aff) reinterpret_cast<bf16x8*>(ao->dst)[dbase + eoff[i] + u * 4] = xmc_aff_unit(o, ap, ao->slope);
                     }
                 }
             } else {
@@ -879,7 +901,8 @@
 }
 
 template <int BN>
-int launch_ptile(const XmcConvDesc& d, const TileCfg& t, hipStream_t st) {
+int launch_ptile(const XmcConvDesc& d, const TileCfg& t, hipStream_t st, const XmcAffOut* aff = nullptr) {
+    if (aff && (d.SA != 1 || xmc_debug_off("no_ptile_epi"))) return XMC_ESHAPE;
     if (d.sc_img && !(d.SA == 1 && d.ntaps == 9 && d.nclass == 1 && t.slab == 64 && d.out_dtype == XMC_BF16 && (d.dst_pool || d.sign_bits))) return XMC_ESHAPE;
     int maxpatch = 0;
     for (int z = 0; z < d.nclass; ++z) maxpatch = t.PH[z] * t.PW[z] > maxpatch ? t.PH[z] * t.PW[z] : maxpatch;
@@ -923,6 +946,14 @@
     if (t.slab == 128) {
         if (BN != 64 || d.ntaps != 4 || d.sign_bits || d.dot) return XMC_ESHAPE;
         const int epis = xmc_debug_off("no_ptile_epi") ? -1 : (xmc_epi_mask(d) & ~kEpiBias);
+        if (aff) {
+            if (epis != 0) return XMC_ESHAPE;
+            XMC_ALLOW_BIG_LDS((ptile3_kernel<64, 128, 4, 1, 1, false, kEpiAff, XmcAffOut>));
+            hipLaunchKernelGGL((ptile3_kernel<64, 128, 4, 1, 1, false, kEpiAff, XmcAffOut>), grid, dim3(512), lds, st, d, t, ntiles, *aff);
+            xmc_note_kernel("ptile3_kernel<64, 128, 4, 1, aff>");
+            XMC_LAUNCH_CHECK();
+            return 0;
+        }
 #define XMC_PT3W(E)                                                                                                         \
         if (epis == (E)) {                                                                                                  \
             XMC_ALLOW_BIG_LDS((ptile3_kernel<64, 128, 4, 1, 1, false, (E)>));                                               \
@@ -949,6 +980,14 @@
             if (d.sign_bits || d.dot) return XMC_ESHAPE;
             static const bool no_epim = xmc_debug_off("no_ptile_epi");
             const int epim = no_epim ? -1 : (xmc_epi_mask(d) & ~kEpiBias);
+            if (aff) {
+                if (epim != 0 || t.slab != 64) return XMC_ESHAPE;
+                XMC_ALLOW_BIG_LDS((ptile3_kernel<BN, 64, 4, 4, 1, false, kEpiAff, XmcAffOut>));
+                hipLaunchKernelGGL((ptile3_kernel<BN, 64, 4, 4, 1, false, kEpiAff, XmcAffOut>), gridm, dim3(512), ldsm, st, d, t, ntiles, *aff);
+                xmc_note_kernel("ptile3_kernel<%d, 64, 4, 4, aff>", BN);
+                XMC_LAUNCH_CHECK();
+                return 0;
+            }
 #define XMC_PT3M(SL, E)                                                                                                     \
             if (t.slab == (SL) && epim == (E)) {                                                                            \
                 XMC_ALLOW_BIG_LDS((ptile3_kernel<BN, SL, 4, 4, 1, false, (E)>));                                            \
@@ -971,6 +1010,14 @@
     }
     static const bool no_m32 = xmc_debug_off("no_ptile_m32");
     static const bool m32_all = xmc_debug_off("ptile_m32_all");
+    if (aff) {
+        if (no_m32 || d.ntaps != 9 || t.slab != 64 || d.sc_img || xmc_epi_mask(d) != kEpiGSum) return XMC_ESHAPE;
+        XMC_ALLOW_BIG_LDS((ptile3_kernel<BN, 64, 9, 1, 1, true, kEpiGSum | kEpiAff, XmcAffOut>));
+        hipLaunchKernelGGL((ptile3_kernel<BN, 64, 9, 1, 1, true, kEpiGSum | kEpiAff, XmcAffOut>), grid, dim3(512), lds, st, d, t, ntiles, *aff);
+        xmc_note_kernel("ptile3_kernel<%d, 64, 9, 1, 1, true, aff>", BN);
+        XMC_LAUNCH_CHECK();
+        return 0;
+    }
     if (!no_m32 && d.ntaps == 9 && d.out_dtype == XMC_BF16 && t.slab == 64 &&
         (m32_all || d.res || d.dst2 || d.dst_pool || d.mask || d.sign_bits)) {
         int epi = xmc_epi_mask(d);
@@ -1137,15 +1184,15 @@
     return rc == XMC_ESHAPE ? 1 : rc;
 }
 
-int xmc_conv_ptile_slab128_try(const XmcConvDesc* d, void* stream) {
+int xmc_conv_ptile_slab128_try(const XmcConvDesc* d, void* stream, const XmcAffOut* aff) {
     if (d->CS != 128 || d->CDw != 64 || d->ntaps != 4 || d->nclass != 4 || d->dst_pool || xmc_debug_off("no_ptile")) return 1;
     TileCfg t;
     if (!tile_plan(d, &t) || t.slab != 128) return 1;
-    const int rc = launch_ptile<64>(*d, t, reinterpret_cast<hipStream_t>(stream));
-    return rc == XMC_ESHAPE ? 1 : rc;
+    const int rc = launch_ptile<64>(*d, t, reinterpret_cast<hipStream_t>(stream), aff);
+    return rc == XMC_ESHAPE ? (aff ? 2 : 1) : rc;
 }
 
-int xmc_conv_tile_try(const XmcConvDesc* d, void* stream) {
+int xmc_conv_tile_try(const XmcConvDesc* d, void* stream, const XmcAffOut* aff) {
     TileCfg t;
     if (!tile_plan(d, &t)) return 1;
     if (t.slab == 128) return 1;
@@ -1153,9 +1200,10 @@
     int rc;
     static const bool no_pt = xmc_debug_off("no_ptile");
     if (!no_pt && d->CS <= 64 && t.slab == d->CS && d->CDw <= 64) {
-        rc = d->CDw == 64 ? launch_ptile<64>(*d, t, st) : launch_ptile<32>(*d, t, st);
+        rc = d->CDw == 64 ? launch_ptile<64>(*d, t, st, aff) : launch_ptile<32>(*d, t, st, aff);
         if (rc != XMC_ESHAPE) return rc;
     }
+    if (aff) return 2;
     static const bool no_pt128 = xmc_debug_off("no_ptile_cd128");
     if (!no_pt && !no_pt128 && d->CS == 32 && t.slab == 32 && d->CDw == 128 && d->SA == 1 && d->nclass == 1 && d->ntaps == 9) {
         rc = launch_ptile<64>(*d, t, st);
diff --git a/xmc-gan_amd/csrc/conv_wtile.hip b/xmc-gan_amd/csrc/conv_wtile.hip
--- a/xmc-gan_amd/csrc/conv_wtile.hip
+++ b/xmc-gan_amd/csrc/conv_wtile.hip
@@ -21,8 +21,10 @@
 constexpr int kPStride = 160;
 constexpr int kPIT = 12;
 
-template <int NTAPS, int MODE, int TN, int CW, int EPI = -1>
-__global__ __launch_bounds__(64 * CW + 256) void wtile2_kernel(const XmcConvDesc d, const WtCfg t, int ntiles) {
+template <int NTAPS, int MODE, int TN, int CW, int EPI = -1, class... AFF>
+__global__ __launch_bounds__(64 * CW + 256) void wtile2_kernel(const XmcConvDesc d, const WtCfg t, int ntiles, const AFF... aff) {
+    constexpr bool e_aff = sizeof...(AFF) > 0;
+    static_assert(e_aff == (EPI >= 0 && (EPI & kEpiAff) != 0), "the affine output travels with kEpiAff, and only with it");
     constexpr int BN = 16 * TN, TM = 4, NS = 64 * CW;
     constexpr int TNW = TN * 4 / CW;
     static_assert(CW == 4 || CW == 8, "4 or 8 compute waves");
@@ -256,6 +258,7 @@
             const bf16x8* __restrict__ res8 = reinterpret_cast<const bf16x8*>(d.res);
             bf16x8* __restrict__ dst2_8 = reinterpret_cast<bf16x8*>(d.dst2);
             bf16x8* __restrict__ pool8 = reinterpret_cast<bf16x8*>(d.dst_pool);
+            const XmcAffOut* const ao = xmc_aff_arg(aff...);
             int eo[TM], ro[TM];
 #pragma unroll
             for (int i = 0; i < TM; ++i) {
@@ -280,6 +283,8 @@
 #pragma unroll
                     for (int i = 0; i < TM; ++i) rrv[i] = res8[ro[i] + u * 4];
                 }
+                XmcAffRegs ap;
+                if (e_aff) xmc_aff_load(*ao, img * d.CD + ch0 + u * 32, ap);
 #pragma unroll
                 for (int i = 0; i < TM; ++i) {
                     float v[8];
@@ -334,6 +339,7 @@
                     for (int r = 0; r < 8; ++r) { o[r] = (xmc_h16)v[r]; fin[i][r] = (float)o[r]; }
                     if (!(WT_ABL & 16)) dst8[eo[i] + u * 4] = o;
                     else asm volatile("" :: "v"(o));
+                    if (e_aff) reinterpret_cast<bf16x8*>(ao->dst)[eo[i] + u * 4] = xmc_aff_unit(o, ap, ao->slope);
                 }
                 if (e_pool) {
 #pragma unroll
@@ -472,7 +478,7 @@
 }
 
 template <int NTAPS, int MODE, int TN, int CW>
-int launch(const XmcConvDesc& d, const WtCfg& t, hipStream_t st) {
+int launch(const XmcConvDesc& d, const WtCfg& t, hipStream_t st, const XmcAffOut* aff) {
     constexpr int BN = 16 * TN;
     const size_t lds = (size_t)3 * BN * 128 + 2 * (size_t)t.patch_bytes;
     if (lds > XMC_MAX_DYN_LDS) return XMC_ESHAPE;
@@ -492,6 +498,18 @@
         XMC_LAUNCH_CHECK();                                                                                                                    \
         return 0;                                                                                                                              \
     }
+#define XMC_W2_AFF(E)                                                                                                                          \
+    if (aff && epi == (E)) {                                                                                                                   \
+        XMC_ALLOW_BIG_LDS((wtile2_kernel<NTAPS, MODE, TN, CW, (E) | kEpiAff, XmcAffOut>));                                                     \
+        hipLaunchKernelGGL((wtile2_kernel<NTAPS, MODE, TN, CW, (E) | kEpiAff, XmcAffOut>), dim3((unsigned)gx, (unsigned)ny, (unsigned)d.nclass), dim3(64 * CW + 256), lds, st, \
+                           d, t, ntiles, *aff);                                                                                                \
+        xmc_note_kernel("wtile2_kernel<%d, %d, %d, %d, aff>", NTAPS, MODE, TN, CW);                                                            \
+        XMC_LAUNCH_CHECK();                                                                                                                    \
+        return 0;                                                                                                                              \
+    }
+    if constexpr (CW == 8 && NTAPS == 4 && MODE == 0) { XMC_W2_AFF(kEpiBias) }
+#undef XMC_W2_AFF
+    if (aff) return 2;
     if constexpr (CW == 8 && NTAPS == 9 && TN == 8) {
         XMC_W2_EPI(kEpiGSum) XMC_W2_EPI(kEpiDKeep) XMC_W2_EPI(kEpiDFwd) XMC_W2_EPI(kEpiDLast) XMC_W2_EPI(kEpiMask) XMC_W2_EPI(0) XMC_W2_EPI(kEpiDLin)
         XMC_W2_EPI(kEpiDKeepS) XMC_W2_EPI(kEpiDLastS) XMC_W2_EPI(kEpiDgDot)
@@ -516,14 +534,14 @@
 
 }
 
-int xmc_conv_wtile_try(const XmcConvDesc* d, void* stream) {
+int xmc_conv_wtile_try(const XmcConvDesc* d, void* stream, const XmcAffOut* aff) {
     WtCfg t;
     int mode = 0, tn = 8;
     if (!plan(d, &t, &mode, &tn)) return 1;
     hipStream_t st = reinterpret_cast<hipStream_t>(stream);
     int rc;
     static const bool cw4 = xmc_debug_off("wtile_cw4");
-#define WT_GO(NT_, MD_, TN_) (cw4 ? launch<NT_, MD_, TN_, 4>(*d, t, st) : launch<NT_, MD_, TN_, 8>(*d, t, st))
+#define WT_GO(NT_, MD_, TN_) (cw4 ? launch<NT_, MD_, TN_, 4>(*d, t, st, aff) : launch<NT_, MD_, TN_, 8>(*d, t, st, aff))
     if (mode == 1) rc = tn == 8 ? WT_GO(4, 1, 8) : WT_GO(4, 1, 4);
     else if (d->ntaps == 9) rc = tn == 8 ? WT_GO(9, 0, 8) : WT_GO(9, 0, 4);
     else rc = tn == 8 ? WT_GO(4, 0, 8) : WT_GO(4, 0, 4);
diff --git a/xmc-gan_amd/csrc/conv_wtile3.hip b/xmc-gan_amd/csrc/conv_wtile3.hip
--- a/xmc-gan_amd/csrc/conv_wtile3.hip
+++ b/xmc-gan_amd/csrc/conv_wtile3.hip
@@ -28,8 +28,10 @@
     __builtin_amdgcn_global_load_lds((gptr_t)src, (__attribute__((address_space(3))) void*)dst, 16, 0, 0);
 }
 
-template <int NTAPS, int MODE, int WM, int EPI = -1>
-__global__ __launch_bounds__(512) void wtile3_kernel(const XmcConvDesc d, const W3Cfg t, int ntiles) {
+template <int NTAPS, int MODE, int WM, int EPI = -1, class... AFF>
+__global__ __launch_bounds__(512) void wtile3_kernel(const XmcConvDesc d, const W3Cfg t, int ntiles, const AFF... aff) {
+    constexpr bool e_aff = sizeof...(AFF) > 0;
+    static_assert(e_aff == (EPI >= 0 && (EPI & kEpiAff) != 0), "the affine output travels with kEpiAff, and only with it");
     constexpr int WN = 8 / WM, BN = 64 * WN;
     constexpr int TMW = 16 / WM;
     constexpr int TNW = 4;
@@ -214,14 +216,16 @@
         const bf16x8* __restrict__ res8 = reinterpret_cast<const bf16x8*>(d.res);
         bf16x8* __restrict__ dst2_8 = reinterpret_cast<bf16x8*>(d.dst2);
         bf16x8* __restrict__ pool8 = reinterpret_cast<bf16x8*>(d.dst_pool);
+        const XmcAffOut* const ao = xmc_aff_arg(aff...);
 #pragma unroll
         for (int g = 0; g < TMW / 4; ++g) {
-            int eo[4], ro[4];
+            int eo[4], ro[4], kim[4];
 #pragma unroll
             for (int i = 0; i < 4; ++i) {
                 const int ml = wr * (256 / WM) + (g * 4 + i) * 16 + lane_op;
                 const int ty = ml >> t.log2TW, txt = ml & (t.TW - 1);
                 const int tx = mi ? (txt & 7) : txt, ki = mi ? (txt >> 3) : 0;
+                kim[i] = ki;
                 eo[i] = dbase + ((ty * d.DA) * d.DW + tx * d.DA) * cd8 + ki * dimg + fc;
                 if (d.res_mode == 2)
                     ro[i] = (((img + ki) * (d.DH >> 1) + ((a0 + ty) >> 1)) * (d.DW >> 1) + ((b0 + tx) >> 1)) * cd8 + nw8 + fc;
@@ -241,6 +245,8 @@
 #pragma unroll
                     for (int i = 0; i < 4; ++i) rrv[i] = res8[ro[i] + u * 4];
                 }
+                XmcAffRegs ap;
+                if (e_aff && !mi) xmc_aff_load(*ao, img * d.CD + ch0 + u * 32, ap);
 #pragma unroll
                 for (int i = 0; i < 4; ++i) {
                     float v[8];
@@ -294,6 +300,10 @@
 #pragma unroll
                     for (int r = 0; r < 8; ++r) { o[r] = (xmc_h16)v[r]; fin[i][r] = (float)o[r]; }
                     dst8[eo[i] + u * 4] = o;
+                    if (e_aff) {
+                        if (mi) xmc_aff_load(*ao, (img + kim[i]) * d.CD + ch0 + u * 32, ap);
+                        reinterpret_cast<bf16x8*>(ao->dst)[eo[i] + u * 4] = xmc_aff_unit(o, ap, ao->slope);
+                    }
                 }
                 if (e_pool) {
 #pragma unroll
@@ -498,7 +508,7 @@
 }
 
 template <int NTAPS, int MODE, int WM>
-int launch3(const XmcConvDesc& d, const W3Cfg& t, hipStream_t st) {
+int launch3(const XmcConvDesc& d, const W3Cfg& t, hipStream_t st, const XmcAffOut* aff) {
     constexpr int BN = 64 * (8 / WM), RING = WM == 2 ? 2 : 4;
     const size_t lds = (size_t)RING * BN * 128 + 2 * (size_t)t.patch_bytes + (size_t)(2 * XMC_MAX_TAPS + 64) * sizeof(int);
     if (lds > XMC_MAX_DYN_LDS) return XMC_ESHAPE;
@@ -517,6 +527,17 @@
         XMC_LAUNCH_CHECK();                                                                                                                  \
         return 0;                                                                                                                            \
     }
+#define XMC_W3_AFF(E)                                                                                                                        \
+    if (aff && epi == (E)) {                                                                                                                 \
+        XMC_ALLOW_BIG_LDS((wtile3_kernel<NTAPS, MODE, WM, (E) | kEpiAff, XmcAffOut>));                                                       \
+        hipLaunchKernelGGL((wtile3_kernel<NTAPS, MODE, WM, (E) | kEpiAff, XmcAffOut>), dim3((unsigned)gx, (unsigned)ny, (unsigned)d.nclass), dim3(512), lds, st, d, t, ntiles, *aff); \
+        xmc_note_kernel("wtile3_kernel<%d, %d, %d, aff>", NTAPS, MODE, WM);                                                                  \
+        XMC_LAUNCH_CHECK();                                                                                                                  \
+        return 0;                                                                                                                            \
+    }
+    if constexpr (NTAPS == 9) { XMC_W3_AFF(kEpiGSum) } else if constexpr (MODE == 0) { XMC_W3_AFF(kEpiBias) }
+#undef XMC_W3_AFF
+    if (aff) return 2;
     if constexpr (NTAPS == 9) {
         XMC_W3_EPI(kEpiGSum) XMC_W3_EPI(kEpiDKeep) XMC_W3_EPI(kEpiDFwd) XMC_W3_EPI(kEpiDLast) XMC_W3_EPI(kEpiMask) XMC_W3_EPI(0) XMC_W3_EPI(kEpiDLin)
         XMC_W3_EPI(kEpiDKeepS) XMC_W3_EPI(kEpiDLastS) XMC_W3_EPI(kEpiDgDot)
@@ -537,7 +558,7 @@
 
 }
 
-int xmc_conv_wtile3_try(const XmcConvDesc* d, void* stream) {
+int xmc_conv_wtile3_try(const XmcConvDesc* d, void* stream, const XmcAffOut* aff) {
     W3Cfg t;
     int mode = 0, wm = 2;
     if (!plan3(d, &t, &mode, &wm)) return 1;
@@ -554,7 +575,7 @@
     }
     hipStream_t st = reinterpret_cast<hipStream_t>(stream);
     int rc;
-#define W3_GO(NT_, MD_) (wm == 2 ? launch3<NT_, MD_, 2>(*d, t, st) : launch3<NT_, MD_, 4>(*d, t, st))
+#define W3_GO(NT_, MD_) (wm == 2 ? launch3<NT_, MD_, 2>(*d, t, st, aff) : launch3<NT_, MD_, 4>(*d, t, st, aff))
     if (mode == 1) rc = W3_GO(4, 1);
     else if (d->ntaps == 9) rc = W3_GO(9, 0);
     else rc = W3_GO(4, 0);
diff --git a/xmc-gan_amd/csrc/pointwise.hip b/xmc-gan_amd/csrc/pointwise.hip
--- a/xmc-gan_amd/csrc/pointwise.hip
+++ b/xmc-gan_amd/csrc/pointwise.hip
@@ -352,10 +352,8 @@
         Vec8<DT>::load(x, idx, v);
 #pragma unroll
         for (int k = 0; k < 8; ++k) {
-            float u = v[k] * G0[k] + B0[k];
-            u = u > 0.f ? u : slope * u;
-            const float t = u * G1[k] + B1[k];
-            v[k] = two ? (t > 0.f ? t : slope * t) : u;
+            const float u = xmc_affine_act(v[k], G0[k], B0[k], slope);
+            v[k] = two ? xmc_affine_act(u, G1[k], B1[k], slope) : u;
         }
         Vec8<DT>::store(y, idx, v);
     }
diff --git a/xmc-gan_amd/lib.py b/xmc-gan_amd/lib.py
--- a/xmc-gan_amd/lib.py
+++ b/xmc-gan_amd/lib.py
@@ -30,6 +30,10 @@
                 ("splitk_ws", vp), ("splitk_ws_bytes", C.c_int64), ("wpk_lo", vp)]
 
 
+class AffOut(C.Structure):
+    _fields_ = [("dst", vp), ("g0", vp), ("b0", vp), ("g1", vp), ("b1", vp), ("slope", f32)]
+
+
 GEMM_PROBLEM = [("A", "u8"), ("B", "u8"), ("bias", "u8"), ("mask", "u8"), ("C", "u8"), ("rowsum", "u8"),
                 ("M", "i4"), ("N", "i4"), ("K", "i4"), ("sa_i", "i4"), ("sa_r", "i4"), ("sb_j", "i4"), ("sb_r", "i4"),
                 ("flags", "i4"), ("tile0", "i4"), ("reserved", "i4")]
@@ -57,6 +61,7 @@
     "xmc_set_prezeroed": [i32],
     "xmc_conv_splitk_ws_bytes": [vp],
     "xmc_conv_igemm": [C.POINTER(ConvDesc), vp],
+    "xmc_conv_igemm_aff": [C.POINTER(ConvDesc), C.POINTER(AffOut), vp],
     "xmc_conv_wgrad": [C.POINTER(ConvDesc), vp, vp],
     "xmc_conv_wgrad_bias": [C.POINTER(ConvDesc), vp, vp, vp],
     "xmc_pack_weight": [vp, vp, i32, i32, i32, i32, i32, i32, i32, i32, vp, vp],
diff --git a/xmc-gan_amd/ops/_engine.py b/xmc-gan_amd/ops/_engine.py
--- a/xmc-gan_amd/ops/_engine.py
+++ b/xmc-gan_amd/ops/_engine.py
@@ -48,6 +48,26 @@
         ws = torch.empty(nb, dtype=torch.uint8, device=torch.cuda.current_device())
         d.splitk_ws, d.splitk_ws_bytes = ws.data_ptr(), nb
     L.check(lib.xmc_conv_igemm(C.byref(d), _st()), what)
+
+
+def aff_epilogue():
+    return "no_aff_epi" not in _DEBUG_DISPATCH
+
+
+def _igemm_aff(d, like, ps, what):
+    N, Cc = like.shape[0], like.shape[3]
+    for t in ps:
+        assert t.shape == (N, Cc) and t.dtype == torch.float32 and t.is_contiguous(), (t.shape, (N, Cc))
+    y = torch.empty_like(like)
+    a = L.AffOut()
+    a.dst, a.g0, a.b0, a.g1, a.b1, a.slope = y.data_ptr(), ps[0].data_ptr(), ps[1].data_ptr(), ps[2].data_ptr(), ps[3].data_ptr(), 0.2
+    lib = L.load()
+    nb = lib.xmc_conv_splitk_ws_bytes(C.byref(d))
+    if nb > 0:
+        ws = torch.empty(nb, dtype=torch.uint8, device=torch.cuda.current_device())
+        d.splitk_ws, d.splitk_ws_bytes = ws.data_ptr(), nb
+    L.check(lib.xmc_conv_igemm_aff(C.byref(d), C.byref(a), _st()), what)
+    return y
 
 
 def _fill_taps(d, cls, taps):
@@ -191,7 +211,7 @@
     return y
 
 
-def _upconv_fwd_raw(x, w, bias, geom, act, out_dtype):
+def _upconv_fwd_raw(x, w, bias, geom, act, out_dtype, aff=None):
     _need_cuda(x, w)
     assert geom.k == 3 and geom.s == 1 and geom.p == 1
     N, H, W, CS = x.shape
@@ -212,7 +232,9 @@
             _fill_taps(d, cls, [(i - 1 + th, j - 1 + tw, cls * 4 + th * 2 + tw) for th in range(2) for tw in range(2)])
             d.dph[cls], d.dpw[cls] = i, j
     with prof.launch("igemm_kernel (conv fwd+dgrad, MFMA implicit GEMM)", 2.0 * N * 4 * H * W * geom.cout * geom.cin * 9,
-                     f"upconv-fwd {x.dtype} N{N} {2 * H}x{2 * W} {geom.cin}->{geom.cout} k3s1", _nbytes(x, wpk, y)):
+                     f"upconv-fwd {x.dtype} N{N} {2 * H}x{2 * W} {geom.cin}->{geom.cout} k3s1", _nbytes(x, wpk, y, *([y] if aff else []))):
+        if aff is not None:
+            return y, _igemm_aff(d, y, aff, "xmc_conv_igemm_aff(upconv fwd)")
         _igemm(d, "xmc_conv_igemm(upconv fwd)")
     return y
 
@@ -247,7 +269,7 @@
 
 
 def _conv_fwd_raw(x, w, bias, geom, act, out_dtype, res=None, alpha=None, up=False, res_mode=0, want2=False, want_pool=False,
-                  round_act=False, mask=None, out=None, post_act=L.ACT_NONE, want_sign=False, sc_img=None, w_lo=False, taps=None):
+                  round_act=False, mask=None, out=None, post_act=L.ACT_NONE, want_sign=False, sc_img=None, w_lo=False, taps=None, aff=None):
     _need_cuda(x, w)
     table = geom.taps() if taps is None else geom.taps()[taps[0]:taps[1]]
     assert 1 <= len(table) <= L.MAX_TAPS, (geom.kh, geom.kw, taps)
@@ -312,8 +334,12 @@
         L.check(rc, "xmc_conv_ptile_scimg")
         return y if len(outs) == 1 else tuple(outs)
     with prof.launch("igemm_kernel (conv fwd+dgrad, MFMA implicit GEMM)", 2.0 * N * OH * OW * geom.cout * geom.cin * len(table),
-                     f"fwd {x.dtype} N{N} {H}x{W} {geom.cin}->{geom.cout} k{geom.k or f'{geom.kh}x{geom.kw}'}s{geom.s}", _nbytes(x, wpk, res, mask, *outs)):
-        _igemm(d, "xmc_conv_igemm(fwd)")
+                     f"fwd {x.dtype} N{N} {H}x{W} {geom.cin}->{geom.cout} k{geom.k or f'{geom.kh}x{geom.kw}'}s{geom.s}", _nbytes(x, wpk, res, mask, *outs, *([y] if aff else []))):
+        if aff is not None:
+            assert not (want_sign or want_pool) and post_act == L.ACT_NONE
+            outs.append(_igemm_aff(d, y, aff, "xmc_conv_igemm_aff(fwd)"))
+        else:
+            _igemm(d, "xmc_conv_igemm(fwd)")
     return y if len(outs) == 1 else tuple(outs)
 
 
diff --git a/xmc-gan_amd/ops/_functional.py b/xmc-gan_amd/ops/_functional.py
--- a/xmc-gan_amd/ops/_functional.py
+++ b/xmc-gan_amd/ops/_functional.py
@@ -38,8 +38,10 @@
     return Affine2LreluFn.apply(x, g0, b0, g1, b1)
 
 
-def upconv3x3(x_lo, w, b, geom):
-    return UpConvFn.apply(x_lo, w, b, geom)
+def upconv3x3(x_lo, w, b, geom, aff=None):
+    if aff is None:
+        return UpConvFn.apply(x_lo, w, b, geom)
+    return UpConvFn.apply(x_lo, w, b, geom, *aff)
 
 
 def axpby_up(a_lo, b_hi, alpha, lrelu=False):
diff --git a/xmc-gan_amd/ops/_nodes_block.py b/xmc-gan_amd/ops/_nodes_block.py
--- a/xmc-gan_amd/ops/_nodes_block.py
+++ b/xmc-gan_amd/ops/_nodes_block.py
@@ -410,10 +410,10 @@
 class Affine2LreluSkipFn(torch.autograd.Function):
 
     @staticmethod
-    def forward(ctx, x, g0, b0, g1, b1, pool_grad=False):
+    def forward(ctx, x, g0, b0, g1, b1, pool_grad=False, y_pre=None):
         x = x.contiguous()
         ps = [t.contiguous().float() for t in (g0, b0, g1, b1)]
-        y = _affine_fwd_raw(x, ps, 0.2)
+        y = _affine_fwd_raw(x, ps, 0.2) if y_pre is None else y_pre.view_as(y_pre)
         ctx.set_materialize_grads(False)
         ctx.pool = bool(pool_grad)
         ctx.save_for_backward(x, *ps)
@@ -424,17 +424,17 @@
     def backward(ctx, dy, dskip):
         x, *ps = ctx.saved_tensors
         if dy is None:
-            return dskip, None, None, None, None, None
+            return dskip, None, None, None, None, None, None
         if ctx.pool and x.shape[1] % 2 == 0 and x.shape[2] % 2 == 0 and x.shape[3] // 8 in (1, 2, 4, 8, 16, 32):
             dx, red, dxp = _affine_bwd_raw(x, dy.contiguous(), ps, 0.2, dx_acc=dskip, want_sumpool=True)
             _pooled_put(dx, dxp)
         else:
             dx, red = _affine_bwd_raw(x, dy.contiguous(), ps, 0.2, dx_acc=dskip)
-        return dx, red[0], red[1], red[2], red[3], None
-
-
-def affine2_lrelu_skip(x, g0, b0, g1, b1, pool_grad=False):
-    return Affine2LreluSkipFn.apply(x, g0, b0, g1, b1, pool_grad)
+        return dx, red[0], red[1], red[2], red[3], None, None
+
+
+def affine2_lrelu_skip(x, g0, b0, g1, b1, pool_grad=False, y_pre=None):
+    return Affine2LreluSkipFn.apply(x, g0, b0, g1, b1, pool_grad, y_pre)
 
 
 class GroupNormFn(torch.autograd.Function):
diff --git a/xmc-gan_amd/ops/_nodes_conv.py b/xmc-gan_amd/ops/_nodes_conv.py
--- a/xmc-gan_amd/ops/_nodes_conv.py
+++ b/xmc-gan_amd/ops/_nodes_conv.py
@@ -179,22 +179,29 @@
 class UpConvFn(torch.autograd.Function):
 
     @staticmethod
-    def forward(ctx, x, w, b, geom):
+    def forward(ctx, x, w, b, geom, g0=None, b0=None, g1=None, b1=None):
         x = x.contiguous()
-        y = _upconv_fwd_raw(x, w, _bias_padded(b, geom), geom, L.ACT_NONE, x.dtype)
-        ctx.geom, ctx.has_b = geom, b is not None
+        ctx.geom, ctx.has_b, ctx.aff = geom, b is not None, g0 is not None
         ctx.save_for_backward(x, w)
-        return y
+        if g0 is None:
+            return _upconv_fwd_raw(x, w, _bias_padded(b, geom), geom, L.ACT_NONE, x.dtype)
+        ps = [t.contiguous().float() for t in (g0, b0, g1, b1)]
+        y, h2 = _upconv_fwd_raw(x, w, _bias_padded(b, geom), geom, L.ACT_NONE, x.dtype, aff=ps)
+        ctx.mark_non_differentiable(h2)
+        ctx.set_materialize_grads(False)
+        return y, h2
 
     @staticmethod
     @torch.autograd.function.once_differentiable
-    def backward(ctx, dy):
+    def backward(ctx, dy, _dh2=None):
+        if dy is None:
+            return (None,) * (8 if ctx.aff else 4)
         x, w = ctx.saved_tensors
         geom = ctx.geom
         dy = dy.contiguous()
         dx = _upconv_dgrad_raw(dy, w, geom, x.dtype) if ctx.needs_input_grad[0] else None
         dw, db = _wgrad_bias_raw(ctx, x, dy, w, geom, up=True)
-        return dx, dw, db, None
+        return (dx, dw, db, None) + ((None,) * 4 if ctx.aff else ())
 
 
 class ConvAxpbyUpFn(torch.autograd.Function):
@@ -229,14 +236,22 @@
 class GBlockEndFn(torch.autograd.Function):
 
     @staticmethod
-    def forward(ctx, h1, g0, b0, g1, b1, w2, b2, geom2, sc_lo, gamma, w_out=None, b_out=None, geom_out=None, nhwc_dst=None):
+    def forward(ctx, h1, g0, b0, g1, b1, w2, b2, geom2, sc_lo, gamma, w_out=None, b_out=None, geom_out=None, nhwc_dst=None,
+                h2=None, next_mod=None):
         h1, sc_lo = h1.contiguous(), sc_lo.contiguous()
         ps = [t.contiguous().float() for t in (g0, b0, g1, b1)]
-        h2 = _affine_fwd_raw(h1, ps, 0.2)
+        if h2 is None:
+            h2 = _affine_fwd_raw(h1, ps, 0.2)
         al = gamma.detach().reshape(-1).float()
         tail = w_out is not None
-        y = _conv_fwd_raw(h2, w2, _bias_padded(b2, geom2), geom2, L.ACT_NONE, h2.dtype, res=sc_lo, alpha=al, res_mode=2,
-                          round_act=True, post_act=L.ACT_LRELU if tail else L.ACT_NONE)
+        a0_next = None
+        if next_mod is not None:
+            assert not tail
+            y, a0_next = _conv_fwd_raw(h2, w2, _bias_padded(b2, geom2), geom2, L.ACT_NONE, h2.dtype, res=sc_lo, alpha=al, res_mode=2,
+                                       round_act=True, aff=[t.contiguous().float() for t in next_mod])
+        else:
+            y = _conv_fwd_raw(h2, w2, _bias_padded(b2, geom2), geom2, L.ACT_NONE, h2.dtype, res=sc_lo, alpha=al, res_mode=2,
+                              round_act=True, post_act=L.ACT_LRELU if tail else L.ACT_NONE)
         img = None
         if tail:
             assert nhwc_dst is None or nhwc_dst._version == 0, "GBlockEndFn(nhwc_dst=): the destination must be a fresh tensor"
@@ -244,11 +259,17 @@
         ctx.geom2, ctx.geom_out, ctx.tail = geom2, geom_out, tail
         ctx.has_b2, ctx.has_bo = b2 is not None, b_out is not None
         ctx.save_for_backward(h1, *ps, h2, w2, b2, gamma, y if tail else None, w_out, img)
+        if a0_next is not None:
+            ctx.mark_non_differentiable(a0_next)
+            ctx.set_materialize_grads(False)
+            return y, a0_next
         return img if tail else y
 
     @staticmethod
     @torch.autograd.function.once_differentiable
-    def backward(ctx, dy):
+    def backward(ctx, dy, _da0=None):
+        if dy is None:
+            return (None,) * 16
         h1, g0, b0, g1, b1, h2, w2, b2, gamma, y, w_out, img = ctx.saved_tensors
         geom2, geom_out = ctx.geom2, ctx.geom_out
         dt = h1.dtype
@@ -288,13 +309,16 @@
         dgamma = dot.reshape(gamma.shape).to(gamma.dtype)
         if skip_w:
             dw2 = db2 = None
-        return (dh1, red[0], red[1], red[2], red[3], dw2, db2, None, dsc, dgamma, dw_out, db_out, None, None)
-
-
-def g_block_end(h1, mod4, c2w, c2b, geom2, sc_lo, gamma, tail=None, nhwc_dst=None):
+        return (dh1, red[0], red[1], red[2], red[3], dw2, db2, None, dsc, dgamma, dw_out, db_out, None, None, None, None)
+
+
+def g_block_end(h1, mod4, c2w, c2b, geom2, sc_lo, gamma, tail=None, nhwc_dst=None, h2=None, next_mod=None):
     if tail is None:
-        return GBlockEndFn.apply(h1, *mod4, c2w, c2b, geom2, sc_lo, gamma)
-    return GBlockEndFn.apply(h1, *mod4, c2w, c2b, geom2, sc_lo, gamma, tail[0], tail[1], tail[2], nhwc_dst)
+        if h2 is None and next_mod is None:
+            return GBlockEndFn.apply(h1, *mod4, c2w, c2b, geom2, sc_lo, gamma)
+        return GBlockEndFn.apply(h1, *mod4, c2w, c2b, geom2, sc_lo, gamma, None, None, None, None, h2,
+                                 None if next_mod is None else tuple(next_mod))
+    return GBlockEndFn.apply(h1, *mod4, c2w, c2b, geom2, sc_lo, gamma, tail[0], tail[1], tail[2], nhwc_dst, h2)
 
 
 def conv2d(x, w, b, geom, act=L.ACT_NONE, out_dtype=None, want_pool=False, out=None, pair=False):
diff --git a/xmc_gan/model/df_gan.py b/xmc_gan/model/df_gan.py
--- a/xmc_gan/model/df_gan.py
+++ b/xmc_gan/model/df_gan.py
@@ -84,16 +84,23 @@
         pending_up = False
         lrelu_done = False
         from_end = False
+        a0 = None
         for bi, (gblock, m) in enumerate(zip(self.upblocks, mods)):
             last = bi == nblk - 1 and not gblock.upsample
             fuse = gblock.fuses_end(out, pending_up)
             if last and fuse:
                 co = self.conv_out[1]
                 out8 = gblock.forward_fused(out, m, pending_up, out_lrelu=True, tail=(co.weight, co.bias, co.geom), nhwc_dst=nhwc_dst,
-                                            x_from_end=from_end)
+                                            x_from_end=from_end, a0=a0)
                 img = ops.to_nchw(out8, 3)
                 return (img, out8) if return_nhwc else img
-            out = gblock.forward_fused(out, m, pending_up, out_lrelu=last, x_from_end=from_end)
+            nm = None
+            if fuse and not last and gblock.upsample and bi + 1 < nblk and gblock.affine_in_epilogue(out):
+                nm = mods[bi + 1][0:4]
+            out = gblock.forward_fused(out, m, pending_up, out_lrelu=last, x_from_end=from_end, a0=a0, next_mod=nm)
+            a0 = None
+            if nm is not None:
+                out, a0 = out
             from_end = fuse and not last
             lrelu_done = last
             pending_up = gblock.upsample
@@ -247,16 +254,25 @@
     def fuses_end(self, x, x_pending_up):
         return bool(x_pending_up) and ops.fused_blocks() and x.is_cuda
 
-    def forward_fused(self, x, mod, x_pending_up, out_lrelu=False, tail=None, nhwc_dst=None, x_from_end=False):
+    @staticmethod
+    def affine_in_epilogue(x):
+        return ops.aff_epilogue() and x.is_cuda and x.dtype != torch.float32
+
+    def forward_fused(self, x, mod, x_pending_up, out_lrelu=False, tail=None, nhwc_dst=None, x_from_end=False, a0=None, next_mod=None):
         if not x_pending_up:
             out = ops.axpby(self.shortcut(x), self.residual(x, None, mod), self.gamma)
             return ops.lrelu(out) if out_lrelu else out
-        h, xs = ops.affine2_lrelu_skip(x, *mod[0:4], pool_grad=x_from_end) if x.is_cuda else (ops.affine2_lrelu(x, *mod[0:4]), x)
+        h, xs = ops.affine2_lrelu_skip(x, *mod[0:4], pool_grad=x_from_end, y_pre=a0) if x.is_cuda else (ops.affine2_lrelu(x, *mod[0:4]), x)
+        if self.fuses_end(x, x_pending_up) and (tail is not None or not out_lrelu):
+            h2 = None
+            if self.affine_in_epilogue(x):
+                h, h2 = ops.upconv3x3(h, self.c1.weight, self.c1.bias, self.c1.geom, aff=mod[4:8])
+            else:
+                h = ops.upconv3x3(h, self.c1.weight, self.c1.bias, self.c1.geom)
+            return ops.g_block_end(h, mod[4:8], self.c2.weight, self.c2.bias, self.c2.geom, self.shortcut(xs), self.gamma,
+                                   tail=tail, nhwc_dst=nhwc_dst, h2=h2, next_mod=next_mod)
         h = ops.upconv3x3(h, self.c1.weight, self.c1.bias, self.c1.geom)
-        if self.fuses_end(x, x_pending_up) and (tail is not None or not out_lrelu):
-            return ops.g_block_end(h, mod[4:8], self.c2.weight, self.c2.bias, self.c2.geom, self.shortcut(xs), self.gamma,
-                                   tail=tail, nhwc_dst=nhwc_dst)
-        assert tail is None
+        assert tail is None and next_mod is None
         h = ops.affine2_lrelu(h, *mod[4:8])
         if not out_lrelu and ops.fused_blocks() and h.shape[1] % 2 == 0:
             return ops.conv_axpby_up(h, self.c2.weight, self.c2.bias, self.c2.geom, self.shortcut(xs), self.gamma)
```

Measured after the change: 5954 images/s, median of 5. Within noise of the previous version (+0.1%).
